# MDIL-SNU/SevenNet

Measured on AMD Instinct MI355X. Metric: atom-steps/sec (energy+forces), SevenNet-0 100k-atom cell, 1/2/4/8 MI355X, higher is better.
Workload: dtype f32 (storage / accumulate / tensor product; in-kernel W2 products f16x3 = two fp16 terms per operand, three matrix-core products: fp32-rounding class; node linears bf16x6); 1 GPU; sevennet_0 shape (5 interaction layers), 97336-atom periodic diamond-Si cell (a=5.431 A x 23^3, sigma=0.05 A), cutoff 5.0 A, 2725408 directed edges, seeded synthetic weights; atoms=97336, edges=2725408, parallelism=single GPU, fused=auto, terms=4

## Files before the change

### include/snet_hip.h

```cpp
#ifndef SNET_HIP_H
#define SNET_HIP_H

#include <stdint.h>

#ifdef __cplusplus
extern "C" {
#endif

#define SNET_ABI_VERSION 4

int snet_abi_version(void);
const char *snet_last_error(void);
int snet_conv_num_shapes(void);
const char *snet_conv_shape_tag(int i);

typedef struct snet_edge_params {
  float cutoff;
  int32_t n_basis;
  int32_t cutoff_kind;
  int32_t poly_p;
  float cutoff_on;
  int32_t lmax;
  int32_t normalize;
} snet_edge_params;

int snet_edge_vectors(const double *pos, const int32_t *center, const int32_t *src, const double *shift, int64_t n_edges,
                      float *edge_vec, void *stream);
int snet_edge_embed_fwd(const snet_edge_params *p_host, const float *coeffs_host, const float *edge_vec,
                        int64_t n_edges, float *emb, float *sh, float *dsh, void *stream);
int snet_edge_embed_bwd(const snet_edge_params *p_host, const float *coeffs_host, const float *edge_vec,
                        int64_t n_edges, const float *g_emb, const float *g_sh, float *g_vec, int32_t accumulate,
                        void *stream);

int snet_gemm(const float *A, const float *B, float *C, int64_t n_nodes, int32_t d, int32_t K, int32_t N,
              int64_t a_node_stride, int64_t a_off, int64_t c_node_stride, int64_t c_off,
              const int32_t *row_idx, int32_t accumulate, void *stream);

typedef struct snet_gemm_desc {
  const float *B;
  const void *B_split;
  int64_t a_off, c_off;
  int32_t d, K, N, accumulate;
} snet_gemm_desc;
#define SNET_MAX_GEMM_GROUP 8
int snet_gemm_grouped(const snet_gemm_desc *descs_host, int32_t n_desc, const float *A, float *C, int64_t n_nodes,
                      int64_t a_node_stride, int64_t c_node_stride, const int32_t *row_idx, void *stream);
int64_t snet_gemm_split_size(int32_t K, int32_t N);
int snet_gemm_split_pack(const float *B_host, int32_t K, int32_t N, void *packed_host);
typedef struct snet_mlp_plan snet_mlp_plan;
int snet_radial_mlp_plan_create(int32_t nb, int32_t h1, int32_t h2, int32_t wn, const float *W0_host,
                                const float *W1_host, const float *W2_host, int32_t act, float cst, int32_t mode,
                                snet_mlp_plan **plan);
void snet_radial_mlp_plan_destroy(snet_mlp_plan *plan);
int snet_radial_mlp_fwd(const snet_mlp_plan *plan, const float *emb, int64_t n_edges, float *w_out, void *stream);
int snet_radial_mlp_bwd(const snet_mlp_plan *plan, const float *emb, const float *g_w, int64_t n_edges,
                        float *g_emb, void *stream);

int snet_act_fwd(const float *z, float *a, int64_t n, int32_t act, float cst, void *stream);
int snet_act_bwd(const float *z, const float *g_a, float *g_z, int64_t n, int32_t act, float cst, void *stream);

typedef struct snet_conv_plan snet_conv_plan;
int snet_conv_plan_create(const char *tag, snet_conv_plan **plan);
void snet_conv_plan_destroy(snet_conv_plan *plan);
int snet_conv_register_library(const char *path);
int snet_conv_plan_dims(const snet_conv_plan *plan, int32_t *dx, int32_t *dout, int32_t *nsh, int32_t *wn);

int snet_conv_fwd(const snet_conv_plan *plan, const float *x, const float *sh, const float *w, const int32_t *w_row,
                  const int32_t *row_ptr, const int32_t *src, int64_t n_dst, float scale, float *out,
                  void *stream);
#define SNET_FUSED_TERMS_DEFAULT 4
typedef struct snet_fused_plan snet_fused_plan;
int snet_radial_mlp_hidden_fwd(const snet_mlp_plan *plan, const float *emb, int64_t n_edges, float *h2, void *stream);
int snet_radial_mlp_hidden_fwd_layers(const snet_mlp_plan *const *plans, int32_t n_layers, const float *emb, int64_t n_edges,
                                      float *const *h2, void *stream);
int snet_radial_mlp_hidden_bwd(const snet_mlp_plan *plan, const float *emb, const float *g_h2, int64_t n_edges,
                               float *g_emb, void *stream);
int snet_conv_fused_available(const snet_conv_plan *plan);
int snet_fused_plan_create(const snet_conv_plan *plan, const snet_mlp_plan *mlp, int32_t terms, snet_fused_plan **out);
void snet_fused_plan_destroy(snet_fused_plan *plan);
int snet_edge_tiles(const int32_t *row_ptr, int64_t n_dst, int32_t *tile_ptr, int32_t *tile_node, int64_t tile_capacity,
                    int64_t *n_tiles, void *stream);
int snet_edge_tiles_packed(const int32_t *row_ptr, int64_t node_begin, int64_t node_end, int32_t *tile_e0,
                           int32_t *tile_nodes, int64_t tile_capacity, int64_t *n_tiles, void *stream);
int snet_fused_plan_tile_mode(const snet_fused_plan *plan);
int snet_conv_plan_transposed(const snet_conv_plan *plan, char *tag, float *col_scale, int32_t *dead, int32_t dead_capacity,
                              int32_t *n_dead);
int snet_edges_by_source(const int32_t *row_ptr, int64_t n_dst, const int32_t *eperm, const int32_t *w_row, int64_t n_edges,
                         int32_t *center_t, int32_t *w_row_t, void *stream);
int snet_conv_fwd_fused(const snet_fused_plan *plan, const float *x, const float *sh, const float *h2,
                        const int32_t *w_row, const int32_t *row_ptr, const int32_t *src, int64_t n_dst, float scale,
                        float *out, void *stream);
int snet_conv_bwd_fused(const snet_fused_plan *plan, const float *x, const float *sh, const float *dsh,
                        const float *h2, const int32_t *w_row, const int32_t *row_ptr, const int32_t *src,
                        const int32_t *tile_ptr, const int32_t *tile_node, int64_t n_tiles, float scale,
                        const float *g_out, float *g_xe, float *g_h2, const float *emb, float *g_emb, float *g_vec,
                        const float *x_rowmax, const float *g_rowmax, void *stream);
int snet_conv_bwd_fused_sh(const snet_fused_plan *plan, const float *x, const float *sh, const float *h2, const int32_t *w_row,
                           const int32_t *row_ptr, const int32_t *src, const int32_t *tile_ptr, const int32_t *tile_node,
                           int64_t n_tiles, float scale, const float *g_out, float *g_xe, float *g_h2, const float *emb,
                           float *g_emb, float *g_sh, const float *x_rowmax, const float *g_rowmax, void *stream);
int snet_fused_plan_has_mlp_tail(const snet_fused_plan *plan);
int snet_fused_plan_prefers_tangent(const snet_fused_plan *plan);
int snet_edge_embed_tangent(const snet_edge_params *p_host, const float *coeffs_host, const float *edge_vec,
                            const int32_t *edge_of_row, int64_t n_rows, float *demb, void *stream);
int snet_radial_mlp_hidden_fwd_layers_tangent(const snet_mlp_plan *const *plans, int32_t n_layers, const float *emb, const float *demb,
                                              int64_t n_rows, float *const *h2, float *const *h2d, void *stream);
int snet_conv_bwd_fused_tangent(const snet_fused_plan *plan, const float *x, const float *sh, const float *dsh, const float *h2,
                                const float *h2d, const int32_t *w_row, const int32_t *row_ptr, const int32_t *src,
                                const int32_t *tile_ptr, const int32_t *tile_node, int64_t n_tiles, float scale, const float *g_out,
                                float *g_xe, const float *edge_vec, float *g_vec, const float *x_rowmax, const float *g_rowmax,
                                void *stream);
typedef struct snet_layer0_plan snet_layer0_plan;
int snet_layer0_plan_create(const snet_conv_plan *conv, const float *W2_host, const float *table_host, float scale,
                            int32_t n_slots, snet_layer0_plan **plan);
void snet_layer0_plan_destroy(snet_layer0_plan *plan);
int snet_layer0_fold(const float *W2_host, int32_t wn, int32_t mul, const float *table_host, float scale, int32_t n_slots, int32_t l,
                     float *bt_host);
int64_t snet_layer0_scratch_size(const snet_layer0_plan *plan, int64_t n_nodes);
int snet_layer0_conv_bwd(const snet_layer0_plan *plan, const float *g_out, const float *h2, const float *h2d, const int32_t *w_row,
                         const int32_t *row_ptr, const int32_t *src, const int32_t *types, const int32_t *species_slot,
                         const float *sh, const float *dsh, const float *edge_vec, int64_t n_nodes, float *scratch, float *g_vec,
                         void *stream);
typedef struct snet_lastlayer_plan snet_lastlayer_plan;
int snet_lastlayer_plan_create(const snet_conv_plan *conv, const float *W2_host, snet_lastlayer_plan **plan);
void snet_lastlayer_plan_destroy(snet_lastlayer_plan *plan);
int snet_lastlayer_conv_bwd(const snet_lastlayer_plan *plan, const float *x, const float *g_out, const float *sh, const float *dsh,
                            const float *edge_vec, const float *h2, const float *h2d, const int32_t *col_ptr,
                            const int32_t *center_t, const int32_t *w_row_t, const int32_t *eperm, int64_t row_a, int64_t row_b,
                            float scale, float *g_x, float *g_vec, void *stream);
int snet_fused_plan_gxe_chunks(const snet_fused_plan *plan, int32_t *chunk_pos, int32_t capacity);
int snet_segment_sum_rows_chunked(const float *x, const int32_t *seg_ptr, const int32_t *perm, int64_t n_seg, int32_t dim,
                                  const int32_t *chunk_pos, float *out, void *stream);
int snet_row_absmax(const float *x, int64_t n_rows, int32_t dim, float *out, void *stream);
int snet_row_absmax_multi(const float *const *x, const int64_t *n_rows, const int32_t *dims, float *const *out, int32_t n,
                          void *stream);
int snet_row_norm2(const float *x, int64_t n_rows, int32_t dim, float mult, float *out, void *stream);
int snet_conv_bwd_edge(const snet_conv_plan *plan, const float *x, const float *sh, const float *w,
                       const int32_t *w_row, const int32_t *row_ptr, const int32_t *src, int64_t n_dst, float scale,
                       const float *g_out, float *g_w, float *g_xe, float *g_sh, void *stream);
int snet_conv_bwd_edge_vec(const snet_conv_plan *plan, const float *x, const float *sh, const float *dsh,
                           const float *w, const int32_t *w_row, const int32_t *row_ptr, const int32_t *src,
                           int64_t n_dst, float scale, const float *g_out, float *g_w, float *g_xe, float *g_vec,
                           void *stream);
int snet_conv_bwd_node(const snet_conv_plan *plan, const float *sh, const float *w, const int32_t *w_row,
                       const int32_t *col_ptr,
                       const int32_t *eperm, const int32_t *dst, int64_t n_src, float scale,
                       const float *g_out, float *g_x, void *stream);

int snet_segment_sum_rows(const float *x, const int32_t *seg_ptr, const int32_t *perm, int64_t n_seg, int32_t dim,
                          float *out, void *stream);

typedef struct snet_gate_seg {
  int32_t kind;
  int32_t in_off;
  int32_t out_off;
  int32_t mul;
  int32_t l;
  int32_t gate_off;
  int32_t act;
  float cst;
} snet_gate_seg;
#define SNET_MAX_GATE_SEGS 16
int snet_gate_fwd(float *y, const float *addend, float *out, int64_t n_nodes, int32_t dim_in, int32_t dim_out,
                  const snet_gate_seg *segs_host, int32_t n_segs, void *stream);
int snet_gate_bwd(const float *y, const float *g_out, float *g_y, int64_t n_nodes, int32_t dim_in,
                  int32_t dim_out, const snet_gate_seg *segs_host, int32_t n_segs, void *stream);
int snet_gate_bwd_norm(const float *y, const float *g_out, float *g_y, int64_t n_nodes, int32_t dim_in, int32_t dim_out,
                       const snet_gate_seg *segs, int32_t n_segs, float norm_mult, float *row_norm, void *stream);

int snet_embed_rows(const float *table, const int32_t *types, float *out, int64_t n_nodes, int32_t dim,
                    void *stream);

int snet_add_inplace(float *y, const float *x, int64_t n, void *stream);
int snet_add_row_bias(float *y, const float *bias, int64_t n_rows, int32_t dim, void *stream);
int snet_permute_cols(const float *x, const int32_t *col_idx, float *out, int64_t n_rows, int32_t dim,
                      void *stream);

int snet_rescale_reduce(const float *e_scaled, const int32_t *types, const float *scale, const float *shift,
                        int32_t n_scale, int64_t n_nodes, float *e_atom, double *energy, void *stream);

int snet_i32_shift(const int32_t *in, int32_t delta, int32_t *out, int64_t n, void *stream);

int snet_readout_energy(const float *x, int64_t n_nodes, int32_t dim, const double *v, double c, const int32_t *types,
                        const float *scale, const float *shift, int32_t n_scale, float *e_atom, double *energy,
                        void *stream);
int snet_readout_grad(const double *v, int32_t dim, const int32_t *types, const float *scale, int32_t n_scale,
                      int64_t n_nodes, float *g_x, void *stream);

int snet_edge_force(const float *g_vec, const float *edge_vec, const int32_t *row_ptr, const int32_t *col_ptr,
                    const int32_t *eperm, int64_t n_nodes, int64_t n_edges, float *forces, float *virial_atom,
                    double *virial_total, void *stream);

int snet_readout_energy_seg(const float *x, int64_t n_nodes, int32_t dim, const double *v, double c, const int32_t *types,
                            const float *scale, const float *shift, int32_t n_scale, const int32_t *seg_ptr, int32_t n_seg,
                            float *e_atom, double *energy_seg, double *energy_total, void *stream);
int snet_rescale_reduce_seg(const float *e_scaled, const int32_t *types, const float *scale, const float *shift,
                            int32_t n_scale, int64_t n_nodes, const int32_t *seg_ptr, int32_t n_seg, float *e_atom,
                            double *energy_seg, double *energy_total, void *stream);
int snet_edge_force_seg(const float *g_vec, const float *edge_vec, const int32_t *row_ptr, const int32_t *col_ptr,
// ... 168 lines not shown
```

### sevennet_amd/_lib.py

```python
from __future__ import annotations

import ctypes as C
import os

_HERE = os.path.dirname(os.path.abspath(__file__))
ABI_VERSION = 4
LIB_PATH = os.environ.get('SNET_HIP_LIB') or os.path.join(_HERE, 'libsnet_hip.so')

c_f32p = C.c_void_p
c_i32p = C.c_void_p
c_f64p = C.c_void_p
c_stream = C.c_void_p


class EdgeParams(C.Structure):
    _fields_ = [('cutoff', C.c_float), ('n_basis', C.c_int32), ('cutoff_kind', C.c_int32),
                ('poly_p', C.c_int32), ('cutoff_on', C.c_float), ('lmax', C.c_int32),
                ('normalize', C.c_int32)]


class GemmDesc(C.Structure):
    _fields_ = [('B', C.c_void_p), ('B_split', C.c_void_p), ('a_off', C.c_int64), ('c_off', C.c_int64), ('d', C.c_int32), ('K', C.c_int32),
                ('N', C.c_int32), ('accumulate', C.c_int32)]


class GateSeg(C.Structure):
    _fields_ = [('kind', C.c_int32), ('in_off', C.c_int32), ('out_off', C.c_int32), ('mul', C.c_int32),
                ('l', C.c_int32), ('gate_off', C.c_int32), ('act', C.c_int32), ('cst', C.c_float)]


SIGNATURES = {
    'snet_abi_version': (C.c_int, []),
    'snet_last_error': (C.c_char_p, []),
    'snet_conv_num_shapes': (C.c_int, []),
    'snet_conv_shape_tag': (C.c_char_p, [C.c_int]),
    'snet_edge_embed_fwd': (C.c_int, [C.POINTER(EdgeParams), C.POINTER(C.c_float), c_f32p, C.c_int64, c_f32p,
                                      c_f32p, c_f32p, c_stream]),
    'snet_edge_embed_bwd': (C.c_int, [C.POINTER(EdgeParams), C.POINTER(C.c_float), c_f32p, C.c_int64, c_f32p,
                                      c_f32p, c_f32p, C.c_int32, c_stream]),
    'snet_radial_mlp_plan_create': (C.c_int, [C.c_int32, C.c_int32, C.c_int32, C.c_int32, C.POINTER(C.c_float),
                                              C.POINTER(C.c_float), C.POINTER(C.c_float), C.c_int32, C.c_float,
                                              C.c_int32, C.POINTER(C.c_void_p)]),
    'snet_radial_mlp_plan_destroy': (None, [C.c_void_p]),
    'snet_radial_mlp_fwd': (C.c_int, [C.c_void_p, c_f32p, C.c_int64, c_f32p, c_stream]),
    'snet_radial_mlp_bwd': (C.c_int, [C.c_void_p, c_f32p, c_f32p, C.c_int64, c_f32p, c_stream]),
    'snet_conv_bwd_edge_vec': (C.c_int, [C.c_void_p, c_f32p, c_f32p, c_f32p, c_f32p, c_i32p, c_i32p, c_i32p, C.c_int64,
                                         C.c_float, c_f32p, c_f32p, c_f32p, c_f32p, c_stream]),
    'snet_gemm': (C.c_int, [c_f32p, c_f32p, c_f32p, C.c_int64, C.c_int32, C.c_int32, C.c_int32, C.c_int64,
                            C.c_int64, C.c_int64, C.c_int64, c_i32p, C.c_int32, c_stream]),
    'snet_gemm_grouped': (C.c_int, [C.POINTER(GemmDesc), C.c_int32, c_f32p, c_f32p, C.c_int64, C.c_int64, C.c_int64,
                                    c_i32p, c_stream]),
    'snet_gemm_split_size': (C.c_int64, [C.c_int32, C.c_int32]),
    'snet_gemm_split_pack': (C.c_int, [C.c_void_p, C.c_int32, C.c_int32, C.c_void_p]),
    'snet_act_fwd': (C.c_int, [c_f32p, c_f32p, C.c_int64, C.c_int32, C.c_float, c_stream]),
    'snet_act_bwd': (C.c_int, [c_f32p, c_f32p, c_f32p, C.c_int64, C.c_int32, C.c_float, c_stream]),
    'snet_conv_plan_create': (C.c_int, [C.c_char_p, C.POINTER(C.c_void_p)]),
    'snet_conv_plan_destroy': (None, [C.c_void_p]),
    'snet_conv_register_library': (C.c_int, [C.c_char_p]),
    'snet_conv_plan_dims': (C.c_int, [C.c_void_p, C.POINTER(C.c_int32), C.POINTER(C.c_int32),
                                      C.POINTER(C.c_int32), C.POINTER(C.c_int32)]),
    'snet_conv_fwd': (C.c_int, [C.c_void_p, c_f32p, c_f32p, c_f32p, c_i32p, c_i32p, c_i32p, C.c_int64, C.c_float,
                                c_f32p, c_stream]),
    'snet_radial_mlp_hidden_fwd': (C.c_int, [C.c_void_p, c_f32p, C.c_int64, c_f32p, c_stream]),
    'snet_radial_mlp_hidden_fwd_layers': (C.c_int, [C.POINTER(C.c_void_p), C.c_int32, c_f32p, C.c_int64, C.POINTER(C.c_void_p), c_stream]),
    'snet_radial_mlp_hidden_bwd': (C.c_int, [C.c_void_p, c_f32p, c_f32p, C.c_int64, c_f32p, c_stream]),
    'snet_conv_fused_available': (C.c_int, [C.c_void_p]),
    'snet_conv_plan_transposed': (C.c_int, [C.c_void_p, C.c_char_p, c_f32p, c_i32p, C.c_int32, C.POINTER(C.c_int32)]),
    'snet_edges_by_source': (C.c_int, [c_i32p, C.c_int64, c_i32p, c_i32p, C.c_int64, c_i32p, c_i32p, c_stream]),
    'snet_fused_plan_create': (C.c_int, [C.c_void_p, C.c_void_p, C.c_int32, C.POINTER(C.c_void_p)]),
    'snet_fused_plan_destroy': (None, [C.c_void_p]),
    'snet_edge_tiles': (C.c_int, [c_i32p, C.c_int64, c_i32p, c_i32p, C.c_int64, C.POINTER(C.c_int64), c_stream]),
    'snet_conv_fwd_fused': (C.c_int, [C.c_void_p, c_f32p, c_f32p, c_f32p, c_i32p, c_i32p, c_i32p, C.c_int64, C.c_float,
                                      c_f32p, c_stream]),
    'snet_conv_bwd_fused': (C.c_int, [C.c_void_p, c_f32p, c_f32p, c_f32p, c_f32p, c_i32p, c_i32p, c_i32p, c_i32p,
                                      c_i32p, C.c_int64, C.c_float, c_f32p, c_f32p, c_f32p, c_f32p, c_f32p, c_f32p, c_f32p, c_f32p,
                                      c_stream]),
    'snet_conv_bwd_fused_sh': (C.c_int, [C.c_void_p, c_f32p, c_f32p, c_f32p, c_i32p, c_i32p, c_i32p, c_i32p,
                                         c_i32p, C.c_int64, C.c_float, c_f32p, c_f32p, c_f32p, c_f32p, c_f32p, c_f32p, c_f32p, c_f32p,
                                         c_stream]),
    'snet_fused_plan_has_mlp_tail': (C.c_int, [C.c_void_p]),
    'snet_fused_plan_prefers_tangent': (C.c_int, [C.c_void_p]),
    'snet_edge_embed_tangent': (C.c_int, [C.POINTER(EdgeParams), C.POINTER(C.c_float), c_f32p, c_i32p, C.c_int64, c_f32p, c_stream]),
    'snet_radial_mlp_hidden_fwd_layers_tangent': (C.c_int, [C.POINTER(C.c_void_p), C.c_int32, c_f32p, c_f32p, C.c_int64,
                                                            C.POINTER(C.c_void_p), C.POINTER(C.c_void_p), c_stream]),
    'snet_conv_bwd_fused_tangent': (C.c_int, [C.c_void_p, c_f32p, c_f32p, c_f32p, c_f32p, c_f32p, c_i32p, c_i32p, c_i32p, c_i32p,
                                              c_i32p, C.c_int64, C.c_float, c_f32p, c_f32p, c_f32p, c_f32p, c_f32p, c_f32p,
                                              c_stream]),
    'snet_model_set_layer0_moments': (C.c_int, [C.c_void_p, C.c_int32]),
    'snet_layer0_plan_create': (C.c_int, [C.c_void_p, C.c_void_p, C.c_void_p, C.c_float, C.c_int32, C.POINTER(C.c_void_p)]),
    'snet_layer0_fold': (C.c_int, [C.c_void_p, C.c_int32, C.c_int32, C.c_void_p, C.c_float, C.c_int32, C.c_int32, C.c_void_p]),
    'snet_layer0_plan_destroy': (None, [C.c_void_p]),
    'snet_layer0_scratch_size': (C.c_int64, [C.c_void_p, C.c_int64]),
    'snet_layer0_conv_bwd': (C.c_int, [C.c_void_p, c_f32p, c_f32p, c_f32p, c_i32p, c_i32p, c_i32p, c_i32p, c_i32p, c_f32p, c_f32p, c_f32p,
                                       C.c_int64, c_f32p, c_f32p, c_stream]),
    'snet_model_set_last_layer_merged': (C.c_int, [C.c_void_p, C.c_int32]),
    'snet_lastlayer_plan_create': (C.c_int, [C.c_void_p, C.c_void_p, C.POINTER(C.c_void_p)]),
    'snet_lastlayer_plan_destroy': (None, [C.c_void_p]),
    'snet_lastlayer_conv_bwd': (C.c_int, [C.c_void_p, c_f32p, c_f32p, c_f32p, c_f32p, c_f32p, c_f32p, c_f32p, c_i32p, c_i32p, c_i32p,
                                          c_i32p, C.c_int64, C.c_int64, C.c_float, c_f32p, c_f32p, c_stream]),
    'snet_fused_plan_gxe_chunks': (C.c_int, [C.c_void_p, C.POINTER(C.c_int32), C.c_int32]),
    'snet_segment_sum_rows_chunked': (C.c_int, [c_f32p, c_i32p, c_i32p, C.c_int64, C.c_int32, c_i32p, c_f32p, c_stream]),
    'snet_edge_vectors': (C.c_int, [c_f64p, c_i32p, c_i32p, c_f64p, C.c_int64, c_f32p, c_stream]),
    'snet_row_absmax': (C.c_int, [c_f32p, C.c_int64, C.c_int32, c_f32p, c_stream]),
    'snet_row_absmax_multi': (C.c_int, [C.POINTER(C.c_void_p), C.POINTER(C.c_int64), C.POINTER(C.c_int32), C.POINTER(C.c_void_p), C.c_int32, c_stream]),
    'snet_row_norm2': (C.c_int, [c_f32p, C.c_int64, C.c_int32, C.c_float, c_f32p, c_stream]),
    'snet_conv_bwd_edge': (C.c_int, [C.c_void_p, c_f32p, c_f32p, c_f32p, c_i32p, c_i32p, c_i32p, C.c_int64, C.c_float,
                                     c_f32p, c_f32p, c_f32p, c_f32p, c_stream]),
    'snet_segment_sum_rows': (C.c_int, [c_f32p, c_i32p, c_i32p, C.c_int64, C.c_int32, c_f32p, c_stream]),
    'snet_conv_bwd_node': (C.c_int, [C.c_void_p, c_f32p, c_f32p, c_i32p, c_i32p, c_i32p, c_i32p, C.c_int64, C.c_float,
                                     c_f32p, c_f32p, c_stream]),
    'snet_gate_fwd': (C.c_int, [c_f32p, c_f32p, c_f32p, C.c_int64, C.c_int32, C.c_int32, C.POINTER(GateSeg), C.c_int32,
                                c_stream]),
    'snet_gate_bwd': (C.c_int, [c_f32p, c_f32p, c_f32p, C.c_int64, C.c_int32, C.c_int32, C.POINTER(GateSeg),
                                C.c_int32, c_stream]),
    'snet_gate_bwd_norm': (C.c_int, [c_f32p, c_f32p, c_f32p, C.c_int64, C.c_int32, C.c_int32, C.POINTER(GateSeg),
                                     C.c_int32, C.c_float, c_f32p, c_stream]),
    'snet_embed_rows': (C.c_int, [c_f32p, c_i32p, c_f32p, C.c_int64, C.c_int32, c_stream]),
    'snet_add_row_bias': (C.c_int, [c_f32p, c_f32p, C.c_int64, C.c_int32, c_stream]),
    'snet_add_inplace': (C.c_int, [c_f32p, c_f32p, C.c_int64, c_stream]),
    'snet_permute_cols': (C.c_int, [c_f32p, c_i32p, c_f32p, C.c_int64, C.c_int32, c_stream]),
    'snet_rescale_reduce': (C.c_int, [c_f32p, c_i32p, c_f32p, c_f32p, C.c_int32, C.c_int64, c_f32p, c_f64p,
                                      c_stream]),
    'snet_readout_energy': (C.c_int, [c_f32p, C.c_int64, C.c_int32, c_f64p, C.c_double, c_i32p, c_f32p, c_f32p, C.c_int32,
                                      c_f32p, c_f64p, c_stream]),
    'snet_readout_grad': (C.c_int, [c_f64p, C.c_int32, c_i32p, c_f32p, C.c_int32, C.c_int64, c_f32p, c_stream]),
    'snet_edge_force': (C.c_int, [c_f32p, c_f32p, c_i32p, c_i32p, c_i32p, C.c_int64, C.c_int64, c_f32p, c_f32p,
                                  c_f64p, c_stream]),
    'snet_readout_energy_seg': (C.c_int, [c_f32p, C.c_int64, C.c_int32, c_f64p, C.c_double, c_i32p, c_f32p, c_f32p, C.c_int32,
                                          c_i32p, C.c_int32, c_f32p, c_f64p, c_f64p, c_stream]),
    'snet_rescale_reduce_seg': (C.c_int, [c_f32p, c_i32p, c_f32p, c_f32p, C.c_int32, C.c_int64, c_i32p, C.c_int32, c_f32p, c_f64p,
                                          c_f64p, c_stream]),
    'snet_edge_force_seg': (C.c_int, [c_f32p, c_f32p, c_i32p, c_i32p, c_i32p, C.c_int64, C.c_int64, c_i32p, C.c_int32, c_f32p,
                                      c_f32p, c_f64p, c_f64p, c_stream]),
    'snet_batch_nl_count': (C.c_int, [C.c_void_p, c_i32p, C.c_int32, C.c_void_p, c_i32p, C.c_int64, C.c_double, c_i32p, c_stream]),
    'snet_batch_nl_fill': (C.c_int, [C.c_void_p, c_i32p, C.c_int32, C.c_void_p, c_i32p, C.c_int64, C.c_double, c_i32p, c_i32p,
                                     c_i32p, c_f32p, c_i32p, c_stream]),
    'snet_fire_step': (C.c_int, [c_f64p, c_f64p, c_f32p, c_f64p, C.c_int64, c_i32p, C.c_int32, c_f64p, c_f64p, c_i32p, c_i32p, c_i32p,
                                 c_f64p, c_i32p, C.c_double, C.c_double, C.c_double, C.c_int32, C.c_double, C.c_double, C.c_double,
                                 C.c_double, C.c_double, c_stream]),
    'snet_fire_cell_step': (C.c_int, [c_f64p, c_f64p, c_f64p, c_f64p, c_f64p, c_f32p, c_f64p, c_f64p, c_f64p, C.c_int64, c_i32p, C.c_int32,
                                      c_f64p, c_f64p, c_i32p, c_i32p, c_i32p, c_i32p, c_f64p, c_i32p, C.c_double, C.c_double,
                                      C.c_double, C.c_int32, C.c_double, C.c_double, C.c_double, C.c_double, C.c_double, C.c_double,
                                      C.c_int32, C.c_int32, C.c_int32, C.c_double, c_stream]),
    'snet_neb_forces': (C.c_int, [c_f64p, c_f32p, c_f64p, c_f64p, c_f64p, C.c_int64, c_i32p, C.c_int32, c_i32p, C.c_int32, c_f64p, c_i32p,
                                  C.c_int64, c_f64p, c_f64p, c_f64p, c_i32p, c_i32p, c_f64p, C.c_int32, c_i32p, c_i32p, c_f64p, c_i32p,
                                  c_stream]),
    'snet_vib_displace': (C.c_int, [c_f64p, C.c_int64, c_i32p, C.c_int32, c_i32p, c_i32p, C.c_int32, C.c_double, c_f64p, C.c_int64, c_i32p,
                                    c_stream]),
    'snet_vib_rows': (C.c_int, [c_f32p, c_f64p, C.c_int64, c_i32p, C.c_int32, c_i32p, C.c_int32, C.c_int32, C.c_double, c_i32p, c_i32p,
                                C.c_int64, C.c_void_p, C.c_int32, c_f64p, C.c_int64, c_i32p, c_stream]),
    'snet_vib_finish': (C.c_int, [c_f64p, C.c_void_p, c_i32p, C.c_int64, c_f64p, C.c_int32, C.c_int64, c_i32p, c_f64p, c_f64p, c_f64p,
                                  c_stream]),
    'snet_ph_rows': (C.c_int, [c_f32p, c_f64p, C.c_int64, c_i32p, C.c_int32, c_i32p, C.c_int32, C.c_int32, C.c_double, c_i32p, c_i32p,
                               C.c_void_p, C.c_int32, c_f64p, C.c_int64, c_i32p, c_stream]),
    'snet_ph_finish': (C.c_int, [c_f64p, C.c_void_p, c_i32p, c_i32p, C.c_int32, C.c_int64, C.c_int32, c_i32p, c_f64p, c_f64p, c_stream]),
    'snet_ph_images': (C.c_int, [c_f64p, C.c_int64, c_i32p, c_i32p, c_i32p, C.c_int32, c_f64p, c_f64p, C.c_void_p, C.c_int32, C.c_double,
                                 c_i32p, c_i32p, C.c_int64, c_i32p, c_stream]),
    'snet_ph_dynmat': (C.c_int, [c_f64p, C.c_void_p, C.c_int64, c_f64p, C.c_int64, c_i32p, c_i32p, c_f64p, C.c_int32, c_f64p, c_i32p,
                                 c_i32p, C.c_void_p, C.c_int64, c_f64p, c_i32p, c_i32p, C.c_int32, C.c_void_p, C.c_int32, C.c_int32,
                                 c_i32p, c_f64p, c_f64p, C.c_int64, c_f64p, c_stream]),
    'snet_mdb_step': (C.c_int, [c_f64p, c_f64p, c_f32p, c_f64p, c_f64p, C.c_int64, c_i32p, c_i32p, C.c_int32, c_f64p, c_i32p, c_f64p,
                                C.c_double, C.c_double, C.c_double, C.c_uint64, C.c_int32, c_stream]),
    'snet_mdb_init_velocities': (C.c_int, [c_f64p, c_f64p, C.c_int64, c_i32p, c_i32p, C.c_int32, c_f64p, C.c_uint64, C.c_int32,
                                           c_stream]),
    'snet_mdb_npt_step': (C.c_int, [c_f64p, c_f64p, c_f64p, c_f32p, c_f64p, c_f64p, c_f64p, c_f64p, C.c_int64, c_i32p, c_i32p, C.c_int32,
                                    c_f64p, c_f64p, c_f64p, c_i32p, c_f64p, c_f64p, c_f64p, c_i32p, c_i32p, C.c_double, C.c_double,
                                    C.c_double, C.c_uint64, C.c_int32, C.c_double, C.c_double, c_stream]),
    'snet_nl_grid': (C.c_int, [C.POINTER(C.c_double), C.c_double, C.POINTER(C.c_int32), C.POINTER(C.c_double), C.POINTER(C.c_int32)]),
    'snet_nl_bin': (C.c_int, [C.POINTER(C.c_double), C.c_double, C.POINTER(C.c_int32), C.POINTER(C.c_double), C.c_void_p, C.c_int64,
                              C.c_void_p, c_i32p, c_i32p, c_stream]),
    'snet_nl_count': (C.c_int, [C.POINTER(C.c_double), C.c_double, C.POINTER(C.c_int32), C.POINTER(C.c_double), C.c_void_p, c_i32p,
                                c_i32p, c_i32p, C.c_int64, c_i32p, c_stream]),
    'snet_nl_fill': (C.c_int, [C.POINTER(C.c_double), C.c_double, C.POINTER(C.c_int32), C.POINTER(C.c_double), C.c_void_p, c_i32p,
                               c_i32p, c_i32p, c_i32p, C.c_int64, c_i32p, c_i32p, c_i32p, c_f32p, c_i32p, c_stream]),
    'snet_gather_rows': (C.c_int, [c_f32p, c_i32p, c_f32p, C.c_int64, C.c_int32, c_stream]),
    'snet_scatter_add_rows': (C.c_int, [c_f32p, c_i32p, c_f32p, C.c_int64, C.c_int32, c_stream]),
    'snet_model_load': (C.c_int, [C.c_char_p, C.POINTER(C.c_void_p)]),
    'snet_model_load_memory': (C.c_int, [C.c_void_p, C.c_int64, C.POINTER(C.c_void_p)]),
    'snet_model_destroy': (None, [C.c_void_p]),
    'snet_model_info': (C.c_int, [C.c_void_p, C.POINTER(C.c_float), C.POINTER(C.c_int32), C.POINTER(C.c_int32),
                                  C.POINTER(C.c_int32), C.c_int32]),
    'snet_model_meta': (C.c_int, [C.c_void_p, C.c_char_p, C.c_char_p, C.c_int32]),
    'snet_edge_tiles_packed': (C.c_int, [c_i32p, C.c_int64, C.c_int64, c_i32p, c_i32p, C.c_int64, C.POINTER(C.c_int64), c_stream]),
    'snet_fused_plan_tile_mode': (C.c_int, [C.c_void_p]),
    'snet_i32_shift': (C.c_int, [c_i32p, C.c_int32, c_i32p, C.c_int64, c_stream]),
    'snet_model_set_interior': (C.c_int, [C.c_void_p, C.c_int64]),
    'snet_model_set_topology_cache': (C.c_int, [C.c_void_p, C.c_int32]),
    'snet_model_topology_changed': (C.c_int, [C.c_void_p]),
    'snet_model_eval_syncs': (C.c_int64, [C.c_void_p]),
    'snet_model_set_halo': (C.c_int, [C.c_void_p, C.c_void_p, C.c_void_p, C.c_void_p, C.c_int32]),
    'snet_model_eval': (C.c_int, [C.c_void_p, C.c_int64, C.c_int64, C.c_int64, c_i32p, c_i32p, c_i32p, c_i32p, c_i32p,
                                  c_i32p, c_f32p, c_i32p, c_i32p, C.c_int64, C.c_void_p, c_f32p, c_f32p, c_f32p, C.c_void_p, c_f32p, c_stream]),
    'snet_rccl_unique_id': (C.c_int, [C.c_void_p]),
    'snet_rccl_comm_create': (C.c_int, [C.c_void_p, C.c_int32, C.c_int32, C.POINTER(C.c_void_p)]),
    'snet_rccl_comm_destroy': (None, [C.c_void_p]),
    'snet_rccl_available': (C.c_int, []),
    'snet_rccl_comm_info': (C.c_int, [C.c_void_p, C.POINTER(C.c_int32), C.POINTER(C.c_int32)]),
    'snet_rccl_allreduce_sum_f64': (C.c_int, [C.c_void_p, c_f64p, C.c_int64, c_stream]),
    'snet_loopback_hub_create': (C.c_int, [C.c_int32, C.POINTER(C.c_void_p)]),
    'snet_loopback_hub_abort': (None, [C.c_void_p]),
    'snet_loopback_hub_destroy': (None, [C.c_void_p]),
    'snet_loopback_comm_create': (C.c_int, [C.c_void_p, C.c_int32, C.POINTER(C.c_void_p)]),
    'snet_halo_create': (C.c_int, [C.c_void_p, C.c_int32, C.c_int32, C.c_void_p, C.c_void_p, C.c_void_p, C.c_void_p, C.POINTER(C.c_void_p)]),
    'snet_halo_destroy': (None, [C.c_void_p]),
# ... 86 lines not shown
```

### sevennet_amd/csrc/snet_gemm.hip

```cpp
#include <cmath>
#include <cstdlib>
#include <cstring>

#include <type_traits>

#include "snet_common.h"
#include "snet_split.h"

#ifndef SNET_GEMM_OCC
#define SNET_GEMM_OCC 4
#endif
namespace {

using snet::f32x16;

struct RowMap {
  int64_t n0;
  uint32_t m0, d, inv;
  __device__ __forceinline__ RowMap(int64_t row0, int d_) : d((uint32_t)d_), inv(65536u / (uint32_t)d_ + 1u) {
    n0 = row0 / d_;
    m0 = (uint32_t)(row0 - n0 * d_);
  }
  __device__ __forceinline__ void at(int off, int64_t &n, int &m) const {
    const uint32_t x = m0 + (uint32_t)off, q = (x * inv) >> 16;
// ... 227 lines not shown
  auto load_a = [&](int q, float (&v)[MT][8]) {
#pragma unroll
    for (int mt = 0; mt < MT; ++mt) {
      const int k = 16 * q + 8 * half;
      if (a_ok[mt] && a_vec && k + 7 < K) {
        const f32x4 lo = *reinterpret_cast<const f32x4 *>(a_ptr[mt] + 16 * q);
        const f32x4 hi = *reinterpret_cast<const f32x4 *>(a_ptr[mt] + 16 * q + 4);
#pragma unroll
        for (int i = 0; i < 4; ++i) { v[mt][i] = lo[i]; v[mt][4 + i] = hi[i]; }
      } else {
#pragma unroll
        for (int i = 0; i < 8; ++i) v[mt][i] = (a_ok[mt] && k + i < K) ? a_ptr[mt][16 * q + i] : 0.f;
      }
    }
  };
  constexpr int NST = (SLAB + 255) / 256;
  auto load_b = [&](int q, u32x4 (&st)[NST]) {
    if (tile0 + NT <= n_tiles) {
#pragma unroll
      for (int i = 0; i < NST; ++i) {
        const int idx = tid + 256 * i;
        const int t = idx / 192, rem = idx - 192 * t;
        if (SLAB % 256 == 0 || idx < SLAB) st[i] = Bp[((int64_t)(tile0 + t) * nq + q) * 192 + rem];
      }
      return;
    }
#pragma unroll
    for (int i = 0; i < NST; ++i) {
      const int idx = tid + 256 * i;
      const int t = idx / 192, rem = idx - 192 * t;
      u32x4 z = {0u, 0u, 0u, 0u};
      if (idx < SLAB && tile0 + t < n_tiles) z = Bp[((int64_t)(tile0 + t) * nq + q) * 192 + rem];
      st[i] = z;
    }
  };
  auto store_b = [&](int buf, const u32x4 (&st)[NST]) {
#pragma unroll
    for (int i = 0; i < NST; ++i) {
      const int idx = tid + 256 * i;
      if (idx < SLAB) Bs[buf * SLAB + idx] = st[i];
    }
  };

  f32x16 acc[MT][NT];
#pragma unroll
  for (int mt = 0; mt < MT; ++mt)
#pragma unroll
    for (int t = 0; t < NT; ++t) acc[mt][t] = zero16();

  float av[MT][8], an[MT][8];
  u32x4 st[NST];
  load_a(0, av);
  load_b(0, st);
  store_b(0, st);
  __syncthreads();
  int buf = 0;
  for (int q = 0; q < nq; ++q) {
    const bool more = q + 1 < nq;
    if (more) {
      load_a(q + 1, an);
      load_b(q + 1, st);
    }
    Split3 a[MT];
#pragma unroll
    for (int mt = 0; mt < MT; ++mt) a[mt] = split8(av[mt]);
#pragma unroll
    for (int t = 0; t < NT; ++t) {
      bf16x8 b[3];
#pragma unroll
      for (int term = 0; term < 3; ++term) b[term] = as_bf16x8(Bs[buf * SLAB + (t * 3 + term) * 64 + lane]);
#pragma unroll
      for (int mt = 0; mt < MT; ++mt) acc[mt][t] = mfma6(a[mt], b, acc[mt][t]);
    }
    if (more) {
      store_b(buf ^ 1, st);
#pragma unroll
      for (int mt = 0; mt < MT; ++mt)
#pragma unroll
        for (int i = 0; i < 8; ++i) av[mt][i] = an[mt][i];
    }
    __syncthreads();
    buf ^= 1;
  }

  gemm_split_store<NT, MT>(acc, rows, row0, half, li, tile0, C, n_rows, N, c_node_stride, c_off, row_idx, accumulate);
}


template <int NT>
__global__ __launch_bounds__(256) void gemm_kernel(
    const float *__restrict__ A, const float *__restrict__ B, float *__restrict__ C, int64_t n_rows, int d, int K,
    int N, int64_t a_node_stride, int64_t a_off, int64_t c_node_stride, int64_t c_off,
    const int32_t *__restrict__ row_idx, int accumulate) {
  __shared__ float As[BK * AS_STRIDE];
  __shared__ float Bs[BK * 32 * NT];
  gemm_body<NT>(As, Bs, blockIdx.x, blockIdx.y, A, B, C, n_rows, d, K, N, a_node_stride, a_off, c_node_stride, c_off,
                row_idx, accumulate);
}

struct GroupArgs {
  int n;
  int first_block[SNET_MAX_GEMM_GROUP + 1];
  int nbx[SNET_MAX_GEMM_GROUP];
  snet_gemm_desc p[SNET_MAX_GEMM_GROUP];
};

__global__ __launch_bounds__(256) void gemm_grouped_kernel(GroupArgs G, const float *__restrict__ A,
                                                           float *__restrict__ C, int64_t n_nodes,
                                                           int64_t a_node_stride, int64_t c_node_stride,
                                                           const int32_t *__restrict__ row_idx) {
  __shared__ float As[BK * AS_STRIDE];
  __shared__ float Bs[BK * 128];
  int q = 0;
  while (q + 1 < G.n && (int)blockIdx.x >= G.first_block[q + 1]) ++q;
  const snet_gemm_desc P = G.p[q];
  const int b = blockIdx.x - G.first_block[q];
  const int bx = b % G.nbx[q], by = b / G.nbx[q];
  const int64_t n_rows = n_nodes * P.d;
  if (P.N > 64)
    gemm_body<4>(As, Bs, bx, by, A, P.B, C, n_rows, P.d, P.K, P.N, a_node_stride, P.a_off, c_node_stride, P.c_off,
                 row_idx, P.accumulate);
  else if (P.N > 32)
    gemm_body<2>(As, Bs, bx, by, A, P.B, C, n_rows, P.d, P.K, P.N, a_node_stride, P.a_off, c_node_stride, P.c_off,
                 row_idx, P.accumulate);
  else
    gemm_body<1>(As, Bs, bx, by, A, P.B, C, n_rows, P.d, P.K, P.N, a_node_stride, P.a_off, c_node_stride, P.c_off,
                 row_idx, P.accumulate);
}

template <int MT>
__global__ __launch_bounds__(256, MT == 1 ? SNET_GEMM_OCC : 2) void gemm_split_grouped_kernel(GroupArgs G, const float *__restrict__ A,
                                                                    float *__restrict__ C, int64_t n_nodes,
                                                                    int64_t a_node_stride, int64_t c_node_stride,
                                                                    const int32_t *__restrict__ row_idx) {
  __shared__ snet::u32x4 Bs[2 * 4 * 192];
  int q = 0;
  while (q + 1 < G.n && (int)blockIdx.x >= G.first_block[q + 1]) ++q;
  const snet_gemm_desc P = G.p[q];
  const int b = blockIdx.x - G.first_block[q];
  const int bx = b % G.nbx[q], by = b / G.nbx[q];
  const int64_t n_rows = n_nodes * P.d;
  const snet::u32x4 *Bp = static_cast<const snet::u32x4 *>(P.B_split);
  if (P.N > 64)
    gemm_split_body<4, MT>(Bs, bx, by, A, Bp, C, n_rows, P.d, P.K, P.N, a_node_stride, P.a_off, c_node_stride, P.c_off,
                           row_idx, P.accumulate);
  else if (P.N > 32)
    gemm_split_body<2, MT>(Bs, bx, by, A, Bp, C, n_rows, P.d, P.K, P.N, a_node_stride, P.a_off, c_node_stride, P.c_off,
                           row_idx, P.accumulate);
  else
    gemm_split_body<1, MT>(Bs, bx, by, A, Bp, C, n_rows, P.d, P.K, P.N, a_node_stride, P.a_off, c_node_stride, P.c_off,
                           row_idx, P.accumulate);
}

inline uint16_t bf16_rne(float v) {
  uint32_t u;
  memcpy(&u, &v, 4);
  u += 0x7fffu + ((u >> 16) & 1u);
  return (uint16_t)(u >> 16);
}
inline float bf16_f(uint16_t h) {
  const uint32_t u = (uint32_t)h << 16;
  float f;
  memcpy(&f, &u, 4);
  return f;
}

}

extern "C" int64_t snet_gemm_split_size(int32_t K, int32_t N) {
  if (K < 1 || N < 1) return 0;
  return (int64_t)((N + 31) / 32) * ((K + 15) / 16) * 3 * 64 * 16;
}

extern "C" int snet_gemm_split_pack(const float *B_host, int32_t K, int32_t N, void *packed_host) {
  SNET_REQUIRE(B_host != nullptr && packed_host != nullptr && K >= 1 && N >= 1, "snet_gemm_split_pack: bad argument");
  uint16_t *out = static_cast<uint16_t *>(packed_host);
  const int nq = (K + 15) / 16, n_tiles = (N + 31) / 32;
  for (int t = 0; t < n_tiles; ++t)
    for (int q = 0; q < nq; ++q)
      for (int lane = 0; lane < 64; ++lane)
        for (int i = 0; i < 8; ++i) {
          const int k = 16 * q + 8 * (lane >> 5) + i, n = 32 * t + (lane & 31);
          const float x = (k < K && n < N) ? B_host[(size_t)k * N + n] : 0.f;
          const uint16_t h = bf16_rne(x);
          const float r1 = x - bf16_f(h);
          const uint16_t m = bf16_rne(r1);
          const uint16_t l = bf16_rne(r1 - bf16_f(m));
          const size_t base = ((size_t)(t * nq + q) * 3) * 64;
          out[((base + 0 * 64 + lane) * 8) + i] = h;
          out[((base + 1 * 64 + lane) * 8) + i] = m;
          out[((base + 2 * 64 + lane) * 8) + i] = l;
        }
  return 0;
}

extern "C" int snet_gemm_grouped(const snet_gemm_desc *descs_host, int32_t n_desc, const float *A, float *C,
                                 int64_t n_nodes, int64_t a_node_stride, int64_t c_node_stride,
                                 const int32_t *row_idx, void *stream) {
  SNET_REQUIRE(descs_host != nullptr && n_desc >= 1 && n_desc <= SNET_MAX_GEMM_GROUP,
               "snet_gemm_grouped: 1..8 problems required");
  if (n_nodes <= 0) return 0;
  GroupArgs G;
  G.n = n_desc;
  int n_split = 0;
  int64_t rows_max = 0;  (void)rows_max;
  for (int i = 0; i < n_desc; ++i) {
    n_split += descs_host[i].B_split != nullptr;
    rows_max = rows_max > n_nodes * descs_host[i].d ? rows_max : n_nodes * descs_host[i].d;
  }
  SNET_REQUIRE(n_split == 0 || n_split == n_desc, "snet_gemm_grouped: mix of split-packed and fp32 weights in one group");
  const bool split = n_split > 0;
  static const int mt_env = getenv("SNET_GEMM_MT") ? atoi(getenv("SNET_GEMM_MT")) : 0;
  const int mt = mt_env ? mt_env : 1;
  const int bm = split ? 128 * mt : BM;
  int64_t total = 0;
  for (int i = 0; i < n_desc; ++i) {
    const snet_gemm_desc &p = descs_host[i];
    SNET_REQUIRE(p.d >= 1 && p.d <= 150 && p.K >= 1 && p.N >= 1 && (p.B != nullptr || p.B_split != nullptr),
                 "snet_gemm_grouped: bad problem");
    const int bn = p.N > 64 ? 128 : (p.N > 32 ? 64 : 32);
    const int64_t nbx = (n_nodes * p.d + bm - 1) / bm;
    const int64_t nby = (p.N + bn - 1) / bn;
    SNET_REQUIRE(nbx < (1ll << 30), "snet_gemm_grouped: too many rows");
    G.p[i] = p;
    G.nbx[i] = (int)nbx;
    G.first_block[i] = (int)total;
    total += nbx * nby;
  }
  G.first_block[n_desc] = (int)total;
  SNET_REQUIRE(total < (1ll << 31), "snet_gemm_grouped: grid too large");
  hipStream_t st = static_cast<hipStream_t>(stream);
  if (!split)
    gemm_grouped_kernel<<<(unsigned)total, 256, 0, st>>>(G, A, C, n_nodes, a_node_stride, c_node_stride, row_idx);
  else if (mt == 2)
    gemm_split_grouped_kernel<2><<<(unsigned)total, 256, 0, st>>>(G, A, C, n_nodes, a_node_stride, c_node_stride, row_idx);
  else
    gemm_split_grouped_kernel<1><<<(unsigned)total, 256, 0, st>>>(G, A, C, n_nodes, a_node_stride, c_node_stride, row_idx);
  SNET_CHECK_LAUNCH("snet_gemm_grouped");
  return 0;
}

extern "C" int snet_gemm(const float *A, const float *B, float *C, int64_t n_nodes, int32_t d, int32_t K,
                         int32_t N, int64_t a_node_stride, int64_t a_off, int64_t c_node_stride, int64_t c_off,
                         const int32_t *row_idx, int32_t accumulate, void *stream) {
  SNET_REQUIRE(d >= 1 && d <= 150 && K >= 1 && N >= 1, "snet_gemm: bad shape (1 <= d <= 150)");
  if (n_nodes <= 0) return 0;
  hipStream_t st = static_cast<hipStream_t>(stream);
  const int64_t n_rows = n_nodes * d;
  const int64_t gx = (n_rows + BM - 1) / BM;
  SNET_REQUIRE(gx < (1ll << 31), "snet_gemm: too many rows");
  if (N > 64) {
    dim3 grid((unsigned)gx, (unsigned)((N + 127) / 128));
    gemm_kernel<4><<<grid, 256, 0, st>>>(A, B, C, n_rows, d, K, N, a_node_stride, a_off, c_node_stride, c_off,
                                         row_idx, accumulate);
  } else if (N > 32) {
    dim3 grid((unsigned)gx, 1);
    gemm_kernel<2><<<grid, 256, 0, st>>>(A, B, C, n_rows, d, K, N, a_node_stride, a_off, c_node_stride, c_off,
                                         row_idx, accumulate);
  } else {
    dim3 grid((unsigned)gx, 1);
    gemm_kernel<1><<<grid, 256, 0, st>>>(A, B, C, n_rows, d, K, N, a_node_stride, a_off, c_node_stride, c_off,
                                         row_idx, accumulate);
  }
  SNET_CHECK_LAUNCH("snet_gemm");
  return 0;
}
```

### sevennet_amd/csrc/snet_model.cpp

```cpp
#include <algorithm>
#include <cmath>
#include <cstdio>
#include <cstdlib>
#include <cstring>
#include <exception>
#include <map>
#include <string>
#include <vector>

#include "snet_common.h"

namespace {

struct Reader {
  const unsigned char *p, *end;
  bool ok = true;
  void get(void *dst, size_t n) {
    if (!ok || (size_t)(end - p) < n) {
      ok = false;
      return;
    }
    memcpy(dst, p, n);
    p += n;
  }
  int32_t i32() {
    int32_t v = 0;
    get(&v, 4);
    return v;
  }
  float f32() {
    float v = 0;
    get(&v, 4);
    return v;
  }
  double f64() {
    double v = 0;
    get(&v, 8);
    return v;
  }
  std::vector<double> darr(size_t n) {
    if (!ok || n > (size_t)(end - p) / 8) {
      ok = false;
      return {};
    }
    std::vector<double> v(n);
    if (n) get(v.data(), 8 * n);
    return v;
  }
  std::vector<float> farr(size_t n) {
    if (!ok || n > (size_t)(end - p) / 4) {
      ok = false;
      return {};
    }
    std::vector<float> v(n);
    if (n) get(v.data(), 4 * n);
    return v;
  }
};

struct Block {
  int l, in_off, mul_in, out_off, mul_out, species, accumulate;
  void *W = nullptr, *WT = nullptr;
};
struct Linear {
  int dim_in = 0, dim_out = 0, n_species = 0;
  std::vector<Block> blocks;
  std::vector<std::pair<int, int>> zero, zero_in;
  struct Group {
    int species;
    std::vector<snet_gemm_desc> descs;
  };
  std::vector<Group> fwd, rev;
  float *bias = nullptr;
  float t_norm = 0.f;
  bool present() const { return dim_out > 0; }
};

void plan_groups(Linear &L, bool transpose) {
  auto &groups = transpose ? L.rev : L.fwd;
  std::vector<std::pair<int, int>> written;
  std::vector<std::vector<int>> targets;
  for (const Block &b : L.blocks) {
    const int tgt = transpose ? b.in_off : b.out_off;
    bool acc = false;
    for (auto &w : written) acc |= (w.first == tgt && w.second == b.species);
    snet_gemm_desc d;
    d.B = nullptr;
    d.B_split = transpose ? b.WT : b.W;
    d.a_off = transpose ? b.out_off : b.in_off;
    d.c_off = tgt;
    d.d = 2 * b.l + 1;
    d.K = transpose ? b.mul_out : b.mul_in;
    d.N = transpose ? b.mul_in : b.mul_out;
    d.accumulate = acc;
    bool placed = false;
    if (!groups.empty() && groups.back().species == b.species && groups.back().descs.size() < SNET_MAX_GEMM_GROUP) {
      bool clash = false;
      for (int t : targets.back()) clash |= (t == tgt);
      if (!clash) {
        groups.back().descs.push_back(d);
        targets.back().push_back(tgt);
        placed = true;
      }
    }
    if (!placed) {
      groups.push_back({b.species, {d}});
      targets.push_back({tgt});
    }
    written.push_back({tgt, b.species});
  }
}
struct Layer {
  int dx, dmid, gin, dout, wn;
  char tag[13];
  float conv_scale;
  int mlp[4];
  snet_conv_plan *conv = nullptr;
  snet_mlp_plan *mlp_plan = nullptr;
  snet_fused_plan *fused = nullptr;
  int32_t *gxe_chunks = nullptr;
  snet_conv_plan *tconv = nullptr;
  snet_mlp_plan *tmlp = nullptr;
  snet_fused_plan *tfused = nullptr;
  snet_lastlayer_plan *merged = nullptr;
  int tile_mode = 0;
  std::vector<int32_t> t_dead;
  Linear sc, si1, si2;
  std::vector<snet_gate_seg> segs;
};

bool dev_upload(const std::vector<float> &h, float **d) {
  if (h.empty()) {
    *d = nullptr;
    return true;
  }
  if (hipMalloc((void **)d, h.size() * 4) != hipSuccess) return false;
  return hipMemcpy(*d, h.data(), h.size() * 4, hipMemcpyHostToDevice) == hipSuccess;
}

bool upload_split(const std::vector<float> &w, int K, int N, void **d) {
  std::vector<unsigned char> packed((size_t)snet_gemm_split_size(K, N));
  if (snet_gemm_split_pack(w.data(), K, N, packed.data())) return false;
  if (hipMalloc(d, packed.size()) != hipSuccess) return false;
  return hipMemcpy(*d, packed.data(), packed.size(), hipMemcpyHostToDevice) == hipSuccess;
}

bool read_linear(Reader &r, Linear &L) {
  L.dim_in = r.i32();
  L.dim_out = r.i32();
  L.n_species = r.i32();
  const int nb = r.i32(), nz = r.i32(), nzi = r.i32();
  if (!r.ok || nb < 0 || nb > 4096 || nz < 0 || nz > 4096 || nzi < 0 || nzi > 4096) return false;
  L.blocks.resize(nb);
  for (auto &b : L.blocks) {
    b.l = r.i32(); b.in_off = r.i32(); b.mul_in = r.i32(); b.out_off = r.i32(); b.mul_out = r.i32();
    b.species = r.i32(); b.accumulate = r.i32();
    if (!r.ok || b.l < 0 || b.l > 8 || b.mul_in <= 0 || b.mul_out <= 0 || b.mul_in > (1 << 16) || b.mul_out > (1 << 16) ||
        b.in_off < 0 || b.out_off < 0 || b.species < -1)
      return false;
  }
  for (int i = 0; i < nz; ++i) {
    const int off = r.i32(), len = r.i32();
    L.zero.push_back({off, len});
  }
  for (int i = 0; i < nzi; ++i) {
    const int off = r.i32(), len = r.i32();
    L.zero_in.push_back({off, len});
  }
  std::map<std::pair<int, int>, std::vector<double>> row_sq;
  for (auto &b : L.blocks) {
    std::vector<float> w = r.farr((size_t)b.mul_in * b.mul_out);
    if (!r.ok) return false;
    std::vector<float> wt(w.size());
    for (int k = 0; k < b.mul_in; ++k)
      for (int n = 0; n < b.mul_out; ++n) wt[(size_t)n * b.mul_in + k] = w[(size_t)k * b.mul_out + n];
    if (!upload_split(w, b.mul_in, b.mul_out, &b.W) || !upload_split(wt, b.mul_out, b.mul_in, &b.WT)) return false;
    auto &sq = row_sq[{b.in_off, b.species}];
    sq.resize((size_t)b.mul_in, 0.0);
    for (int k = 0; k < b.mul_in; ++k)
      for (int n = 0; n < b.mul_out; ++n) sq[k] += (double)w[(size_t)k * b.mul_out + n] * w[(size_t)k * b.mul_out + n];
  }
  for (auto &kv : row_sq)
    for (double v : kv.second) L.t_norm = std::max(L.t_norm, (float)std::sqrt(v));
  const int has_bias = r.i32();
  if (!r.ok || (has_bias != 0 && has_bias != 1)) return false;
  if (has_bias) {
    std::vector<float> b = r.farr((size_t)L.dim_out);
    if (!r.ok || !dev_upload(b, &L.bias)) return false;
  }
  plan_groups(L, false);
  plan_groups(L, true);
  return r.ok;
}

struct Arena {
  char *base = nullptr;
  size_t cap = 0, off = 0;
  float *f(size_t n) {
    const size_t bytes = ((n * 4 + 255) / 256) * 256;
    float *p = reinterpret_cast<float *>(base + off);
    off += bytes;
    return p;
  }
};

}

struct snet_model {
  int n_species, n_layers, lmax, normalize, n_basis, cutoff_kind, poly_p, act_radial, n_scale, d0;
  float cutoff, cutoff_on, act_cst;
  std::vector<float> coeffs;
  float *embed = nullptr, *scale = nullptr, *shift = nullptr;
  double *ro_v = nullptr, ro_c = 0.0;
  std::vector<int> fcn_dims;
  std::vector<float *> fcn_w, fcn_wt;
  int fcn_act = 0;
  float fcn_cst = 1.f;
  double *one_d = nullptr;
  float *h0_table = nullptr, *sc0_table = nullptr;
  float scale0 = 1.f;
  std::vector<Layer> layers;
  Linear ro1, ro2;
  std::string meta;
  Arena arena;
  snet_halo_fn halo_fwd = nullptr, halo_rev = nullptr;
  void *halo_user = nullptr;
  bool fold_forces = true;
  std::vector<std::vector<int32_t>> species_rows_host;
  int32_t *species_rows = nullptr;
  size_t species_rows_cap = 0;
  std::vector<int64_t> species_off, species_cnt;
  bool topo_cache = false, topo_valid = false;
  struct TopoKey { int64_t NT, N, E; const void *row_ptr, *src, *eperm, *w_row; } topo_key{0, 0, 0, nullptr, nullptr, nullptr, nullptr};
  int32_t *c_tile_ptr = nullptr, *c_tile_node = nullptr, *c_center_t = nullptr, *c_w_row_t = nullptr;
  size_t c_tile_cap = 0, c_edge_cap = 0, c_node_cap = 0;
  int64_t c_n_tiles = 0;
  int64_t n_interior = 0;
  hipStream_t halo_stream = nullptr;
  hipEvent_t ev_h0 = nullptr, ev_h1 = nullptr;
  int32_t *c_tile_ptr_b = nullptr;
  size_t c_tile_ptr_b_cap = 0;
  int64_t c_tile_k = 0;
  bool c_split_valid = false;
  int32_t *c_ptile_e0 = nullptr, *c_ptile_nodes = nullptr;
  size_t c_ptile_cap = 0;
  int64_t c_pn_tiles = 0, c_ptile_k = 0;
  std::vector<int32_t> types_prev;
  int64_t eval_syncs = 0;
  hipStream_t side = nullptr;
  hipEvent_t ev_main = nullptr, ev_bwd[2] = {nullptr, nullptr};
  std::vector<hipEvent_t> ev_w;
  bool overlap = getenv("SNET_NO_OVERLAP") == nullptr;
  int fused_terms = [] {
    const char *e = getenv("SNET_FUSED_TERMS");
    const int v = e ? atoi(e) : SNET_FUSED_TERMS_DEFAULT;
    return v >= 1 && v <= 4 ? v : SNET_FUSED_TERMS_DEFAULT;
  }();
  bool l0_mode = [] {
    const char *e = getenv("SNET_LAYER0_MOMENTS");
    return e == nullptr || strcmp(e, "0") != 0;
  }();
  bool ll_mode = [] {
    const char *e = getenv("SNET_LAST_LAYER_MERGED");
    return e == nullptr || strcmp(e, "0") != 0;
  }();
  bool l0_shape_ok = false;
  std::vector<float> h0_host;
  struct L0Plan { snet_layer0_plan *plan; int32_t *slot; int n_slots; };
  std::map<std::vector<int32_t>, L0Plan> l0_plans;
  std::vector<int32_t> l0_present;
  const void *l0_key_types = nullptr;
  int64_t l0_key_nt = -1;
};

constexpr int64_t OVERLAP_MAX_EDGES = 1000000;

namespace {

int run_linear(snet_model *m, const Linear &L, const float *x, float *y, int64_t n, bool transpose, bool accumulate_all,
               hipStream_t st) {
  if (n <= 0) return 0;
  const int64_t a_stride = transpose ? L.dim_out : L.dim_in, c_stride = transpose ? L.dim_in : L.dim_out;
  if (!accumulate_all)
    for (auto &z : transpose ? L.zero_in : L.zero)
      if (hipMemset2DAsync(y + z.first, (size_t)c_stride * 4, 0, (size_t)z.second * 4, (size_t)n, st) != hipSuccess) {
        snet::set_error("snet_model_eval: memset failed");
        return 1;
      }
  for (const Linear::Group &g : transpose ? L.rev : L.fwd) {
    const int32_t *rows = nullptr;
    int64_t cnt = n;
    if (g.species >= 0) {
      cnt = m->species_cnt[g.species];
      rows = m->species_rows + m->species_off[g.species];
      if (cnt == 0) continue;
    }
    int rc;
    if (accumulate_all) {
      snet_gemm_desc tmp[SNET_MAX_GEMM_GROUP];
      for (size_t i = 0; i < g.descs.size(); ++i) {
        tmp[i] = g.descs[i];
        tmp[i].accumulate = 1;
      }
      rc = snet_gemm_grouped(tmp, (int)g.descs.size(), x, y, cnt, a_stride, c_stride, rows, st);
    } else {
      rc = snet_gemm_grouped(g.descs.data(), (int)g.descs.size(), x, y, cnt, a_stride, c_stride, rows, st);
    }
    if (rc) return rc;
  }
  if (!transpose && L.bias) return snet_add_row_bias(y, L.bias, n, L.dim_out, st);
  return 0;
}

}

extern "C" int snet_model_load_memory(const void *blob, int64_t n_bytes, snet_model **out) {
  SNET_REQUIRE(blob != nullptr && out != nullptr && n_bytes > 8, "snet_model_load: null / empty model");
  Reader r{static_cast<const unsigned char *>(blob), static_cast<const unsigned char *>(blob) + n_bytes};
  char magic[8];
  r.get(magic, 8);
  SNET_REQUIRE(r.ok && memcmp(magic, "SNETMDL4", 8) == 0, "snet_model_load: not a .snet model file of this version (SNETMDL4)");
  auto *m = new snet_model;
  bool good = false;
  try {
  m->n_species = r.i32(); m->n_layers = r.i32(); m->lmax = r.i32(); m->normalize = r.i32(); m->n_basis = r.i32();
  m->cutoff_kind = r.i32(); m->poly_p = r.i32(); m->act_radial = r.i32(); m->n_scale = r.i32(); m->d0 = r.i32();
  m->cutoff = r.f32(); m->cutoff_on = r.f32(); m->act_cst = r.f32();
  good = r.ok && m->n_layers > 0 && m->n_layers < 64 && m->n_basis > 0 && m->n_basis <= 16 && m->n_species > 0 &&
         m->n_species <= 4096 && m->lmax >= 0 && m->lmax <= 3 && (m->normalize == 0 || m->normalize == 1) &&
         (m->act_radial >= 0 && m->act_radial < 7) && (m->cutoff_kind == 0 || m->cutoff_kind == 1) &&
         (m->n_scale == 1 || m->n_scale == m->n_species) && m->d0 > 0 && m->d0 <= (1 << 16) && m->cutoff > 0.f;
  if (good) {
    m->coeffs = r.farr(m->n_basis);
    std::vector<float> emb = r.farr((size_t)m->n_species * m->d0), sc = r.farr(m->n_scale), sh = r.farr(m->n_scale);
    good = r.ok && dev_upload(emb, &m->embed) && dev_upload(sc, &m->scale) && dev_upload(sh, &m->shift);
    if (good) m->scale0 = sc[0];
  }
  for (int t = 0; good && t < m->n_layers; ++t) {
    Layer L;
    L.dx = r.i32(); L.dmid = r.i32(); L.gin = r.i32(); L.dout = r.i32(); L.wn = r.i32();
    r.get(L.tag, 12);
    L.tag[12] = 0;
    L.conv_scale = r.f32();
    for (int i = 0; i < 4; ++i) L.mlp[i] = r.i32();
    if (!r.ok) { good = false; break; }
    bool dims_ok = L.dx > 0 && L.dmid > 0 && L.gin > 0 && L.dout > 0 && L.wn > 0;
    for (int i = 0; i < 4; ++i) dims_ok = dims_ok && L.mlp[i] > 0 && L.mlp[i] <= (1 << 16);
    for (int v : {L.dx, L.dmid, L.gin, L.dout, L.wn}) dims_ok = dims_ok && v <= (1 << 20);
    if (!dims_ok) { good = false; break; }
    std::vector<float> w0 = r.farr((size_t)L.mlp[0] * L.mlp[1]), w1 = r.farr((size_t)L.mlp[1] * L.mlp[2]),
                       w2 = r.farr((size_t)L.mlp[2] * L.mlp[3]);
    good = r.ok && L.mlp[3] == L.wn;
    if (good && snet_radial_mlp_plan_create(L.mlp[0], L.mlp[1], L.mlp[2], L.mlp[3], w0.data(), w1.data(), w2.data(),
                                            m->act_radial, m->act_cst, 1, &L.mlp_plan)) good = false;
    if (good && snet_conv_plan_create(L.tag, &L.conv)) good = false;
    if (good && getenv("SNET_NO_FUSED") == nullptr && snet_conv_fused_available(L.conv) &&
        snet_fused_plan_create(L.conv, L.mlp_plan, m->fused_terms, &L.fused))
      good = false;
    if (good && L.fused) {
      L.tile_mode = snet_fused_plan_tile_mode(L.fused);
      std::vector<int32_t> cp((size_t)L.dx / 16);
      good = snet_fused_plan_gxe_chunks(L.fused, cp.data(), (int32_t)cp.size()) == 0 &&
             hipMalloc((void **)&L.gxe_chunks, cp.size() * 4) == hipSuccess &&
             hipMemcpy(L.gxe_chunks, cp.data(), cp.size() * 4, hipMemcpyHostToDevice) == hipSuccess;
    }
    if (good && L.fused && t > 0 && L.dmid < L.dx && getenv("SNET_NO_TRANSPOSED") == nullptr) {
      char ttag[13];
      std::vector<float> cs((size_t)L.wn);
      int32_t dead[32], nd = 0;
      if (snet_conv_plan_transposed(L.conv, ttag, cs.data(), dead, 32, &nd) == 0 && ttag[0] != 0 &&
          snet_conv_plan_create(ttag, &L.tconv) == 0 && snet_conv_fused_available(L.tconv)) {
        std::vector<float> w2t(w2);
        for (int k = 0; k < L.mlp[2]; ++k)
          for (int c = 0; c < L.wn; ++c) w2t[(size_t)k * L.wn + c] *= cs[c];
        good = snet_radial_mlp_plan_create(L.mlp[0], L.mlp[1], L.mlp[2], L.mlp[3], w0.data(), w1.data(), w2t.data(),
                                           m->act_radial, m->act_cst, 1, &L.tmlp) == 0 &&
               snet_fused_plan_create(L.tconv, L.tmlp, m->fused_terms, &L.tfused) == 0;
        L.t_dead.assign(dead, dead + 2 * nd);
      } else if (L.tconv) {
        snet_conv_plan_destroy(L.tconv);
        L.tconv = nullptr;
      }
    }
    good = good && read_linear(r, L.sc) && read_linear(r, L.si1) && read_linear(r, L.si2);
    if (good) {
      const int ns = r.i32();
      good = r.ok && ns >= 1 && ns <= SNET_MAX_GATE_SEGS;
      for (int i = 0; good && i < ns; ++i) {
        snet_gate_seg s;
        s.kind = r.i32(); s.in_off = r.i32(); s.out_off = r.i32(); s.mul = r.i32(); s.l = r.i32();
        s.gate_off = r.i32(); s.act = r.i32(); s.cst = r.f32();
        L.segs.push_back(s);
      }
      good = good && r.ok;
    }
    m->layers.push_back(L);
  }
  const int ro_kind = good ? r.i32() : 0;
  good = good && r.ok && (ro_kind == 0 || ro_kind == 1);
  if (good && ro_kind == 0) good = read_linear(r, m->ro1) && read_linear(r, m->ro2);
  if (good) {
    const int dx0 = r.i32(), gin0 = r.i32();
    good = r.ok && dx0 == m->layers[0].dx && (gin0 == 0 || gin0 == m->layers[0].gin) && (gin0 != 0) == m->layers[0].sc.present();
    if (good) {
      std::vector<float> h0 = r.farr((size_t)m->n_species * dx0), sc0 = r.farr((size_t)m->n_species * gin0);
      good = r.ok && dev_upload(h0, &m->h0_table) && dev_upload(sc0, &m->sc0_table);
      m->h0_host = h0;
    }
  }
  if (good && ro_kind == 1) {
    const int nl = r.i32();
    good = r.ok && nl >= 1 && nl <= 16;
    for (int i = 0; good && i <= nl; ++i) {
      m->fcn_dims.push_back(r.i32());
      good = r.ok && m->fcn_dims.back() >= 1 && m->fcn_dims.back() <= (1 << 16);
    }
    m->fcn_act = good ? r.i32() : 0;
    m->fcn_cst = good ? r.f32() : 1.f;
    good = good && r.ok && m->fcn_act >= 0 && m->fcn_act < snet::N_ACT && m->fcn_dims.front() == m->layers.back().dout && m->fcn_dims.back() == 1;
    for (int i = 0; good && i < nl; ++i) {
      const int di = m->fcn_dims[i], dn = m->fcn_dims[i + 1];
      std::vector<float> w = r.farr((size_t)di * dn), wt((size_t)di * dn);
      for (int a = 0; a < di && r.ok; ++a)
        for (int b = 0; b < dn; ++b) wt[(size_t)b * di + a] = w[(size_t)a * dn + b];
      float *dw = nullptr, *dwt = nullptr;
      good = r.ok && dev_upload(w, &dw) && dev_upload(wt, &dwt);
      m->fcn_w.push_back(dw);
      m->fcn_wt.push_back(dwt);
    }
    const double one = 1.0;
    good = good && hipMalloc((void **)&m->one_d, 8) == hipSuccess && hipMemcpy(m->one_d, &one, 8, hipMemcpyHostToDevice) == hipSuccess;
    if (good) m->ro1.dim_in = m->fcn_dims.front();
  }
  if (good && ro_kind == 0) {
    const int d_ro = r.i32();
    m->ro_c = r.f64();
    good = r.ok && d_ro == m->ro1.dim_in && d_ro == m->layers.back().dout;
    if (good) {
      std::vector<double> v = r.darr((size_t)d_ro);
      good = r.ok && hipMalloc((void **)&m->ro_v, v.size() * 8) == hipSuccess &&
             hipMemcpy(m->ro_v, v.data(), v.size() * 8, hipMemcpyHostToDevice) == hipSuccess;
    }
  }
  if (good) {
    const int nm = r.i32();
    good = r.ok && nm >= 0 && nm <= (1 << 20) && (int64_t)(r.end - r.p) == nm;
    if (good) m->meta.assign(reinterpret_cast<const char *>(r.p), (size_t)nm);
  }
  if (good && ("\n" + m->meta).find("\nlayer0_moments=1\n") != std::string::npos) {
    const Layer &L0 = m->layers[0];
    snet_layer0_plan *probe = nullptr;
    const int nsl = m->n_species <= 4 ? m->n_species : 1;
    if (L0.fused && L0.mlp[1] == 64 && L0.mlp[2] == 64 &&
        snet_layer0_plan_create(L0.conv, snet::mlp_plan_w2_host(L0.mlp_plan), m->h0_host.data(), L0.conv_scale, nsl, &probe) == 0) {
      m->l0_shape_ok = true;
      if (m->n_species <= 4) {
        std::vector<int32_t> all(m->n_species);
        for (int s = 0; s < m->n_species; ++s) all[s] = s;
        int32_t *ds = nullptr;
        good = hipMalloc((void **)&ds, all.size() * 4) == hipSuccess &&
               hipMemcpy(ds, all.data(), all.size() * 4, hipMemcpyHostToDevice) == hipSuccess;
        m->l0_plans[all] = {probe, ds, m->n_species};
      } else {
        snet_layer0_plan_destroy(probe);
      }
    }
  }
  if (good && m->n_layers > 1 && ("\n" + m->meta).find("\nlast_layer_merged=1\n") != std::string::npos) {
    Layer &LL = m->layers.back();
    if (LL.fused && LL.tfused && m->fused_terms == 4 && LL.mlp[1] == 64 && LL.mlp[2] == 64 &&
        snet_lastlayer_plan_create(LL.conv, snet::mlp_plan_w2_host(LL.mlp_plan), &LL.merged) != 0)
      LL.merged = nullptr;
  }
  } catch (const std::exception &e) {
    snet::set_error(std::string("exception: ") + e.what());
    good = false;
  }
  if (!good) {
    const std::string prev = snet_last_error();
    snet::set_error("snet_model_load: malformed model file or device upload failed" +
                    (prev.empty() ? std::string() : " (" + prev + ")"));
    snet_model_destroy(m);
    return 1;
  }
  *out = m;
  return 0;
}

extern "C" int snet_model_load(const char *path, snet_model **out) {
  SNET_REQUIRE(path != nullptr, "snet_model_load: null path");
  FILE *f = fopen(path, "rb");
  if (!f) {
    snet::set_error(std::string("snet_model_load: cannot open ") + path);
    return 1;
  }
  fseek(f, 0, SEEK_END);
  const long n = ftell(f);
  fseek(f, 0, SEEK_SET);
  std::vector<unsigned char> buf(n > 0 ? n : 0);
  const size_t got = n > 0 ? fread(buf.data(), 1, n, f) : 0;
  fclose(f);
  SNET_REQUIRE((long)got == n && n > 0, "snet_model_load: short read");
  return snet_model_load_memory(buf.data(), n, out);
}

extern "C" void snet_model_destroy(snet_model *m) {
  if (!m) return;
  auto free_lin = [](Linear &L) {
    for (auto &b : L.blocks) {
      if (b.W) (void)hipFree(b.W);
      if (b.WT) (void)hipFree(b.WT);
    }
    if (L.bias) (void)hipFree(L.bias);
  };
  for (float *w : m->fcn_w) if (w) (void)hipFree(w);
  for (float *w : m->fcn_wt) if (w) (void)hipFree(w);
  if (m->one_d) (void)hipFree(m->one_d);
  for (auto &kv : m->l0_plans) {
    snet_layer0_plan_destroy(kv.second.plan);
    if (kv.second.slot) (void)hipFree(kv.second.slot);
  }
  for (auto &L : m->layers) {
    snet_fused_plan_destroy(L.fused);
    snet_fused_plan_destroy(L.tfused);
    snet_lastlayer_plan_destroy(L.merged);
    snet_radial_mlp_plan_destroy(L.tmlp);
    snet_conv_plan_destroy(L.tconv);
    if (L.gxe_chunks) (void)hipFree(L.gxe_chunks);
    snet_conv_plan_destroy(L.conv);
    snet_radial_mlp_plan_destroy(L.mlp_plan);
    free_lin(L.sc); free_lin(L.si1); free_lin(L.si2);
  }
  free_lin(m->ro1); free_lin(m->ro2);
  for (hipEvent_t e : m->ev_w) if (e) (void)hipEventDestroy(e);
  for (hipEvent_t e : {m->ev_main, m->ev_bwd[0], m->ev_bwd[1]}) if (e) (void)hipEventDestroy(e);
  if (m->side) (void)hipStreamDestroy(m->side);
  if (m->halo_stream) (void)hipStreamDestroy(m->halo_stream);
// ... 290 lines not shown
    if (m->topo_cache) {
      if (m->c_node_cap < (size_t)N + 64 || m->c_tile_cap < (size_t)N + (size_t)E / 16 + 64) {
        if (m->c_tile_ptr) (void)hipFree(m->c_tile_ptr);
        if (m->c_tile_node) (void)hipFree(m->c_tile_node);
        m->c_tile_ptr = m->c_tile_node = nullptr;
        m->c_node_cap = (size_t)N + 64;
        m->c_tile_cap = (size_t)N + (size_t)E / 16 + 64;
        SNET_REQUIRE(hipMalloc((void **)&m->c_tile_ptr, m->c_node_cap * 4) == hipSuccess &&
                         hipMalloc((void **)&m->c_tile_node, m->c_tile_cap * 4) == hipSuccess, "snet_model_eval: alloc");
      }
      tile_ptr = m->c_tile_ptr;
      tile_node = m->c_tile_node;
    } else {
      tile_ptr = reinterpret_cast<int32_t *>(A.f((size_t)N + 64));
      tile_node = reinterpret_cast<int32_t *>(A.f((size_t)N + (size_t)E / 16 + 64));
    }
    if (topo_hit) {
      n_tiles = m->c_n_tiles;
    } else {
      if ((rc = snet_edge_tiles(row_ptr, N, tile_ptr, tile_node, N + E / 16 + 1, &n_tiles, st))) return rc;
      ++m->eval_syncs;
      m->c_n_tiles = n_tiles;
    }
  }
  int32_t *ptile_e0 = nullptr, *ptile_nodes = nullptr;
  int64_t pn_tiles = 0, ptile_k = 0;
  if (need_tiles[1] && E > 0) {
    const size_t cap = (size_t)N + (size_t)E / 16 + 2;
    if (m->topo_cache) {
      if (m->c_ptile_cap < cap) {
        if (m->c_ptile_e0) (void)hipFree(m->c_ptile_e0);
        if (m->c_ptile_nodes) (void)hipFree(m->c_ptile_nodes);
        m->c_ptile_e0 = m->c_ptile_nodes = nullptr;
        m->c_ptile_cap = cap + cap / 8 + 64;
        SNET_REQUIRE(hipMalloc((void **)&m->c_ptile_e0, (m->c_ptile_cap + 1) * 4) == hipSuccess &&
                         hipMalloc((void **)&m->c_ptile_nodes, m->c_ptile_cap * 8) == hipSuccess, "snet_model_eval: alloc");
      }
      ptile_e0 = m->c_ptile_e0;
      ptile_nodes = m->c_ptile_nodes;
    } else {
      ptile_e0 = reinterpret_cast<int32_t *>(A.f((size_t)N + (size_t)E / 16 + 64));
      ptile_nodes = reinterpret_cast<int32_t *>(A.f(2 * ((size_t)N + (size_t)E / 16 + 64)));
    }
    if (topo_hit) {
      pn_tiles = m->c_pn_tiles;
      ptile_k = m->c_ptile_k;
    } else {
      const int64_t cut = n_int > 0 && n_int < N ? n_int : 0;
      int64_t nb = 0;
      if (cut > 0) {
        if ((rc = snet_edge_tiles_packed(row_ptr, 0, cut, ptile_e0, ptile_nodes, (int64_t)cap, &ptile_k, st))) return rc;
        ++m->eval_syncs;
      }
      if ((rc = snet_edge_tiles_packed(row_ptr, cut, N, ptile_e0 + ptile_k, ptile_nodes + 2 * ptile_k, (int64_t)cap - ptile_k, &nb, st)))
        return rc;
      ++m->eval_syncs;
      pn_tiles = ptile_k + nb;
      m->c_pn_tiles = pn_tiles;
      m->c_ptile_k = ptile_k;
    }
  }
  int32_t *center_t = nullptr, *w_row_t = nullptr;
  float *sh_t = nullptr;
  if (any_transposed && E > 0) {
    if (m->topo_cache) {
      if (m->c_edge_cap < (size_t)E + 64) {
        if (m->c_center_t) (void)hipFree(m->c_center_t);
        if (m->c_w_row_t) (void)hipFree(m->c_w_row_t);
        m->c_center_t = m->c_w_row_t = nullptr;
        m->c_edge_cap = (size_t)E + 64;
        SNET_REQUIRE(hipMalloc((void **)&m->c_center_t, m->c_edge_cap * 4) == hipSuccess &&
                         hipMalloc((void **)&m->c_w_row_t, m->c_edge_cap * 4) == hipSuccess, "snet_model_eval: alloc");
      }
      center_t = m->c_center_t;
      w_row_t = m->c_w_row_t;
    } else {
      center_t = reinterpret_cast<int32_t *>(A.f((size_t)E + 64));
      w_row_t = reinterpret_cast<int32_t *>(A.f((size_t)E + 64));
    }
    if (need_sh_t) sh_t = A.f((size_t)E * nsh + 64);
    if (!topo_hit && (rc = snet_edges_by_source(row_ptr, N, eperm, pairs ? w_row : nullptr, E, center_t, w_row_t, st))) return rc;
    if (need_sh_t && (rc = snet_gather_rows(sh, eperm, sh_t, E, nsh, st))) return rc;
  }
  int32_t *tile_ptr_b = nullptr;
  int64_t tile_k = 0;
  if (hsplit && need_tiles[0]) {
    if (m->c_tile_ptr_b_cap < (size_t)N + 64) {
      if (m->c_tile_ptr_b) (void)hipFree(m->c_tile_ptr_b);
      m->c_tile_ptr_b = nullptr;
      m->c_tile_ptr_b_cap = (size_t)N + 64;
      m->c_split_valid = false;
      SNET_REQUIRE(hipMalloc((void **)&m->c_tile_ptr_b, m->c_tile_ptr_b_cap * 4) == hipSuccess, "snet_model_eval: alloc");
    }
    tile_ptr_b = m->c_tile_ptr_b;
    if (topo_hit && m->c_split_valid) {
      tile_k = m->c_tile_k;
    } else {
      int32_t k32 = 0;
      SNET_REQUIRE(hipMemcpyAsync(&k32, tile_ptr + n_int, 4, hipMemcpyDeviceToHost, st) == hipSuccess &&
                       hipStreamSynchronize(st) == hipSuccess, "snet_model_eval: tile readback failed");
      ++m->eval_syncs;
      tile_k = m->c_tile_k = k32;
      if ((rc = snet_i32_shift(tile_ptr, -k32, tile_ptr_b, N + 1, st))) return rc;
      m->c_split_valid = true;
    }
  }
  if (!topo_hit && !(hsplit && need_tiles[0])) m->c_split_valid = false;
  if (m->topo_cache) {
    m->topo_key = key;
    m->topo_valid = true;
  }
  float *gw_buf[2] = {nullptr, nullptr};
  bool gw_busy[2] = {false, false};
  if (ov) {
    gw_buf[0] = A.f((size_t)E * wn_max);
    gw_buf[1] = A.f((size_t)E * wn_max);
    SNET_REQUIRE(hipEventRecord(m->ev_main, st) == hipSuccess && hipStreamWaitEvent(m->side, m->ev_main, 0) == hipSuccess,
                 "snet_model_eval: stream ordering failed");
    for (int t = 0; t < Lc; ++t) {
      if ((rc = snet_radial_mlp_fwd(m->layers[t].mlp_plan, emb_w, WR, saved[t].w, m->side))) return rc;
      SNET_REQUIRE(hipEventRecord(m->ev_w[t], m->side) == hipSuccess, "snet_model_eval: stream ordering failed");
    }
  }
  const size_t mark = A.off;

  {
    const snet_mlp_plan *hp[8];
    float *ho[8], *hd[8];
    float *demb = nullptr;
    for (int pass = 0; pass < 2; ++pass) {
      int nh = 0;
      for (int t = 0; t <= Lc; ++t) {
        if (t < Lc && m->layers[t].fused && (saved[t].wd != nullptr) == (pass == 0)) {
          hp[nh] = m->layers[t].mlp_plan; ho[nh] = saved[t].w; hd[nh] = saved[t].wd; ++nh;
        }
        if (nh == 8 || (t == Lc && nh > 0)) {
          if (pass == 0 && demb == nullptr) {
            demb = A.f((size_t)WR * nb);
            if ((rc = snet_edge_embed_tangent(&ep, m->coeffs.data(), edge_vec, pairs ? pair_edge : nullptr, WR, demb, st))) return rc;
          }
          if ((rc = pass == 0 ? snet_radial_mlp_hidden_fwd_layers_tangent(hp, nh, emb_w, demb, WR, ho, hd, st)
                              : snet_radial_mlp_hidden_fwd_layers(hp, nh, emb_w, WR, ho, st))) return rc;
          nh = 0;
        }
      }
    }
  }

  for (int t = 0; t < Lc; ++t) {
    Layer &L = m->layers[t];
    A.off = mark;
    float *sc = nullptr;
    float *h = saved[t].h;
    if (t == 0) {
      if (L.sc.present()) {
        sc = saved[t].y;
        if ((rc = snet_embed_rows(m->sc0_table, types, sc, N, L.gin, st))) return rc;
      }
      if ((rc = snet_embed_rows(m->h0_table, types, h, NT, L.dx, st))) return rc;
    } else {
      if (L.sc.present()) {
        sc = saved[t].y;
        if ((rc = run_linear(m, L.sc, x, sc, N, false, false, st))) return rc;
      }
      if ((rc = run_linear(m, L.si1, x, h, N, false, false, st))) return rc;
    }
    const bool fsplit = hsplit && t > 0 && L.fused != nullptr;
    if (t > 0 && has_halo) {
      if (fsplit)
        SNET_REQUIRE(hipEventRecord(m->ev_h0, st) == hipSuccess && hipStreamWaitEvent(m->halo_stream, m->ev_h0, 0) == hipSuccess,
                     "snet_model_eval: stream ordering failed");
      if ((rc = m->halo_fwd(m->halo_user, h, NT, N, L.dx, fsplit ? (void *)m->halo_stream : stream))) {
        snet::set_error("snet_model_eval: forward halo callback failed");
        return rc;
      }
      if (fsplit) SNET_REQUIRE(hipEventRecord(m->ev_h1, m->halo_stream) == hipSuccess, "snet_model_eval: stream ordering failed");
    }
    float *mid = A.f((size_t)N * L.dmid);
    if (E == 0) SNET_REQUIRE(hipMemsetAsync(mid, 0, (size_t)N * L.dmid * 4, st) == hipSuccess, "snet_model_eval: memset");
    else
      for (auto &z : L.si2.zero_in)
        SNET_REQUIRE(hipMemset2DAsync(mid + z.first, (size_t)L.dmid * 4, 0, (size_t)z.second * 4, (size_t)N, st) == hipSuccess,
                     "snet_model_eval: memset");
    if (L.fused) {
      const int64_t na = fsplit ? n_int : 0;
      if (na > 0 && (rc = snet_conv_fwd_fused(L.fused, h, sh, saved[t].w, pairs ? w_row : nullptr, row_ptr, src, na, L.conv_scale, mid, st)))
        return rc;
      if (fsplit) SNET_REQUIRE(hipStreamWaitEvent(st, m->ev_h1, 0) == hipSuccess, "snet_model_eval: stream ordering failed");
      if ((rc = snet_conv_fwd_fused(L.fused, h, sh, saved[t].w, pairs ? w_row : nullptr, row_ptr + na, src, N - na, L.conv_scale,
                                    mid + (size_t)na * L.dmid, st)))
        return rc;
    } else {
      if (ov)
        SNET_REQUIRE(hipStreamWaitEvent(st, m->ev_w[t], 0) == hipSuccess, "snet_model_eval: stream ordering failed");
      else if ((rc = snet_radial_mlp_fwd(L.mlp_plan, emb_w, WR, saved[t].w, st)))
        return rc;
      if ((rc = snet_conv_fwd(L.conv, h, sh, saved[t].w, pairs ? w_row : nullptr, row_ptr, src, N, L.conv_scale, mid, st)))
        return rc;
    }
    float *y = saved[t].y;
    if ((rc = run_linear(m, L.si2, mid, y, N, false, sc != nullptr, st))) return rc;
    if ((rc = snet_gate_fwd(y, nullptr, x2, N, L.gin, L.dout, L.segs.data(), (int)L.segs.size(), st))) return rc;
    std::swap(x, x2);
  }
  A.off = mark;
  float *ea = e_atom ? e_atom : A.f((size_t)N + 64);
  float *g_x = x2, *gx_next = x;
  if (!m->fcn_dims.empty()) {
    const std::vector<int> &d = m->fcn_dims;
    const int nl = (int)d.size() - 1;
    std::vector<float *> zs;
    const float *a = x;
    float *z = nullptr;
    for (int i = 0; i < nl; ++i) {
      z = A.f((size_t)N * d[i + 1] + 64);
      if ((rc = snet_gemm(a, m->fcn_w[i], z, N, 1, d[i], d[i + 1], d[i], 0, d[i + 1], 0, nullptr, 0, st))) return rc;
      if (i + 1 < nl) {
        float *an = A.f((size_t)N * d[i + 1] + 64);
        if ((rc = snet_act_fwd(z, an, N * d[i + 1], m->fcn_act, m->fcn_cst, st))) return rc;
        zs.push_back(z);
        a = an;
      }
    }
    if ((rc = snet_rescale_reduce(z, types, m->scale, m->shift, m->n_scale, N, ea, energy, st))) return rc;
    float *gz = A.f((size_t)N + 64);
    if ((rc = snet_readout_grad(m->one_d, 1, types, m->scale, m->n_scale, N, gz, st))) return rc;
    for (int i = nl - 1; i >= 0; --i) {
      float *ga = i == 0 ? g_x : A.f((size_t)N * d[i] + 64);
      if ((rc = snet_gemm(gz, m->fcn_wt[i], ga, N, 1, d[i + 1], d[i], d[i + 1], 0, d[i], 0, nullptr, 0, st))) return rc;
      if (i > 0 && (rc = snet_act_bwd(zs[i - 1], ga, ga, N * d[i], m->fcn_act, m->fcn_cst, st))) return rc;
      gz = ga;
    }
  } else {
    if ((rc = snet_readout_energy(x, N, m->ro1.dim_in, m->ro_v, m->ro_c, types, m->scale, m->shift, m->n_scale, ea, energy, st)))
      return rc;
    if ((rc = snet_readout_grad(m->ro_v, m->ro1.dim_in, types, m->scale, m->n_scale, N, g_x, st))) return rc;
  }
  SNET_REQUIRE(hipMemsetAsync(g_vec, 0, (size_t)E * 3 * 4, st) == hipSuccess &&
                   (all_tangent || hipMemsetAsync(g_emb, 0, (size_t)E * nb * 4, st) == hipSuccess),
               "snet_model_eval: memset failed");
  std::vector<float *> x_max_of((size_t)Lc, nullptr);
  if (E > 0 && m->fused_terms == 4) {
    const float *xs[8];
    float *outs[8];
    int64_t rows[8];
    int32_t dims[8];
    int nj = 0;
    for (int t = 0; t <= Lc; ++t) {
      if (t < Lc && m->layers[t].fused && !(t == 0 && l0 != nullptr) &&
          !(t == Lc - 1 && ll_on && m->layers[t].tfused && t > 0)) {
        x_max_of[t] = A.f((size_t)NT + 64);
        xs[nj] = saved[t].h; outs[nj] = x_max_of[t]; rows[nj] = NT; dims[nj] = m->layers[t].dx; ++nj;
      }
      if (nj == 8 || (t == Lc && nj > 0)) {
        if ((rc = snet_row_absmax_multi(xs, rows, dims, outs, nj, st))) return rc;
        nj = 0;
      }
    }
  }
  const size_t mark2 = A.off;
  for (int t = Lc - 1; t >= 0; --t) {
    Layer &L = m->layers[t];
    A.off = mark2;
    float *g_y = A.f((size_t)N * L.gin);
    const bool merged = t > 0 && t == Lc - 1 && ll_on && L.tfused != nullptr && E > 0;
    float *g_max = (L.fused && E > 0 && m->fused_terms == 4 && !(t == 0 && l0 != nullptr) && !merged) ? A.f((size_t)N) : nullptr;
    if ((rc = snet_gate_bwd_norm(saved[t].y, g_x, g_y, N, L.gin, L.dout, L.segs.data(), (int)L.segs.size(),
                                 g_max ? L.si2.t_norm : 0.f, g_max, st)))
      return rc;
    float *g_m = A.f((size_t)N * L.dmid);
    if ((rc = run_linear(m, L.si2, g_y, g_m, N, true, false, st))) return rc;
    const bool transposed = t > 0 && L.tfused != nullptr && E > 0;
    float *g_xe = t > 0 && !transposed ? A.f((size_t)E * L.dx) : nullptr;
    if (L.fused) {
      const bool tg = saved[t].wd != nullptr;
      const bool tail = tg || snet_fused_plan_has_mlp_tail(L.fused) != 0;
      float *g_h2 = tail ? nullptr : A.f((size_t)E * 64);
      float *x_max = x_max_of[t];
      auto bwd_tiles = [&](const int32_t *tp, const int32_t *tn, int64_t nt) -> int {
        if (E <= 0 || nt <= 0 || merged) return 0;
        if (tg)
          return snet_conv_bwd_fused_tangent(L.fused, saved[t].h, sh, dsh, saved[t].w, saved[t].wd, pairs ? w_row : nullptr, row_ptr, src,
                                             tp, tn, nt, L.conv_scale, g_m, g_xe, edge_vec, g_vec, x_max, g_max, st);
        return snet_conv_bwd_fused(L.fused, saved[t].h, sh, dsh, saved[t].w, pairs ? w_row : nullptr, row_ptr, src, tp, tn, nt,
                                   L.conv_scale, g_m, g_xe, g_h2, tail ? emb : nullptr, tail ? g_emb : nullptr, g_vec, x_max, g_max, st);
      };
      const bool rsplit = hsplit && t > 0;
      const bool packed = L.tile_mode != 0;
      auto bwd_all = [&]() -> int {
        if (t == 0 && l0 != nullptr)
          return snet_layer0_conv_bwd(l0->plan, g_m, saved[t].w, saved[t].wd, pairs ? w_row : nullptr, row_ptr, src, types, l0->slot, sh,
                                      dsh, edge_vec, N, A.f(l0_scratch), g_vec, st);
        return packed ? bwd_tiles(ptile_e0, ptile_nodes, pn_tiles) : bwd_tiles(tile_ptr, tile_node, n_tiles);
      };
      if (!rsplit && (rc = bwd_all())) return rc;
      if (t > 0) {
        float *g_h = A.f((size_t)NT * L.dx);
        auto gh_rows = [&](int64_t a, int64_t b) -> int {
          if (b <= a) return 0;
          if (merged)
            return snet_lastlayer_conv_bwd(L.merged, saved[t].h, g_m, sh, dsh, edge_vec, saved[t].w, saved[t].wd, col_ptr, center_t,
                                           w_row_t, eperm, a, b, L.conv_scale, g_h, g_vec, st);
          if (transposed)
            return snet_conv_fwd_fused(L.tfused, g_m, sh_t, saved[t].w, w_row_t, col_ptr + a, center_t, b - a, L.conv_scale,
                                       g_h + (size_t)a * L.dx, st);
          return snet_segment_sum_rows_chunked(g_xe, col_ptr + a, eperm, b - a, L.dx, L.gxe_chunks, g_h + (size_t)a * L.dx, st);
        };
        if (transposed && !merged)
          for (size_t i = 0; i + 1 < L.t_dead.size(); i += 2)
            SNET_REQUIRE(hipMemset2DAsync(g_h + L.t_dead[i], (size_t)L.dx * 4, 0, (size_t)L.t_dead[i + 1] * 4, (size_t)NT, st) ==
                             hipSuccess, "snet_model_eval: memset failed");
        if (rsplit) {
          if (!transposed && (rc = packed ? bwd_tiles(ptile_e0 + ptile_k, ptile_nodes + 2 * ptile_k, pn_tiles - ptile_k)
                                          : bwd_tiles(tile_ptr_b, tile_node + tile_k, n_tiles - tile_k))) return rc;
          if ((rc = gh_rows(N, NT))) return rc;
          SNET_REQUIRE(hipEventRecord(m->ev_h0, st) == hipSuccess && hipStreamWaitEvent(m->halo_stream, m->ev_h0, 0) == hipSuccess,
                       "snet_model_eval: stream ordering failed");
          if ((rc = snet_halo_reverse_exchange(m->halo_user, g_h, NT, N, L.dx, m->halo_stream))) return rc;
          SNET_REQUIRE(hipEventRecord(m->ev_h1, m->halo_stream) == hipSuccess, "snet_model_eval: stream ordering failed");
          if ((rc = transposed ? bwd_all() : packed ? bwd_tiles(ptile_e0, ptile_nodes, ptile_k) : bwd_tiles(tile_ptr, tile_node, tile_k))) return rc;
          if ((rc = gh_rows(0, N))) return rc;
          if (!tail && (rc = snet_radial_mlp_hidden_bwd(L.mlp_plan, emb, g_h2, E, g_emb, st))) return rc;
          if (L.sc.present())
            if ((rc = run_linear(m, L.sc, g_y, gx_next, N, true, false, st))) return rc;
          SNET_REQUIRE(hipStreamWaitEvent(st, m->ev_h1, 0) == hipSuccess, "snet_model_eval: stream ordering failed");
          if ((rc = snet_halo_reverse_accumulate(m->halo_user, g_h, L.dx, st))) return rc;
          if ((rc = run_linear(m, L.si1, g_h, gx_next, N, true, L.sc.present(), st))) return rc;
          std::swap(g_x, gx_next);
          continue;
        }
        if ((rc = gh_rows(0, NT))) return rc;
        if (has_halo)
          if ((rc = m->halo_rev(m->halo_user, g_h, NT, N, L.dx, stream))) {
            snet::set_error("snet_model_eval: reverse halo callback failed");
            return rc;
          }
        if (!tail && (rc = snet_radial_mlp_hidden_bwd(L.mlp_plan, emb, g_h2, E, g_emb, st))) return rc;
        if (L.sc.present())
          if ((rc = run_linear(m, L.sc, g_y, gx_next, N, true, false, st))) return rc;
        if ((rc = run_linear(m, L.si1, g_h, gx_next, N, true, L.sc.present(), st))) return rc;
        std::swap(g_x, gx_next);
        continue;
      }
      if (!tail && (rc = snet_radial_mlp_hidden_bwd(L.mlp_plan, emb, g_h2, E, g_emb, st))) return rc;
      break;
    }
    float *g_w = ov ? gw_buf[t & 1] : A.f((size_t)E * L.wn);
    if (ov && gw_busy[t & 1])
      SNET_REQUIRE(hipStreamWaitEvent(st, m->ev_bwd[t & 1], 0) == hipSuccess, "snet_model_eval: stream ordering failed");
    if ((rc = snet_conv_bwd_edge_vec(L.conv, saved[t].h, sh, dsh, saved[t].w, pairs ? w_row : nullptr, row_ptr, src, N,
                                     L.conv_scale, g_m, g_w,
                                     g_xe, g_vec, st)))
      return rc;
    if (ov) {
      SNET_REQUIRE(hipEventRecord(m->ev_main, st) == hipSuccess && hipStreamWaitEvent(m->side, m->ev_main, 0) == hipSuccess,
                   "snet_model_eval: stream ordering failed");
      if ((rc = snet_radial_mlp_bwd(L.mlp_plan, emb, g_w, E, g_emb, m->side))) return rc;
      SNET_REQUIRE(hipEventRecord(m->ev_bwd[t & 1], m->side) == hipSuccess, "snet_model_eval: stream ordering failed");
      gw_busy[t & 1] = true;
    } else if ((rc = snet_radial_mlp_bwd(L.mlp_plan, emb, g_w, E, g_emb, st))) {
      return rc;
    }
    if (t == 0) break;
    float *g_h = A.f((size_t)NT * L.dx);
    if ((rc = snet_segment_sum_rows(g_xe, col_ptr, eperm, NT, L.dx, g_h, st))) return rc;
    if (has_halo)
      if ((rc = m->halo_rev(m->halo_user, g_h, NT, N, L.dx, stream))) {
        snet::set_error("snet_model_eval: reverse halo callback failed");
        return rc;
      }
    if (L.sc.present())
      if ((rc = run_linear(m, L.sc, g_y, gx_next, N, true, false, st))) return rc;
    if ((rc = run_linear(m, L.si1, g_h, gx_next, N, true, L.sc.present(), st))) return rc;
    std::swap(g_x, gx_next);
  }
  for (int b = 0; b < 2; ++b)
    if (gw_busy[b])
      SNET_REQUIRE(hipStreamWaitEvent(st, m->ev_bwd[b], 0) == hipSuccess, "snet_model_eval: stream ordering failed");
  if (!all_tangent && (rc = snet_edge_embed_bwd(&ep, m->coeffs.data(), edge_vec, E, g_emb, nullptr, g_vec, 1, st))) return rc;
  A.off = mark2;
  float *F = forces ? forces : A.f((size_t)NT * 3);
  if ((rc = snet_edge_force(g_vec, edge_vec, row_ptr, col_ptr, eperm, NT, E, F, virial_atom, virial, st))) return rc;
  if (has_halo && m->fold_forces) {
    if ((rc = m->halo_rev(m->halo_user, F, NT, N, 3, stream))) return rc;
    if (virial_atom && (rc = m->halo_rev(m->halo_user, virial_atom, NT, N, 6, stream))) return rc;
  }
  return 0;
}
```

### sevennet_amd/engine.py

```python
from __future__ import annotations

import ctypes as C
from dataclasses import dataclass
from typing import Dict, List, Optional

import numpy as np
import torch

from . import _lib
from .model_spec import (ACT_CST, ACT_ID, LinearSpec, ModelSpec, build_model_spec, folded_readout, lastlayer_merged_eligible,
                         layer0_moments_eligible,                         linear_modal_bias, linear_weight_matrices, species_only_tables, transposed_scalar_conv)


def _ptr(t: Optional[torch.Tensor]):
    return None if t is None else C.c_void_p(t.data_ptr())


def _stream():
    return C.c_void_p(torch.cuda.current_stream().cuda_stream)


@dataclass
class Graph:
    n_total: int
    n_local: int
    n_edges: int
    types: torch.Tensor
    center: torch.Tensor
    src: torch.Tensor
    row_ptr: torch.Tensor
    col_ptr: torch.Tensor
    eperm: torch.Tensor
    edge_vec: torch.Tensor
    order: Optional[torch.Tensor] = None
    species_rows: Optional[List[torch.Tensor]] = None
    w_row: Optional[torch.Tensor] = None
    pair_edge: Optional[torch.Tensor] = None
    n_pairs: int = 0
    tile_ptr: Optional[torch.Tensor] = None
    tile_node: Optional[torch.Tensor] = None
    n_tiles: int = 0
    src_T: Optional[torch.Tensor] = None
    w_row_T: Optional[torch.Tensor] = None
    n_interior: int = 0
    _tile_split: Optional[tuple] = None
    _tiles_packed: Optional[tuple] = None
    seg_ptr: Optional[torch.Tensor] = None
    seg_ptr_host: Optional[np.ndarray] = None

    def by_source(self, lib, stream):
        if self.src_T is None:
            self.src_T, self.w_row_T = torch.empty_like(self.eperm), torch.empty_like(self.eperm)
            _lib.check(lib.snet_edges_by_source(_ptr(self.row_ptr), self.n_local, _ptr(self.eperm), _ptr(self.w_row),
                                                self.n_edges, _ptr(self.src_T), _ptr(self.w_row_T), stream),
                       'snet_edges_by_source')
        return self.src_T, self.w_row_T

    def _packed_tiles(self):
        lib = _lib.load()
        dev = self.edge_vec.device
        cut = self.n_interior if 0 < self.n_interior < self.n_local else 0
        with torch.cuda.device(dev):
            cap = self.n_local + self.n_edges // 16 + 2
            tp = torch.empty(cap + 1, dtype=torch.int32, device=dev)
            tn = torch.empty(2 * cap, dtype=torch.int32, device=dev)
            k = 0
            n = C.c_int64()
            if cut:
                _lib.check(lib.snet_edge_tiles_packed(_ptr(self.row_ptr), 0, cut, _ptr(tp), _ptr(tn), cap, C.byref(n), _stream()),
                           'snet_edge_tiles_packed')
                k = int(n.value)
            _lib.check(lib.snet_edge_tiles_packed(_ptr(self.row_ptr), cut, self.n_local, C.c_void_p(tp.data_ptr() + 4 * k),
                                                  C.c_void_p(tn.data_ptr() + 8 * k), cap - k, C.byref(n), _stream()),
                       'snet_edge_tiles_packed')
        return tp, tn, k + int(n.value), k

    def tiles(self, mode: int = 0):
        if mode == 1:
            if self._tiles_packed is None:
                self._tiles_packed = self._packed_tiles()
            return self._tiles_packed[:3]
        if self.tile_ptr is None:
            lib = _lib.load()
            dev = self.edge_vec.device
            with torch.cuda.device(dev):
                tp = torch.empty(self.n_local + 1, dtype=torch.int32, device=dev)
                cap = self.n_local + self.n_edges // 16 + 1
                tn = torch.empty(cap, dtype=torch.int32, device=dev)
                n = C.c_int64()
                _lib.check(lib.snet_edge_tiles(_ptr(self.row_ptr), self.n_local, _ptr(tp), _ptr(tn), cap, C.byref(n),
                                               _stream()), 'snet_edge_tiles')
            self.tile_ptr, self.tile_node, self.n_tiles = tp, tn, int(n.value)
        return self.tile_ptr, self.tile_node, self.n_tiles

    def tiles_split(self, mode: int = 0):
        if mode == 1:
            tp, tn, nt = self.tiles(1)
            k = self._tiles_packed[3]
            return (tp, tn, k), (tp[k:], tn[2 * k:], nt - k)
        if self._tile_split is None:
            tp, tn, nt = self.tiles()
            k = int(tp[self.n_interior].item())
            self._tile_split = ((tp, tn, k), ((tp - k).contiguous(), tn[k:], nt - k))
        return self._tile_split

    def share_pairs(self):
        lib = _lib.load()
        E = self.n_edges
        if E == 0:
            return self
        dev = self.edge_vec.device
        with torch.cuda.device(dev):
            w_row = torch.empty(E, dtype=torch.int32, device=dev)
            pair_edge = torch.empty(E, dtype=torch.int32, device=dev)
            n = C.c_int64()
            _lib.check(lib.snet_edge_pairs(_ptr(self.row_ptr), _ptr(self.src), _ptr(self.edge_vec), self.n_local, E,
                                           _ptr(w_row), _ptr(pair_edge), C.byref(n), _stream()), 'snet_edge_pairs')
        self.w_row, self.pair_edge, self.n_pairs = w_row, pair_edge[:n.value].contiguous(), int(n.value)
        return self


def species_row_lists(types_local: torch.Tensor, num_species: int) -> List[torch.Tensor]:
    t = types_local.long()
    order = torch.sort(t, stable=True).indices.to(torch.int32)
    counts = torch.bincount(t, minlength=num_species).cpu().tolist()
    rows, o = [], 0
    for s in range(num_species):
        rows.append(order[o:o + counts[s]])
        o += counts[s]
    return rows


def build_graph(types, edge_index, edge_vec, n_local: Optional[int] = None, device='cuda',
                num_species: int = 0, share_pairs: bool = True, n_interior: int = 0) -> Graph:
    dev = torch.device(device)
    types = torch.as_tensor(types).to(dev, torch.int32)
    ei = torch.as_tensor(edge_index).to(dev, torch.int64)
    ev = torch.as_tensor(edge_vec).to(dev, torch.float32)
    n_total = int(types.shape[0])
    n_local = n_total if n_local is None else int(n_local)
    E = int(ei.shape[1])
    order = None
    if E > 1 and bool((ei[0, 1:] < ei[0, :-1]).any()):
        order = torch.sort(ei[0], stable=True).indices
        ei = ei[:, order]
        ev = ev[order]
    center, src = ei[0], ei[1]
    if E and (int(center.max()) >= n_local):
        raise ValueError('edge centers must be owned (local) atoms')
    row_ptr = torch.zeros(n_total + 1, dtype=torch.int64, device=dev)
    col_ptr = torch.zeros(n_total + 1, dtype=torch.int64, device=dev)
    if E:
        row_ptr[1:] = torch.cumsum(torch.bincount(center, minlength=n_total), 0)
        col_ptr[1:] = torch.cumsum(torch.bincount(src, minlength=n_total), 0)
        eperm = torch.sort(src, stable=True).indices
    else:
        eperm = torch.zeros(0, dtype=torch.int64, device=dev)
    rows = None
    if num_species:
        rows = species_row_lists(types[:n_local], num_species)
    g = Graph(n_total, n_local, E, types, center.to(torch.int32).contiguous(), src.to(torch.int32).contiguous(),
              row_ptr.to(torch.int32), col_ptr.to(torch.int32), eperm.to(torch.int32).contiguous(),
              ev.contiguous(), order, rows)
    g.n_interior = int(n_interior) if 0 < int(n_interior) < n_local else 0
    return g.share_pairs() if share_pairs and dev.type == 'cuda' else g


def _pack_split(m: np.ndarray, dev) -> torch.Tensor:
    lib = _lib.load()
    m = np.ascontiguousarray(m, dtype=np.float32)
    K, N = m.shape
    buf = np.empty(int(lib.snet_gemm_split_size(K, N)), np.uint8)
    _lib.check(lib.snet_gemm_split_pack(C.c_void_p(m.ctypes.data), K, N, C.c_void_p(buf.ctypes.data)),
               'snet_gemm_split_pack')
    return torch.from_numpy(buf).to(dev)


class _Linear:

    def __init__(self, spec: LinearSpec, flat: np.ndarray, dev, split: bool = True, modal_idx: int = -1, bias_flat=None):
        self.spec = spec
        self.split = split
        b = linear_modal_bias(spec, flat, modal_idx, bias_flat)
        self.bias = None if b is None else torch.from_numpy(b).to(dev)
        mats = linear_weight_matrices(spec, flat)
        if split:
            self.w = [_pack_split(m, dev) for m in mats]
            self.wt = [_pack_split(np.ascontiguousarray(m.T), dev) for m in mats]
        else:
            self.w = [torch.from_numpy(m).to(dev) for m in mats]
            self.wt = [torch.from_numpy(np.ascontiguousarray(m.T)).to(dev) for m in mats]
        fed = {b.in_off for b in spec.blocks}
        self.zero_in = [(off, m * (2 * l + 1)) for off, (m, l, _) in zip(spec.irreps_in.offsets(), spec.irreps_in) if off not in fed]
        self.groups_fwd = self._plan(transpose=False)
        self.groups_T = self._plan(transpose=True)
        acc = {}
        for b, m in zip(spec.blocks, mats):
            acc[(b.in_off, b.species)] = acc.get((b.in_off, b.species), 0.0) + (np.asarray(m, np.float32).astype(np.float64) ** 2).sum(1)
        self.t_norm = float(max(np.sqrt(v).max() for v in acc.values())) if acc else 0.0

    def _plan(self, transpose: bool):
        sp = self.spec
        groups = []
        written = set()
        pair_seen = {}
        for b, w, wt in zip(sp.blocks, self.w, self.wt):
            if transpose:
                tgt, a_off, c_off, K, N, B = b.in_off, b.out_off, b.in_off, b.mul_out, b.mul_in, wt
            else:
                tgt, a_off, c_off, K, N, B = b.out_off, b.in_off, b.out_off, b.mul_in, b.mul_out, w
            key = (tgt, b.species)
            acc = key in written
            desc = _lib.GemmDesc(None if self.split else B.data_ptr(), B.data_ptr() if self.split else None, a_off, c_off,
                                 2 * b.l + 1, K, N, int(acc))
            placed = False
            if groups and groups[-1][0] == b.species and len(groups[-1][1]) < 8 and tgt not in groups[-1][2]:
                groups[-1][1].append(desc)
                groups[-1][2].add(tgt)
                placed = True
            if not placed:
                groups.append([b.species, [desc], {tgt}])
            written.add(key)
        out = []
        for species, descs, _ in groups:
            arr = (_lib.GemmDesc * len(descs))(*descs)
            out.append((species, arr, len(descs)))
        return out


class _Span:

    def __init__(self, eng, name):
        self.eng, self.name = eng, name

    def __enter__(self):
        self.on = self.eng.events is not None and (self.eng.event_filter is None or self.name in self.eng.event_filter)
        if self.on:
            self.a = torch.cuda.Event(enable_timing=True)
            self.b = torch.cuda.Event(enable_timing=True)
            self.a.record()

    def __exit__(self, *exc):
        if self.on:
            self.b.record()
            self.eng.events.append((self.name, self.a, self.b))


class HipForceEngine:
    OVERLAP_MAX_EDGES = 1_000_000

    def __init__(self, config: dict, state_dict: Dict[str, np.ndarray], device='cuda:0', mlp_mode: str = 'bf16x6',
                 linear_mode: str = 'bf16x6', fused='auto', fused_terms='f16x3', modal=None, overlap: bool = True,
                 mlp_tail: bool = True, transposed_conv: bool = True, species_tables: bool = True,
                 fold_readout: bool = True, tangent: bool = True, layer0_moments: bool = True,
                 last_layer_merged: bool = True):
        self.fused_terms, self.fused_mode = self._check_modes(mlp_mode, linear_mode, fused, fused_terms)
        self.mlp_mode = mlp_mode
        self.linear_mode = linear_mode
        self.overlap, self.halo_split = bool(overlap), True
        self._side = None
        self._acc_descs = {}
        self.events = None
        self.event_filter = None
        self.lib = _lib.load()
        if not torch.cuda.is_available():
            raise RuntimeError('HipForceEngine needs a ROCm GPU (no CPU fallback exists)')
        self.dev = torch.device(device)
        self.spec: ModelSpec = build_model_spec(config)
        sp = self.spec
        self.modal_idx = mi = sp.modal_index(modal)
        shapes = sp.param_shapes()
        sd = {}
        for k, shp in shapes.items():
            if k not in state_dict:
                raise KeyError(f'state_dict is missing {k}')
            v = state_dict[k]
            v = v.detach().cpu().numpy() if isinstance(v, torch.Tensor) else np.asarray(v)
            if k.startswith('rescale_atomic_energy.'):
                sd[k] = v.astype(np.float64)
                continue
            if v.size != int(np.prod(shp)):
                raise ValueError(f'{k}: checkpoint tensor has {v.size} entries, the model config implies {shp}')
            sd[k] = v.astype(np.float64).reshape(shp)

        self.edge_params = _lib.EdgeParams(sp.cutoff, sp.n_basis, sp.cutoff_kind, sp.cutoff_p, sp.cutoff_on,
                                           sp.lmax_edge, int(sp.normalize_sph))
        self.coeffs = (C.c_float * sp.n_basis)(*[float(v) for v in sd['edge_embedding.basis_function.coeffs']])
        self.nsh = sp.irreps_sh.dim
        with torch.cuda.device(self.dev):
            emb = linear_weight_matrices(sp.embed, sd[sp.embed.name])
            assert len(emb) == 1
            eb = linear_modal_bias(sp.embed, sd[sp.embed.name], mi, sd.get(sp.embed.bias_name))
            table = emb[0] if eb is None else emb[0] + eb[None, :]
            self.embed_table = torch.from_numpy(np.ascontiguousarray(table, np.float32)).to(self.dev)
            self.layers = []
            split = linear_mode == 'bf16x6'
            for ls in sp.layers:
                L = type('L', (), {})()
                L.spec = ls
                L.sc = _Linear(ls.sc, sd[ls.sc.name], self.dev, split, mi) if ls.sc is not None else None
                L.si1 = _Linear(ls.si1, sd[ls.si1.name], self.dev, split, mi, sd.get(ls.si1.bias_name))
                L.si2 = _Linear(ls.si2, sd[ls.si2.name], self.dev, split, mi, sd.get(ls.si2.bias_name))
                L.mlp_w, L.mlp_wt = [], []
                rw = ls.radial_weights(sd)
                for i in range(len(ls.mlp_dims) - 1):
                    w = rw[i] / np.sqrt(ls.mlp_dims[i])
                    L.mlp_w.append(torch.from_numpy(np.ascontiguousarray(w, dtype=np.float32)).to(self.dev))
                    L.mlp_wt.append(torch.from_numpy(np.ascontiguousarray(w.T, dtype=np.float32)).to(self.dev))
                L.fused_mlp = (len(ls.mlp_dims) == 4 and ls.mlp_dims[1] == 64 and ls.mlp_dims[2] == 64
                               and ls.mlp_dims[0] <= 32)
                L.mlp_plan = None
                if L.fused_mlp:
                    d = ls.mlp_dims
                    hw = [np.ascontiguousarray(rw[i] / np.sqrt(d[i]), dtype=np.float32) for i in range(3)]
                    fp = [w.ctypes.data_as(C.POINTER(C.c_float)) for w in hw]
                    mp = C.c_void_p()
                    _lib.check(self.lib.snet_radial_mlp_plan_create(d[0], d[1], d[2], d[3], fp[0], fp[1], fp[2],
                                                                    ACT_ID[sp.act_radial], ACT_CST[sp.act_radial],
                                                                    1 if mlp_mode == 'bf16x6' else 0, C.byref(mp)),
                               'snet_radial_mlp_plan_create')
                    L.mlp_plan, L.w2_host = mp, hw[2]
                L.scale = 1.0 / float(sd[f'{ls.t}_convolution.denominator'][0])
                if ls.conv.tag not in _lib.compiled_conv_tags():
                    from .jit import ensure_conv_shape
                    ensure_conv_shape(ls.conv)
                plan = C.c_void_p()
                _lib.check(self.lib.snet_conv_plan_create(ls.conv.tag.encode(), C.byref(plan)), 'snet_conv_plan_create')
                L.plan = plan
                L.fplan = None
                L.mlp_tail = False
                can = bool(L.fused_mlp and mlp_mode == 'bf16x6' and self.lib.snet_conv_fused_available(plan))
                if fused is True and not can:
                    raise RuntimeError(f'layer {ls.t}: no fused tensor-product kernels for this shape / mlp_mode')
                if fused is not False and can:
                    fpl = C.c_void_p()
                    _lib.check(self.lib.snet_fused_plan_create(plan, L.mlp_plan, self.fused_terms, C.byref(fpl)),
                               'snet_fused_plan_create')
                    L.fplan = fpl
                    L.mlp_tail = bool(self.lib.snet_fused_plan_has_mlp_tail(fpl)) and mlp_tail
                    nch = ls.si1.dim_out // 16
                    cp = (C.c_int32 * nch)()
                    _lib.check(self.lib.snet_fused_plan_gxe_chunks(fpl, cp, nch), 'snet_fused_plan_gxe_chunks')
                    L.gxe_chunks = torch.tensor(list(cp), dtype=torch.int32, device=self.dev)
                L.fused_fwd = L.fplan is not None and fused in ('auto', True, 'fwd')
                L.fused_bwd = L.fplan is not None and fused in ('auto', True, 'bwd')
                L.tile_mode = int(self.lib.snet_fused_plan_tile_mode(L.fplan)) if L.fplan is not None else 0
                L.tangent = bool(L.fused_bwd and tangent and self.lib.snet_fused_plan_prefers_tangent(L.fplan))
                L.tplan = None
                tr = transposed_scalar_conv(ls.conv) if (L.fused_bwd and transposed_conv and ls.t > 0) else None
                if tr is not None and ls.conv.irreps_out.dim < ls.conv.irreps_x.dim:
                    spec_t, kappa = tr
                    if spec_t.tag not in _lib.compiled_conv_tags():
                        from .jit import ensure_conv_shape
                        ensure_conv_shape(spec_t)
                    ttag, col = C.create_string_buffer(13), np.empty(ls.conv.weight_numel, np.float32)
                    dead, nd = (C.c_int32 * 32)(), C.c_int32()
                    _lib.check(self.lib.snet_conv_plan_transposed(plan, ttag, col.ctypes.data_as(C.c_void_p), C.cast(dead, C.c_void_p),
                                                                  32, C.byref(nd)), 'snet_conv_plan_transposed')
                    assert ttag.value.decode() == spec_t.tag, (ttag.value, spec_t.tag)
                    w2t = np.ascontiguousarray(np.asarray(hw[2], np.float32) * col[None, :], dtype=np.float32)
                    tpl, tmlp, tfp = C.c_void_p(), C.c_void_p(), C.c_void_p()
                    _lib.check(self.lib.snet_conv_plan_create(spec_t.tag.encode(), C.byref(tpl)), 'snet_conv_plan_create')
                    _lib.check(self.lib.snet_radial_mlp_plan_create(d[0], d[1], d[2], d[3], fp[0], fp[1],
                                                                    w2t.ctypes.data_as(C.POINTER(C.c_float)),
                                                                    ACT_ID[sp.act_radial], ACT_CST[sp.act_radial], 1, C.byref(tmlp)),
                               'snet_radial_mlp_plan_create')
                    _lib.check(self.lib.snet_fused_plan_create(tpl, tmlp, self.fused_terms, C.byref(tfp)), 'snet_fused_plan_create')
                    L.tplan, L.tmlp, L.tconv = tfp, tmlp, tpl
                    L.t_dead = [(dead[2 * i], dead[2 * i + 1]) for i in range(nd.value)]
                self._init_last_layer(L, len(sp.layers), last_layer_merged)
                segs = (_lib.GateSeg * len(ls.gate.segs))()
                inv_act = {v: k for k, v in ACT_ID.items()}
                for i, s in enumerate(ls.gate.segs):
                    segs[i] = _lib.GateSeg(s.kind, s.in_off, s.out_off, s.mul, s.l, s.gate_off, s.act,
                                           ACT_CST[inv_act[s.act]])
                L.gate_segs = segs
                self.layers.append(L)
            self.h0_table = self.sc0_table = None
            if species_tables:
                h0, sc0 = species_only_tables(sp, sd, mi)
                self.h0_table = torch.from_numpy(h0).to(self.dev)
                self.sc0_table = None if sc0 is None else torch.from_numpy(sc0).to(self.dev)
            self.ro_v = self.ro_fcn = None
            if sp.readout_fcn_dims:
                d = sp.readout_fcn_dims
                ws = [np.ascontiguousarray(sd[f'readout_FCN.fcn.layer{i}.weight'] / np.sqrt(d[i]), dtype=np.float32) for i in range(len(d) - 1)]
                self.ro_fcn = type('F', (), {})()
                self.ro_fcn.dims = d
                self.ro_fcn.w = [torch.from_numpy(w).to(self.dev) for w in ws]
                self.ro_fcn.wt = [torch.from_numpy(np.ascontiguousarray(w.T)).to(self.dev) for w in ws]
                self.ro_fcn.act, self.ro_fcn.cst = ACT_ID[sp.readout_fcn_act], ACT_CST[sp.readout_fcn_act]
            else:
                if fold_readout:
                    v, self.ro_c = folded_readout(sp, sd, mi)
                    self.ro_v = torch.from_numpy(v).to(self.dev)
                self.ro1 = _Linear(sp.readout1, sd[sp.readout1.name], self.dev, split, mi, sd.get(sp.readout1.bias_name))
                self.ro2 = _Linear(sp.readout2, sd[sp.readout2.name], self.dev, split, mi, sd.get(sp.readout2.bias_name))
            sc_v, sh_v = sp.rescale_vectors(sd, mi)
            self.n_scale = len(sc_v)
            self.scale = torch.tensor(sc_v, dtype=torch.float32, device=self.dev)
            self.shift = torch.tensor(sh_v, dtype=torch.float32, device=self.dev)
            self.scale0 = float(sc_v[0])
        self.act_radial = ACT_ID[sp.act_radial]
        self.act_cst = ACT_CST[sp.act_radial]
        self.needs_species_rows = any(ls.sc is not None and ls.sc.n_species for ls in sp.layers)
        self._init_layer0(layer0_moments)

    @staticmethod
    def _check_modes(mlp_mode, linear_mode, fused, fused_terms):
        if mlp_mode not in ('bf16x6', 'fp32') or linear_mode not in ('bf16x6', 'fp32'):
            raise ValueError("mlp_mode / linear_mode must be 'bf16x6' or 'fp32'")
        if fused not in ('auto', True, False, 'fwd', 'bwd'):
            raise ValueError("fused must be 'auto', True, False, 'fwd' or 'bwd'")
        codes = {'bf16': 1, 'bf16x3': 2, 'bf16x6': 3, 'f16x3': 4}
        if fused_terms not in codes and fused_terms not in codes.values():
            raise ValueError(f"fused_terms must be one of {sorted(codes)} (or the C-ABI code 1..4)")
        code = int(codes.get(fused_terms, fused_terms))
        return code, {v: k for k, v in codes.items()}[code]

    def __del__(self):
        try:
            for pl, _, _ in (getattr(self, 'l0_plans', None) or {}).values():
                self.lib.snet_layer0_plan_destroy(pl)
            for L in getattr(self, 'layers', []):
                if getattr(L, 'fplan', None) is not None:
                    self.lib.snet_fused_plan_destroy(L.fplan)
                if getattr(L, 'tplan', None) is not None:
                    self.lib.snet_fused_plan_destroy(L.tplan)
                    self.lib.snet_conv_plan_destroy(L.tconv)
                    self.lib.snet_radial_mlp_plan_destroy(L.tmlp)
                if getattr(L, 'mplan', None) is not None:
                    self.lib.snet_lastlayer_plan_destroy(L.mplan)
                self.lib.snet_conv_plan_destroy(L.plan)
                if getattr(L, 'mlp_plan', None) is not None:
                    self.lib.snet_radial_mlp_plan_destroy(L.mlp_plan)
        except Exception:
            pass

    def kernel_times_ms(self) -> Dict[str, List[float]]:
        out: Dict[str, List[float]] = {}
        for name, a, b in self.events or []:
            out.setdefault(name, []).append(a.elapsed_time(b))
        return out

    def _new(self, *shape):
        return torch.empty(*shape, dtype=torch.float32, device=self.dev)

    def _gemm(self, A, B, Cm, n_nodes, d, K, N, a_stride, a_off, c_stride, c_off, rows=None, acc=False):
        _lib.check(self.lib.snet_gemm(_ptr(A), _ptr(B), _ptr(Cm), n_nodes, d, K, N, a_stride, a_off, c_stride,
                                      c_off, _ptr(rows), int(acc), _stream()), 'snet_gemm')

    def _run_groups(self, groups, A, Cm, n, a_stride, c_stride, g: Graph, force_acc=False):
        for species, arr, cnt in groups:
            rows, m = None, n
            if species >= 0:
                rows = g.species_rows[species]
                m = rows.numel()
                if m == 0:
                    continue
            if force_acc:
                arr2 = self._acc_descs.get(id(arr))
                if arr2 is None:
                    arr2 = (_lib.GemmDesc * cnt)(*[_lib.GemmDesc(d.B, d.B_split, d.a_off, d.c_off, d.d, d.K, d.N, 1) for d in arr[:cnt]])
                    self._acc_descs[id(arr)] = arr2
                arr = arr2
            _lib.check(self.lib.snet_gemm_grouped(arr, cnt, _ptr(A), _ptr(Cm), m, a_stride, c_stride, _ptr(rows),
                                                  _stream()), 'snet_gemm_grouped')

    def _linear(self, lin: _Linear, x, n, g: Graph, out=None, accumulate=False):
        sp = lin.spec
        y = self._new(max(n, 0), sp.dim_out) if out is None else out
        if not accumulate:
            for off, ln in sp.zero_out:
                y[:, off:off + ln].zero_()
        self._run_groups(lin.groups_fwd, x, y, n, sp.dim_in, sp.dim_out, g, force_acc=accumulate)
        if lin.bias is not None and n > 0:
            _lib.check(self.lib.snet_add_row_bias(_ptr(y), _ptr(lin.bias), n, sp.dim_out, _stream()), 'snet_add_row_bias')
        return y

    def _linear_T(self, lin: _Linear, gy, n, g: Graph, out=None, accumulate=False):
        sp = lin.spec
        gx = out if out is not None else self._new(max(n, 0), sp.dim_in)
        if not accumulate:
            fed = {b.in_off for b in sp.blocks}
            for off, (m, l, _) in zip(sp.irreps_in.offsets(), sp.irreps_in):
                if off not in fed:
                    gx[:, off:off + m * (2 * l + 1)].zero_()
        self._run_groups(lin.groups_T, gy, gx, n, sp.dim_out, sp.dim_in, g, force_acc=accumulate)
        return gx

    def _mlp_fwd(self, L, emb, E, out=None):
        dims = L.spec.mlp_dims
        if L.fused_mlp:
            w = self._new(E, dims[3]) if out is None else out
            _lib.check(self.lib.snet_radial_mlp_fwd(L.mlp_plan, _ptr(emb), E, _ptr(w), _stream()), 'snet_radial_mlp_fwd')
            return w, None
        zs, a = [], emb
        for i, wm in enumerate(L.mlp_w):
            z = self._new(E, dims[i + 1])
            self._gemm(a, wm, z, E, 1, dims[i], dims[i + 1], dims[i], 0, dims[i + 1], 0)
            if i + 1 < len(L.mlp_w):
                zs.append(z)
                a = self._new(E, dims[i + 1])
                _lib.check(self.lib.snet_act_fwd(_ptr(z), _ptr(a), z.numel(), self.act_radial, self.act_cst,
                                                 _stream()), 'snet_act_fwd')
                zs.append(a)
            else:
                return z, zs

    def _mlp_bwd(self, L, emb, zs, g_w, g_emb_total, E):
        dims = L.spec.mlp_dims
        if L.fused_mlp:
            _lib.check(self.lib.snet_radial_mlp_bwd(L.mlp_plan, _ptr(emb), _ptr(g_w), E, _ptr(g_emb_total), _stream()),
                       'snet_radial_mlp_bwd')
            return
        g = g_w
        nl = len(L.mlp_w)
        for i in range(nl - 1, -1, -1):
            if i == 0:
                self._gemm(g, L.mlp_wt[0], g_emb_total, E, 1, dims[1], dims[0], dims[1], 0, dims[0], 0, None, True)
            else:
                ga = self._new(E, dims[i])
                self._gemm(g, L.mlp_wt[i], ga, E, 1, dims[i + 1], dims[i], dims[i + 1], 0, dims[i], 0)
                z = zs[2 * (i - 1)]
                _lib.check(self.lib.snet_act_bwd(_ptr(z), _ptr(ga), _ptr(ga), z.numel(), self.act_radial,
                                                 self.act_cst, _stream()), 'snet_act_bwd')
                g = ga

    def _init_last_layer(self, L, n_layers, last_layer_merged):
        ls = L.spec
        L.mplan = None
        if (last_layer_merged and L.tplan is not None and ls.t == n_layers - 1 and L.fused_fwd and self.fused_terms == 4
                and lastlayer_merged_eligible(ls.conv, ls.mlp_dims)):
            mpl = C.c_void_p()
            _lib.check(self.lib.snet_lastlayer_plan_create(L.plan, L.w2_host.ctypes.data_as(C.c_void_p), C.byref(mpl)),
                       'snet_lastlayer_plan_create')
            L.mplan, L.tangent = mpl, True

    def _init_layer0(self, layer0_moments):
        L0 = self.layers[0]
        self.l0_plans = None
        if (layer0_moments and self.h0_table is not None and L0.fused_fwd and L0.fused_bwd
                and layer0_moments_eligible(L0.spec.conv, L0.spec.mlp_dims)):
            self.l0_plans, self.h0_host = {}, self.h0_table.cpu().numpy()

    def _layer0_plan(self, g: Graph):
        if self.l0_plans is None or g.n_edges == 0:
            return None
        ns = self.h0_host.shape[0]
        present = tuple(range(ns)) if ns <= 4 else getattr(g, '_species_present', None)
        if present is None:
            present = g._species_present = tuple(int(v) for v in torch.unique(g.types).cpu())
        if not 1 <= len(present) <= 4 or present[0] < 0 or present[-1] >= ns:
            return None
        if present not in self.l0_plans:
            L0, plan = self.layers[0], C.c_void_p()
            table = np.ascontiguousarray(self.h0_host[list(present)], np.float32)
            _lib.check(self.lib.snet_layer0_plan_create(L0.plan, C.c_void_p(L0.w2_host.ctypes.data), C.c_void_p(table.ctypes.data),
                                                        L0.scale, len(present), C.byref(plan)), 'snet_layer0_plan_create')
            slot = np.zeros(ns, np.int32)
            slot[list(present)] = np.arange(len(present), dtype=np.int32)
            self.l0_plans[present] = (plan, torch.from_numpy(slot).to(self.dev), len(present))
        return self.l0_plans[present]

    def _layer0_bwd(self, c, g_m, h2, h2d, g_vec):
        g, (plan, slot, _) = c.g, c.l0
        scratch = self._new(int(self.lib.snet_layer0_scratch_size(plan, c.N)))
        with _Span(self, 'conv_bwd_l0'):
            _lib.check(self.lib.snet_layer0_conv_bwd(plan, _ptr(g_m), _ptr(h2), _ptr(h2d), _ptr(c.w_row), _ptr(g.row_ptr), _ptr(g.src),
                                                     _ptr(g.types), _ptr(slot), _ptr(c.sh), _ptr(c.dsh), _ptr(g.edge_vec), c.N,
                                                     _ptr(scratch), _ptr(g_vec), c.st), 'snet_layer0_conv_bwd')

    def compute(self, g: Graph, halo=None, want_atomic_virial: bool = False, keep: bool = False):
        lib, sp = self.lib, self.spec
        if self.needs_species_rows and g.species_rows is None:
            raise ValueError('graph was built without num_species but the model has a per-species self-connection')
        if g.seg_ptr is not None and (halo is not None or g.n_total != g.n_local):
            raise ValueError('a batch of systems (Graph.seg_ptr) cannot be combined with a halo decomposition')
        with torch.cuda.device(self.dev):
            c = self._begin(g, halo, keep)
            x = self._forward_layers(c)
            e_atom, energy, g_x = self._readout(c, x)
            g_vec = self._reverse_layers(c, g_x)
            return self._forces(c, g_vec, e_atom, energy, want_atomic_virial)

    def _begin(self, g: Graph, halo, keep: bool):
        from types import SimpleNamespace
        lib, sp = self.lib, self.spec
        st = _stream()
        N, NT, E = g.n_local, g.n_total, g.n_edges
        nb, nsh = sp.n_basis, self.nsh
        inter = {}
        emb, sh, dsh = self._new(E, nb), self._new(E, nsh), self._new(E, nsh * 3)
        with _Span(self, 'edge_embed_fwd'):
            _lib.check(lib.snet_edge_embed_fwd(C.byref(self.edge_params), self.coeffs, _ptr(g.edge_vec), E,
                                               _ptr(emb), _ptr(sh), _ptr(dsh), st), 'snet_edge_embed_fwd')
        pairs = g.w_row is not None and all(L.fused_mlp for L in self.layers)
        w_row = g.w_row if pairs else None
        if pairs:
            emb_p = self._new(g.n_pairs, nb)
            _lib.check(lib.snet_gather_rows(_ptr(emb), _ptr(g.pair_edge), _ptr(emb_p), g.n_pairs, nb, st),
                       'snet_gather_rows')
        side = None
        w_ready = {}
        any_fused = any(L.fused_fwd or L.fused_bwd for L in self.layers)
        l0 = self._layer0_plan(g)
        if E > 0:
            for L in self.layers:
                if L.fused_bwd:
                    g.tiles(L.tile_mode)
        if self.overlap and E <= self.OVERLAP_MAX_EDGES and not any_fused and all(L.fused_mlp for L in self.layers):
            if self._side is None:
                self._side = torch.cuda.Stream(device=self.dev)
            side = self._side
            main = torch.cuda.current_stream()
            rows_w = g.n_pairs if pairs else E
            w_bufs = [self._new(rows_w, L_.spec.conv.weight_numel) for L_ in self.layers]
            wn_max = max(L_.spec.conv.weight_numel for L_ in self.layers)
            gw_bufs = [self._new(E * wn_max), self._new(E * wn_max)]
            gw_done = [None, None]
            side.wait_stream(main)
            with torch.cuda.stream(side):
                for t_, L_ in enumerate(self.layers):
                    with _Span(self, f'radial_mlp_fwd[wn={L_.spec.conv.weight_numel}]@side'):
                        self._mlp_fwd(L_, emb_p if pairs else emb, rows_w, out=w_bufs[t_])
                    ev = torch.cuda.Event()
                    ev.record(side)
                    w_ready[t_] = (w_bufs[t_], ev)
        d0 = sp.embed.dim_out
        x = None
        if keep or self.h0_table is None:
            x = self._new(NT, d0)
            _lib.check(lib.snet_embed_rows(_ptr(self.embed_table), _ptr(g.types), _ptr(x), NT, d0, st),
                       'snet_embed_rows')
        if keep:
            inter['edge_embedding'], inter['edge_attr'], inter['x_embed'] = emb, sh, x[:N]
        saved = []
        split = bool(halo is not None and g.n_interior and hasattr(halo, 'forward_start') and hasattr(halo, 'reverse_start')
                     and E > 0 and self.halo_split)
        h2_rows = g.n_pairs if pairs else E
        h2_of = {t_: self._new(h2_rows, 64) for t_, L_ in enumerate(self.layers) if L_.fused_fwd or L_.fused_bwd}
        h2d_of = {t_: self._new(h2_rows, 64) for t_, L_ in enumerate(self.layers) if L_.tangent or (t_ == 0 and l0 is not None)}
        with _Span(self, 'radial_mlp_hidden_fwd'):
            demb = None
            if h2d_of:
                demb = self._new(h2_rows, nb)
                _lib.check(lib.snet_edge_embed_tangent(C.byref(self.edge_params), self.coeffs, _ptr(g.edge_vec),
                                                       _ptr(g.pair_edge) if pairs else None, h2_rows, _ptr(demb), st), 'snet_edge_embed_tangent')
            for tg_, ts in ((True, sorted(h2d_of)), (False, sorted(set(h2_of) - set(h2d_of)))):
                for i in range(0, len(ts), 8):
                    grp = ts[i:i + 8]
                    plans = (C.c_void_p * len(grp))(*[self.layers[t_].mlp_plan for t_ in grp])
                    outs = (C.c_void_p * len(grp))(*[h2_of[t_].data_ptr() for t_ in grp])
                    if tg_:
                        outs_d = (C.c_void_p * len(grp))(*[h2d_of[t_].data_ptr() for t_ in grp])
                        _lib.check(lib.snet_radial_mlp_hidden_fwd_layers_tangent(plans, len(grp), _ptr(emb_p if pairs else emb), _ptr(demb),
                                                                                 h2_rows, outs, outs_d, st),
                                   'snet_radial_mlp_hidden_fwd_layers_tangent')
                    else:
                        _lib.check(lib.snet_radial_mlp_hidden_fwd_layers(plans, len(grp), _ptr(emb_p if pairs else emb), h2_rows, outs, st),
                                   'snet_radial_mlp_hidden_fwd_layers')
        return SimpleNamespace(g=g, halo=halo, keep=keep, st=st, N=N, NT=NT, E=E, nb=nb, nsh=nsh, inter=inter, emb=emb, sh=sh, dsh=dsh,
                               pairs=pairs, w_row=w_row, emb_p=emb_p if pairs else None, side=side, w_ready=w_ready,
                               gw_bufs=gw_bufs if side is not None else None, gw_done=gw_done if side is not None else None,
                               x=x, saved=saved, split=split, h2_of=h2_of, h2d_of=h2d_of, l0=l0)

    def _forward_layers(self, c):
        lib, g, halo, keep, st, inter = self.lib, c.g, c.halo, c.keep, c.st, c.inter
        N, NT, E = c.N, c.NT, c.E
        emb, sh, pairs, emb_p, w_row, side, w_ready = c.emb, c.sh, c.pairs, c.emb_p, c.w_row, c.side, c.w_ready
        x, saved, split, h2_of = c.x, c.saved, c.split, c.h2_of
        for t, L in enumerate(self.layers):
            ls = L.spec
            n_in = NT if t == 0 else N
            with _Span(self, 'node_linear_fwd'):
                h = self._new(NT, ls.si1.dim_out)
                if t == 0 and self.h0_table is not None:
                    _lib.check(lib.snet_embed_rows(_ptr(self.h0_table), _ptr(g.types), _ptr(h), NT, ls.si1.dim_out, st),
                               'snet_embed_rows')
                else:
                    self._linear(L.si1, x, n_in, g, out=h)
            pending = None
            if t > 0 and halo is not None:
                with _Span(self, 'halo_fwd'):
                    if hasattr(halo, 'forward_start'):
                        pending = halo.forward_start(h, N)
                    else:
                        halo.forward(h, N)
            with _Span(self, 'node_linear_fwd'):
                if t == 0 and self.h0_table is not None:
                    sc = None
                    if self.sc0_table is not None:
                        sc = self._new(N, ls.gate.irreps_in.dim)
                        _lib.check(lib.snet_embed_rows(_ptr(self.sc0_table), _ptr(g.types), _ptr(sc), N, ls.gate.irreps_in.dim,
                                                       st), 'snet_embed_rows')
                else:
                    sc = self._linear(L.sc, x, N, g) if L.sc is not None else None
            dmid = ls.conv.irreps_out.dim
            m = self._new(N, dmid)
            if E == 0:
                m.zero_()
            else:
                for off, ln in L.si2.zero_in:
                    m[:, off:off + ln].zero_()
            h2 = w = zs = None
            rows_w = g.n_pairs if pairs else E
            h2 = h2_of.pop(t, None)
            if not (L.fused_fwd and L.fused_bwd):
                if side is not None:
                    (w, ev), zs = w_ready.pop(t), None
                    torch.cuda.current_stream().wait_event(ev)
                else:
                    with _Span(self, f'radial_mlp_fwd[wn={ls.conv.weight_numel}]'):
                        w, zs = self._mlp_fwd(L, emb_p, g.n_pairs) if pairs else self._mlp_fwd(L, emb, E)
            def conv_rows(a, b):
                if b <= a:
                    return
                rp, mo = C.c_void_p(g.row_ptr.data_ptr() + 4 * a), C.c_void_p(m.data_ptr() + 4 * a * dmid)
                if L.fused_fwd:
                    with _Span(self, f'conv_fwd_fused[{ls.conv.tag}]'):
                        _lib.check(lib.snet_conv_fwd_fused(L.fplan, _ptr(h), _ptr(sh), _ptr(h2), _ptr(w_row), rp,
                                                           _ptr(g.src), b - a, L.scale, mo, st), 'snet_conv_fwd_fused')
                else:
                    with _Span(self, f'conv_fwd[{ls.conv.tag}]'):
                        _lib.check(lib.snet_conv_fwd(L.plan, _ptr(h), _ptr(sh), _ptr(w), _ptr(w_row), rp,
                                                     _ptr(g.src), b - a, L.scale, mo, st), 'snet_conv_fwd')
            n_int = g.n_interior if (pending is not None and split) else 0
            conv_rows(0, n_int)
            if pending is not None:
                with _Span(self, 'halo_fwd'):
                    halo.forward_finish(pending)
            conv_rows(n_int, N)
            if L.fused_bwd:
                w = None
            with _Span(self, 'node_linear_fwd'):
                y = self._linear(L.si2, m, N, g) if sc is None else self._linear(L.si2, m, N, g, out=sc, accumulate=True)
            xo = self._new(N, ls.gate.irreps_out.dim)
            with _Span(self, 'gate_fwd'):
                _lib.check(lib.snet_gate_fwd(_ptr(y), None, _ptr(xo), N, ls.gate.irreps_in.dim,
                                             ls.gate.irreps_out.dim, L.gate_segs, len(ls.gate.segs), st), 'snet_gate_fwd')
            saved.append((h, w, zs, y, h2))
            if keep:
                inter[f'{t}_si1'], inter[f'{t}_conv'], inter[f'{t}_gate_in'], inter[f'{t}_x'] = h[:N], m, y, xo
            x = xo
        return x

    def _readout(self, c, x):
        lib, sp, g, st, N = self.lib, self.spec, c.g, c.st, c.N
        e_atom = self._new(N)
        energy = torch.empty(1, dtype=torch.float64, device=self.dev)
        c.e_sys = None if g.seg_ptr is None else torch.empty(len(g.seg_ptr_host) - 1, dtype=torch.float64, device=self.dev)
        d_ro = sp.readout1.dim_in
        if self.ro_fcn is not None:
            F = self.ro_fcn
            d, nl = F.dims, len(F.w)
            zs, a = [], x
            for i in range(nl):
                z = self._new(N, d[i + 1])
                self._gemm(a, F.w[i], z, N, 1, d[i], d[i + 1], d[i], 0, d[i + 1], 0)
                if i + 1 < nl:
                    a = self._new(N, d[i + 1])
                    _lib.check(lib.snet_act_fwd(_ptr(z), _ptr(a), z.numel(), F.act, F.cst, st), 'snet_act_fwd')
                    zs.append(z)
            self._rescale_reduce(c, z, e_atom, energy)
            gz = self._new(N, 1)
            if self.n_scale > 1:
                _lib.check(lib.snet_embed_rows(_ptr(self.scale), _ptr(g.types), _ptr(gz), N, 1, st), 'snet_embed_rows')
            else:
                gz.fill_(self.scale0)
            for i in range(nl - 1, -1, -1):
                ga = self._new(N, d[i])
                self._gemm(gz, F.wt[i], ga, N, 1, d[i + 1], d[i], d[i + 1], 0, d[i], 0)
                if i > 0:
                    _lib.check(lib.snet_act_bwd(_ptr(zs[i - 1]), _ptr(ga), _ptr(ga), ga.numel(), F.act, F.cst, st), 'snet_act_bwd')
                gz = ga
            g_x = gz
        elif self.ro_v is not None:
            if c.e_sys is None:
                _lib.check(lib.snet_readout_energy(_ptr(x), N, d_ro, _ptr(self.ro_v), self.ro_c, _ptr(g.types), _ptr(self.scale),
                                                   _ptr(self.shift), self.n_scale, _ptr(e_atom), _ptr(energy), st), 'snet_readout_energy')
            else:
                _lib.check(lib.snet_readout_energy_seg(_ptr(x), N, d_ro, _ptr(self.ro_v), self.ro_c, _ptr(g.types), _ptr(self.scale),
                                                       _ptr(self.shift), self.n_scale, _ptr(g.seg_ptr), c.e_sys.numel(), _ptr(e_atom),
                                                       _ptr(c.e_sys), _ptr(energy), st), 'snet_readout_energy_seg')
            g_x = self._new(N, d_ro)
            _lib.check(lib.snet_readout_grad(_ptr(self.ro_v), d_ro, _ptr(g.types), _ptr(self.scale), self.n_scale, N, _ptr(g_x),
                                             st), 'snet_readout_grad')
        else:
            h1 = self._linear(self.ro1, x, N, g)
            e_sc = self._linear(self.ro2, h1, N, g)
            self._rescale_reduce(c, e_sc, e_atom, energy)
            g_e = self._new(N, 1)
            if self.n_scale > 1:
                _lib.check(lib.snet_embed_rows(_ptr(self.scale), _ptr(g.types), _ptr(g_e), N, 1, st), 'snet_embed_rows')
            else:
                g_e.fill_(self.scale0)
            g_h1 = self._linear_T(self.ro2, g_e, N, g)
            g_x = self._linear_T(self.ro1, g_h1, N, g)
        return e_atom, energy, g_x

    def _rescale_reduce(self, c, e_sc, e_atom, energy):
        lib, g, st, N = self.lib, c.g, c.st, c.N
        if c.e_sys is None:
            _lib.check(lib.snet_rescale_reduce(_ptr(e_sc), _ptr(g.types), _ptr(self.scale), _ptr(self.shift),
                                               self.n_scale, N, _ptr(e_atom), _ptr(energy), st), 'snet_rescale_reduce')
        else:
            _lib.check(lib.snet_rescale_reduce_seg(_ptr(e_sc), _ptr(g.types), _ptr(self.scale), _ptr(self.shift), self.n_scale, N,
                                                   _ptr(g.seg_ptr), c.e_sys.numel(), _ptr(e_atom), _ptr(c.e_sys), _ptr(energy), st),
                       'snet_rescale_reduce_seg')

    def _reverse_layers(self, c, g_x):
        lib, g, halo, st = self.lib, c.g, c.halo, c.st
        N, NT, E, nb, nsh = c.N, c.NT, c.E, c.nb, c.nsh
        emb, sh, dsh, w_row, side, gw_bufs, gw_done = c.emb, c.sh, c.dsh, c.w_row, c.side, c.gw_bufs, c.gw_done
        saved, split = c.saved, c.split
        sh_T = None
        g_vec = torch.zeros(E, 3, dtype=torch.float32, device=self.dev)
        need_g_emb = any(not (L_.tangent or (t_ == 0 and c.l0 is not None)) for t_, L_ in enumerate(self.layers))
        g_emb = torch.zeros(E, nb, dtype=torch.float32, device=self.dev) if need_g_emb else None
        x_max_of = {}
        if self.fused_terms == 4 and E > 0:
            ts = [t_ for t_, L_ in enumerate(self.layers)
                  if L_.fused_bwd and not (t_ == 0 and c.l0 is not None) and L_.mplan is None]
            for t_ in ts:
                x_max_of[t_] = self._new(NT)
            with _Span(self, 'row_bounds'):
                for i in range(0, len(ts), 8):
                    grp = ts[i:i + 8]
                    k = len(grp)
                    _lib.check(lib.snet_row_absmax_multi((C.c_void_p * k)(*[saved[t_][0].data_ptr() for t_ in grp]), (C.c_int64 * k)(*[NT] * k),
                                                         (C.c_int32 * k)(*[self.layers[t_].spec.si1.dim_out for t_ in grp]),
                                                         (C.c_void_p * k)(*[x_max_of[t_].data_ptr() for t_ in grp]), k, st),
                               'snet_row_absmax_multi')
        for t in range(len(self.layers) - 1, -1, -1):
            L = self.layers[t]
            ls = L.spec
            h, w, zs, y, h2 = saved[t]
            l0 = c.l0 if t == 0 else None
            tangent = L.tangent or l0 is not None
            g_y = self._new(N, ls.gate.irreps_in.dim)
            g_max = self._new(N) if (L.fused_bwd and self.fused_terms == 4 and E > 0 and l0 is None and L.mplan is None) else None
            with _Span(self, 'gate_bwd'):
                _lib.check(lib.snet_gate_bwd_norm(_ptr(y), _ptr(g_x), _ptr(g_y), N, ls.gate.irreps_in.dim, ls.gate.irreps_out.dim,
                                                  L.gate_segs, len(ls.gate.segs), L.si2.t_norm if g_max is not None else 0.0,
                                                  _ptr(g_max), st), 'snet_gate_bwd_norm')
            with _Span(self, 'node_linear_bwd'):
                g_m = self._linear_T(L.si2, g_y, N, g)
            use_t = t > 0 and getattr(L, 'tplan', None) is not None and E > 0
            use_m = use_t and L.mplan is not None
            g_xe = self._new(E, ls.si1.dim_out) if (t > 0 and not use_t) else None
            g_w = g_h2 = None
            rsplit = split and t > 0 and L.fused_bwd
            pending = None
            g_h = self._new(NT, ls.si1.dim_out) if t > 0 else None
            if use_t:
                src_t, w_row_t = g.by_source(lib, st)
                if L.t_dead and not use_m:
                    g_h.zero_()
                if sh_T is None and not use_m:
                    sh_T = self._new(E, nsh)
                    _lib.check(lib.snet_gather_rows(_ptr(sh), _ptr(g.eperm), _ptr(sh_T), E, nsh, st), 'snet_gather_rows')

            def gh_rows(a, b):
                if b <= a:
                    return
                cp, go = C.c_void_p(g.col_ptr.data_ptr() + 4 * a), C.c_void_p(g_h.data_ptr() + 4 * a * ls.si1.dim_out)
                if use_m:
                    with _Span(self, f'conv_bwd_merged[{ls.conv.tag}]'):
                        _lib.check(lib.snet_lastlayer_conv_bwd(L.mplan, _ptr(h), _ptr(g_m), _ptr(sh), _ptr(dsh), _ptr(g.edge_vec), _ptr(h2),
                                                               _ptr(h2d), _ptr(g.col_ptr), _ptr(src_t), _ptr(w_row_t), _ptr(g.eperm), a, b,
                                                               L.scale, _ptr(g_h), _ptr(g_vec), st), 'snet_lastlayer_conv_bwd')
                    return
                if use_t:
                    with _Span(self, f'conv_bwd_node[transposed {ls.conv.tag}]'):
                        _lib.check(lib.snet_conv_fwd_fused(L.tplan, _ptr(g_m), _ptr(sh_T), _ptr(h2), _ptr(w_row_t), cp, _ptr(src_t),
                                                           b - a, L.scale, go, st), 'snet_conv_fwd_fused')
                    return
                with _Span(self, 'conv_bwd_node[segment_sum]'):
                    if L.fused_bwd:
                        _lib.check(lib.snet_segment_sum_rows_chunked(_ptr(g_xe), cp, _ptr(g.eperm), b - a, ls.si1.dim_out,
                                                                     _ptr(L.gxe_chunks), go, st), 'snet_segment_sum_rows_chunked')
                    else:
                        _lib.check(lib.snet_segment_sum_rows(_ptr(g_xe), cp, _ptr(g.eperm), b - a, ls.si1.dim_out, go, st),
                                   'snet_segment_sum_rows')

            if L.fused_bwd:
                g_h2 = None if (L.mlp_tail or tangent) else self._new(E, 64)
                x_max = x_max_of.pop(t, None)
                h2d = c.h2d_of.pop(t, None)

                def bwd_tiles(tp_, tn_, nt_):
                    if nt_ <= 0 or use_m:
                        return
                    with _Span(self, f'conv_bwd_fused[{ls.conv.tag}]'):
                        if tangent:
                            _lib.check(lib.snet_conv_bwd_fused_tangent(L.fplan, _ptr(h), _ptr(sh), _ptr(dsh), _ptr(h2), _ptr(h2d), _ptr(w_row),
                                                                       _ptr(g.row_ptr), _ptr(g.src), _ptr(tp_), _ptr(tn_), nt_, L.scale,
                                                                       _ptr(g_m), _ptr(g_xe), _ptr(g.edge_vec), _ptr(g_vec), _ptr(x_max),
                                                                       _ptr(g_max), st), 'snet_conv_bwd_fused_tangent')
                            return
                        _lib.check(lib.snet_conv_bwd_fused(L.fplan, _ptr(h), _ptr(sh), _ptr(dsh), _ptr(h2), _ptr(w_row),
                                                           _ptr(g.row_ptr), _ptr(g.src), _ptr(tp_), _ptr(tn_), nt_, L.scale,
                                                           _ptr(g_m), _ptr(g_xe), _ptr(g_h2),
                                                           _ptr(emb) if L.mlp_tail else None, _ptr(g_emb) if L.mlp_tail else None,
                                                           _ptr(g_vec), _ptr(x_max), _ptr(g_max), st),
                                   'snet_conv_bwd_fused')
                if rsplit:
                    (tpi, tni, nti), (tpb, tnb, ntb) = g.tiles_split(L.tile_mode)
                    if use_t:
                        gh_rows(N, NT)
                    else:
                        bwd_tiles(tpb, tnb, ntb)
                        gh_rows(N, NT)
                    with _Span(self, 'halo_rev'):
                        pending = halo.reverse_start(g_h, N)
                    if use_t:
                        bwd_tiles(*g.tiles(L.tile_mode))
                    else:
                        bwd_tiles(tpi, tni, nti)
                    gh_rows(0, N)
                elif l0 is not None:
                    self._layer0_bwd(c, g_m, h2, h2d, g_vec)
                elif E > 0:
                    bwd_tiles(*g.tiles(L.tile_mode))
            else:
                if side is not None:
                    if gw_done[t & 1] is not None:
                        torch.cuda.current_stream().wait_event(gw_done[t & 1])
                    g_w = gw_bufs[t & 1][:E * ls.conv.weight_numel].view(E, ls.conv.weight_numel)
                else:
                    g_w = self._new(E, ls.conv.weight_numel)
                with _Span(self, f'conv_bwd_edge[{ls.conv.tag}]'):
                    _lib.check(lib.snet_conv_bwd_edge_vec(L.plan, _ptr(h), _ptr(sh), _ptr(dsh), _ptr(w), _ptr(w_row),
                                                          _ptr(g.row_ptr), _ptr(g.src), N, L.scale, _ptr(g_m), _ptr(g_w),
                                                          _ptr(g_xe), _ptr(g_vec), st), 'snet_conv_bwd_edge_vec')
            if t > 0 and not rsplit:
                gh_rows(0, NT)
                if halo is not None:
                    with _Span(self, 'halo_rev'):
                        if hasattr(halo, 'reverse_start'):
                            pending = halo.reverse_start(g_h, N)
                        else:
                            halo.reverse(g_h, N)
            del g_xe
            if L.fused_bwd and (L.mlp_tail or tangent):
                pass
            elif L.fused_bwd:
                with _Span(self, 'radial_mlp_hidden_bwd'):
                    _lib.check(lib.snet_radial_mlp_hidden_bwd(L.mlp_plan, _ptr(emb), _ptr(g_h2), E, _ptr(g_emb), st),
                               'snet_radial_mlp_hidden_bwd')
            elif side is not None:
                side.wait_stream(torch.cuda.current_stream())
                with torch.cuda.stream(side):
                    with _Span(self, f'radial_mlp_bwd[wn={ls.conv.weight_numel}]@side'):
                        self._mlp_bwd(L, emb, zs, g_w, g_emb, E)
                    gw_done[t & 1] = torch.cuda.Event()
                    gw_done[t & 1].record(side)
            else:
                with _Span(self, f'radial_mlp_bwd[wn={ls.conv.weight_numel}]'):
                    self._mlp_bwd(L, emb, zs, g_w, g_emb, E)
            del g_w, g_h2
            if t == 0:
                break
            with _Span(self, 'node_linear_bwd'):
                g_x = self._linear_T(L.sc, g_y, N, g) if L.sc is not None else None
            if pending is not None:
                with _Span(self, 'halo_rev'):
                    halo.reverse_finish(pending, g_h)
            with _Span(self, 'node_linear_bwd'):
                g_x = self._linear_T(L.si1, g_h, N, g, out=g_x, accumulate=g_x is not None)
            saved[t] = None
        if side is not None:
            torch.cuda.current_stream().wait_stream(side)
        if g_emb is not None:
            _lib.check(lib.snet_edge_embed_bwd(C.byref(self.edge_params), self.coeffs, _ptr(g.edge_vec), E, _ptr(g_emb),
                                               None, _ptr(g_vec), 1, st), 'snet_edge_embed_bwd')
        return g_vec

    def _forces(self, c, g_vec, e_atom, energy, want_atomic_virial: bool):
        lib, g, halo, st, N, NT, E = self.lib, c.g, c.halo, c.st, c.N, c.NT, c.E
        keep, inter = c.keep, c.inter
        forces = self._new(NT, 3)
        vir_atom = self._new(NT, 6) if want_atomic_virial else None
        virial = torch.empty(6, dtype=torch.float64, device=self.dev)
        vir_sys = None
        if c.e_sys is None:
            _lib.check(lib.snet_edge_force(_ptr(g_vec), _ptr(g.edge_vec), _ptr(g.row_ptr), _ptr(g.col_ptr),
                                           _ptr(g.eperm), NT, E, _ptr(forces), _ptr(vir_atom), _ptr(virial), st),
                       'snet_edge_force')
        else:
            vir_sys = torch.empty(c.e_sys.numel(), 6, dtype=torch.float64, device=self.dev)
            _lib.check(lib.snet_edge_force_seg(_ptr(g_vec), _ptr(g.edge_vec), _ptr(g.row_ptr), _ptr(g.col_ptr), _ptr(g.eperm), NT, E,
                                               _ptr(g.seg_ptr), c.e_sys.numel(), _ptr(forces), _ptr(vir_atom), _ptr(vir_sys),
                                               _ptr(virial), st), 'snet_edge_force_seg')
        if halo is not None:
            with _Span(self, 'halo_rev'):
                if vir_atom is None:
                    halo.reverse(forces, N)
                else:
                    fv = torch.cat([forces, vir_atom], 1).contiguous()
                    halo.reverse(fv, N)
                    forces, vir_atom = fv[:, :3].contiguous(), fv[:, 3:].contiguous()
        if g.order is not None:
            tmp = torch.empty_like(g_vec)
            tmp[g.order] = g_vec
            g_vec = tmp
        out = dict(energy=energy, atomic_energy=e_atom, dE_dr=g_vec, forces=forces[:N], virial=virial)
        if vir_atom is not None:
            out['atomic_virial'] = vir_atom[:N]
        if vir_sys is not None:
            out['energy_per_system'], out['virial_per_system'] = c.e_sys, vir_sys
        if keep:
            out['inter'] = inter
        return out
```

### sevennet_amd/model_spec.py

```python
from __future__ import annotations

import hashlib
import math
from dataclasses import dataclass, field
from typing import Dict, List, Optional, Tuple

import numpy as np

from .irreps import Irreps, infer_irreps_out

ACT_ID = {'silu': 0, 'tanh': 1, 'relu': 2, 'abs': 3, 'ssp': 4, 'sigmoid': 5, 'elu': 6}
ACT_CST = {'silu': 1.6791767923989418, 'tanh': 1.5937334472592695, 'relu': 1.4163393446331367, 'abs': 1.001110600838467,
           'ssp': 1.878204668541552, 'sigmoid': 1.8467055342154763, 'elu': 1.2467863885570512}

DEFAULT_CONFIG = dict(
    cutoff=4.5, channel=32, irreps_manual=False, lmax=1, lmax_edge=-1, lmax_node=-1,
    is_parity=True, num_convolution_layer=3,
    radial_basis={'radial_basis_name': 'bessel'},
    cutoff_function={'cutoff_function_name': 'poly_cut'},
    act_radial='silu', act_scalar={'e': 'silu', 'o': 'tanh'}, act_gate={'e': 'silu', 'o': 'tanh'},
    weight_nn_hidden_neurons=[64, 64], conv_denominator=1.0, self_connection_type='nequip',
    _normalize_sph=True, shift=0.0, scale=1.0, version='0.12.0', use_bias_in_linear=False,
    readout_as_fcn=False, readout_fcn_hidden_neurons=[30, 30], readout_fcn_activation='relu',
)


@dataclass
class GemmBlock:
    l: int
    in_off: int
    mul_in: int
    out_off: int
    mul_out: int
    w_off: int
    alpha: float
    accumulate: bool
    species: int = -1


@dataclass
class LinearSpec:
    name: str
    irreps_in: Irreps
    irreps_out: Irreps
    blocks: List[GemmBlock]
    zero_out: List[Tuple[int, int]]
    n_species: int = 0
    numel: int = 0
    n_modal: int = 0
    modal_bias: List[Tuple[int, int, int, float]] = field(default_factory=list)
    bias_blocks: List[Tuple[int, int, int]] = field(default_factory=list)

    @property
    def bias_name(self) -> str:
        return self.name[:-len('weight')] + 'bias'

    @property
    def n_bias(self) -> int:
        return sum(m for _, m, _ in self.bias_blocks)

    @property
    def dim_in(self):
        return self.irreps_in.dim

    @property
    def dim_out(self):
        return self.irreps_out.dim


def make_linear(name: str, irreps_in: Irreps, irreps_out: Irreps, n_species: int = 0, n_modal: int = 0,
                biases: bool = False) -> LinearSpec:
    assert not (n_species and n_modal)
    ns = max(n_species, 1)
    in_off, out_off = irreps_in.offsets(), irreps_out.offsets()
    pairs = [(i, j) for i, (_, li, pi) in enumerate(irreps_in)
             for j, (_, lj, pj) in enumerate(irreps_out) if (li, pi) == (lj, pj)]
    fan = [0] * len(irreps_out)
    for i, j in pairs:
        fan[j] += irreps_in[i][0] * ns
    modal_j = [j for j, (_, l, p) in enumerate(irreps_out) if (l, p) == (0, 1)] if n_modal else []
    for j in modal_j:
        fan[j] += n_modal
    blocks, seen, w_off = [], set(), 0
    for i, j in pairs:
        mi, l, _ = irreps_in[i]
        mo = irreps_out[j][0]
        for s in range(ns):
            blocks.append(GemmBlock(l, in_off[i], mi, out_off[j], mo, w_off, 1.0 / math.sqrt(fan[j]),
                                    accumulate=(j in seen), species=(s if n_species else -1)))
        seen.add(j)
        w_off += mi * ns * mo
    modal_bias = []
    for j in modal_j:
        mo = irreps_out[j][0]
        modal_bias.append((out_off[j], mo, w_off, 1.0 / math.sqrt(fan[j])))
        seen.add(j)
        w_off += n_modal * mo
    zero = [(out_off[j], irreps_out[j][0] * (2 * irreps_out[j][1] + 1))
            for j in range(len(irreps_out)) if j not in seen]
    bias_blocks, b_off = [], 0
    if biases:
        for j, (mo, l, p) in enumerate(irreps_out):
            if (l, p) == (0, 1):
                bias_blocks.append((out_off[j], mo, b_off))
                b_off += mo
    return LinearSpec(name, irreps_in, irreps_out, blocks, zero, n_species, w_off, n_modal, modal_bias, bias_blocks)


def linear_modal_bias(spec: LinearSpec, flat: np.ndarray, modal_idx: int, bias_flat=None, dtype=np.float32):
    if not spec.n_modal and not spec.bias_blocks:
        return None
    bias = np.zeros(spec.dim_out, np.float64)
    if spec.n_modal:
        flat = np.asarray(flat, dtype=np.float64).reshape(-1)
        for off, mo, w_off, alpha in spec.modal_bias:
            bias[off:off + mo] = flat[w_off:w_off + spec.n_modal * mo].reshape(spec.n_modal, mo)[modal_idx] * alpha
    if spec.bias_blocks:
        if bias_flat is None:
            raise KeyError(f'state_dict is missing {spec.bias_name}')
        b = np.asarray(bias_flat, dtype=np.float64).reshape(-1)
        assert b.size == spec.n_bias, (spec.bias_name, b.size, spec.n_bias)
        for off, mo, b_off in spec.bias_blocks:
            bias[off:off + mo] += b[b_off:b_off + mo]
    return bias.astype(dtype)


def linear_weight_matrices(spec: LinearSpec, flat: np.ndarray):
    flat = np.asarray(flat, dtype=np.float64).reshape(-1)
    assert flat.size == spec.numel, (spec.name, flat.size, spec.numel)
    ns = max(spec.n_species, 1)
    out = []
    for b in spec.blocks:
        w = flat[b.w_off:b.w_off + b.mul_in * ns * b.mul_out]
        if spec.n_species:
            w = w.reshape(b.mul_in, ns, b.mul_out)[:, b.species, :]
        else:
            w = w.reshape(b.mul_in, b.mul_out)
        out.append(np.ascontiguousarray(w * b.alpha, dtype=np.float32))
    return out


def linear_rows_fp64(spec: LinearSpec, flat: np.ndarray, x: np.ndarray, species=None, modal_idx: int = -1, bias_flat=None) -> np.ndarray:
    flat = np.asarray(flat, dtype=np.float64).reshape(-1)
    x = np.asarray(x, dtype=np.float64)
    ns = max(spec.n_species, 1)
    y = np.zeros((x.shape[0], spec.dim_out), np.float64)
    for b in spec.blocks:
        w = flat[b.w_off:b.w_off + b.mul_in * ns * b.mul_out]
        w = (w.reshape(b.mul_in, ns, b.mul_out)[:, b.species, :] if spec.n_species else w.reshape(b.mul_in, b.mul_out)) * b.alpha
        rows = slice(None) if b.species < 0 else np.nonzero(np.asarray(species) == b.species)[0]
        for m in range(2 * b.l + 1):
            y[rows, b.out_off + m * b.mul_out:b.out_off + (m + 1) * b.mul_out] += \
                x[rows, b.in_off + m * b.mul_in:b.in_off + (m + 1) * b.mul_in] @ w
    b = linear_modal_bias(spec, flat, modal_idx, bias_flat, dtype=np.float64)
    if b is not None:
        y += b[None, :]
    return y


def species_only_tables(sp: 'ModelSpec', sd, modal_idx: int):
    ls = sp.layers[0]
    e64 = linear_rows_fp64(sp.embed, sd[sp.embed.name], np.eye(sp.num_species), None, modal_idx, sd.get(sp.embed.bias_name))
    species = np.arange(sp.num_species)
    h0 = linear_rows_fp64(ls.si1, sd[ls.si1.name], e64, species, modal_idx, sd.get(ls.si1.bias_name))
    sc0 = linear_rows_fp64(ls.sc, sd[ls.sc.name], e64, species, modal_idx) if ls.sc is not None else None
    return h0.astype(np.float32), (None if sc0 is None else sc0.astype(np.float32))


def folded_readout(sp: 'ModelSpec', sd, modal_idx: int):
    d = sp.readout1.dim_in

    def chain(x):
        return linear_rows_fp64(sp.readout2, sd[sp.readout2.name],
                                linear_rows_fp64(sp.readout1, sd[sp.readout1.name], x, None, modal_idx, sd.get(sp.readout1.bias_name)),
                                None, -1, sd.get(sp.readout2.bias_name))

    c = chain(np.zeros((1, d)))[0, 0]
    v = chain(np.eye(d))[:, 0] - c
    return np.ascontiguousarray(v, np.float64), float(c)


@dataclass
class ConvPath:
    i_x: int
    i_sh: int
    l1: int
    l2: int
    l3: int
    mul: int
    w_off: int
    x_off: int
    sh_off: int
    out_off: int
    out_mul: int
    out_ch: int


@dataclass
class ConvSpec:
    irreps_x: Irreps
    irreps_sh: Irreps
    irreps_mid: Irreps
    irreps_out: Irreps
    paths: List[ConvPath]
    weight_numel: int

    @property
    def key(self) -> str:
        ps = ';'.join(f'{p.i_x},{p.i_sh},{p.l3},{p.w_off},{p.out_off},{p.out_mul},{p.out_ch}' for p in self.paths)
        return f'x={self.irreps_x}|sh={self.irreps_sh}|{ps}'

    @property
    def tag(self) -> str:
        return hashlib.sha1(self.key.encode()).hexdigest()[:12]


def layer0_moments_eligible(conv: ConvSpec, mlp_dims) -> bool:
    from .irreps import cg_nonzeros
    if len(conv.irreps_x) != 1 or conv.irreps_x[0][1] != 0:
        return False
    mul = conv.irreps_x[0][0]
    if mul % 16 or not 16 <= mul <= 512 or len(mlp_dims) != 4 or tuple(mlp_dims[1:3]) != (64, 64):
        return False
    lmax = len(conv.paths) - 1
    if not 0 <= lmax <= 3 or conv.irreps_sh.dim != (lmax + 1) ** 2 or conv.weight_numel != (lmax + 1) * mul or mlp_dims[3] != conv.weight_numel:
        return False
    for l, p in enumerate(conv.paths):
        if (p.l1, p.l2, p.l3, p.mul, p.out_mul, p.out_ch) != (0, l, l, mul, mul, 0):
            return False
        if (p.w_off, p.x_off, p.sh_off, p.out_off) != (l * mul, 0, l * l, l * l * mul):
            return False
        terms = sorted((a, b, c, v * math.sqrt(2 * l + 1)) for a, b, c, v in cg_nonzeros(0, l, l))
        if [(a, b, c) for a, b, c, _ in terms] != [(0, m, m) for m in range(2 * l + 1)] or any(abs(v - 1.0) > 1e-12 for *_, v in terms):
            return False
    return conv.irreps_out.dim == (lmax + 1) ** 2 * mul


def transposed_scalar_conv(conv: ConvSpec):
    from .codegen import _path_terms
    if not conv.paths or any(p.l3 != 0 for p in conv.paths):
        return None
    x_off = conv.irreps_x.offsets()
    order = sorted(range(len(conv.paths)), key=lambda k: (conv.paths[k].out_off, conv.paths[k].out_ch))
    if len({conv.paths[k].i_x for k in order}) != len(order):
        return None
    irreps_g = Irreps([(conv.paths[k].mul, 0, 1) for k in order])
    g_index = {k: i for i, k in enumerate(order)}
    g_off = irreps_g.offsets()
    if irreps_g.dim != conv.irreps_out.dim or any(g_off[g_index[k]] != p.out_off + p.out_ch for k, p in enumerate(conv.paths)):
        return None
    paths, kappa = [], []
    for k, p in enumerate(conv.paths):
        mul, l, par = conv.irreps_x[p.i_x]
        q = ConvPath(g_index[k], p.i_sh, 0, p.l2, l, p.mul, p.w_off, g_off[g_index[k]], p.sh_off, x_off[p.i_x], mul, 0)
        fwd = {(a, b): v for a, b, c, v in _path_terms(p)}
        tr = {(c, b): v for a, b, c, v in _path_terms(q)}
        if set(fwd) != set(tr):
            return None
        r = [fwd[key] / tr[key] for key in fwd]
        if max(r) - min(r) > 1e-12 * max(abs(v) for v in r):
            return None
        kappa.append(float(r[0]))
        paths.append(q)
    spec = ConvSpec(irreps_g, conv.irreps_sh, Irreps(conv.irreps_x), Irreps(conv.irreps_x), paths, conv.weight_numel)
    return spec, kappa


LASTLAYER_TILES = ((1, 1), (1, 1, 1), (8, 4, 2), (8, 4, 2, 2))
LASTLAYER_LDS_BUDGET = 80 * 1024


def lastlayer_merged_eligible(conv: ConvSpec, mlp_dims) -> bool:
    from .codegen import _path_terms
    tr = transposed_scalar_conv(conv)
    if tr is None or len(mlp_dims) != 4 or tuple(mlp_dims[1:3]) != (64, 64) or mlp_dims[3] != conv.weight_numel:
        return False
    lmax = len(conv.paths) - 1
    if not 0 <= lmax <= 3 or conv.irreps_sh.dim != (lmax + 1) ** 2:
        return False
    x_offs, col, prev_x, live = conv.irreps_x.offsets(), 0, -1, 0
    for l, (p, q, kappa) in enumerate(zip(conv.paths, tr[0].paths, tr[1])):
        mul, lx, _ = conv.irreps_x[p.i_x]
        if (p.l1, p.l2, p.l3, lx) != (l, l, 0, l) or p.mul != mul or mul % 16 or p.sh_off != l * l:
            return False
        if p.w_off != col or p.out_off + p.out_ch != col or p.x_off != x_offs[p.i_x] or x_offs[p.i_x] <= prev_x:
            return False
        terms = sorted(_path_terms(q))
        if [(a, b, c) for a, b, c, _ in terms] != [(0, m, m) for m in range(2 * l + 1)] or any(abs(v - 1.0) > 1e-12 for *_, v in terms):
            return False
        if abs(kappa - 1.0 / math.sqrt(2 * l + 1)) > 1e-9:
            return False
        prev_x, col, live = x_offs[p.i_x], col + mul, live + (2 * l + 1) * mul
# ... 361 lines not shown
```

Measured before the change: 2.913 million atom-steps/s.

## Fuse two-source node linears into one multi-source split GEMM launch

Adds a multi-source grouped GEMM kernel that accumulates two linears (si2 and self-connection forward, sc^T and si1^T backward) into one output tile in a single launch. An optional per-type table is added in the epilogue for the first layer. This removes the separate accumulate pass, in which the output was written, re-read and rewritten, and it cuts kernel launches. The cost is more complex planning code and a fallback path, and the second source uses a separate accumulator, which raises register pressure.

```diff
diff --git a/include/snet_hip.h b/include/snet_hip.h
--- a/include/snet_hip.h
+++ b/include/snet_hip.h
@@ -45,6 +45,21 @@
 #define SNET_MAX_GEMM_GROUP 8
 int snet_gemm_grouped(const snet_gemm_desc *descs_host, int32_t n_desc, const float *A, float *C, int64_t n_nodes,
                       int64_t a_node_stride, int64_t c_node_stride, const int32_t *row_idx, void *stream);
+#define SNET_GEMM_MAX_SRC 2
+typedef struct snet_gemm_src {
+  const float *A;
+  const float *B;
+  const void *B_split;
+  int64_t a_node_stride, a_off;
+  int32_t K, reserved;
+} snet_gemm_src;
+typedef struct snet_gemm_multi_desc {
+  snet_gemm_src src[SNET_GEMM_MAX_SRC];
+  int64_t c_off;
+  int32_t n_src, d, N, reserved;
+} snet_gemm_multi_desc;
+int snet_gemm_multi(const snet_gemm_multi_desc *descs_host, int32_t n_desc, float *C, int64_t n_nodes, int64_t c_node_stride,
+                    const int32_t *row_idx, const float *table, const int32_t *types, void *stream);
 int64_t snet_gemm_split_size(int32_t K, int32_t N);
 int snet_gemm_split_pack(const float *B_host, int32_t K, int32_t N, void *packed_host);
 typedef struct snet_mlp_plan snet_mlp_plan;
diff --git a/sevennet_amd/_lib.py b/sevennet_amd/_lib.py
--- a/sevennet_amd/_lib.py
+++ b/sevennet_amd/_lib.py
@@ -22,6 +22,16 @@
 class GemmDesc(C.Structure):
     _fields_ = [('B', C.c_void_p), ('B_split', C.c_void_p), ('a_off', C.c_int64), ('c_off', C.c_int64), ('d', C.c_int32), ('K', C.c_int32),
                 ('N', C.c_int32), ('accumulate', C.c_int32)]
+
+
+class GemmSrc(C.Structure):
+    _fields_ = [('A', C.c_void_p), ('B', C.c_void_p), ('B_split', C.c_void_p), ('a_node_stride', C.c_int64), ('a_off', C.c_int64),
+                ('K', C.c_int32), ('reserved', C.c_int32)]
+
+
+class GemmMultiDesc(C.Structure):
+    _fields_ = [('src', GemmSrc * 2), ('c_off', C.c_int64), ('n_src', C.c_int32), ('d', C.c_int32), ('N', C.c_int32),
+                ('reserved', C.c_int32)]
 
 
 class GateSeg(C.Structure):
@@ -50,6 +60,8 @@
                             C.c_int64, C.c_int64, C.c_int64, c_i32p, C.c_int32, c_stream]),
     'snet_gemm_grouped': (C.c_int, [C.POINTER(GemmDesc), C.c_int32, c_f32p, c_f32p, C.c_int64, C.c_int64, C.c_int64,
                                     c_i32p, c_stream]),
+    'snet_gemm_multi': (C.c_int, [C.POINTER(GemmMultiDesc), C.c_int32, c_f32p, C.c_int64, C.c_int64, c_i32p, c_f32p, c_i32p,
+                                  c_stream]),
     'snet_gemm_split_size': (C.c_int64, [C.c_int32, C.c_int32]),
     'snet_gemm_split_pack': (C.c_int, [C.c_void_p, C.c_int32, C.c_int32, C.c_void_p]),
     'snet_act_fwd': (C.c_int, [c_f32p, c_f32p, C.c_int64, C.c_int32, C.c_float, c_stream]),
diff --git a/sevennet_amd/csrc/snet_gemm.hip b/sevennet_amd/csrc/snet_gemm.hip
--- a/sevennet_amd/csrc/snet_gemm.hip
+++ b/sevennet_amd/csrc/snet_gemm.hip
@@ -403,6 +403,220 @@
                            row_idx, P.accumulate);
 }
 
+struct MultiSrc {
+  const float *A;
+  const snet::u32x4 *Bp;
+  int64_t a_node_stride, a_off;
+  int K, nq;
+};
+struct MultiProb {
+  MultiSrc s[2];
+  int64_t c_off;
+  int d, N;
+};
+struct MultiArgs {
+  int n;
+  int first_block[SNET_MAX_GEMM_GROUP + 1];
+  int nby[SNET_MAX_GEMM_GROUP];
+  MultiProb p[SNET_MAX_GEMM_GROUP];
+};
+
+template <int NT>
+__device__ __forceinline__ void gemm_multi_store_table(const snet::f32x16 (&acc)[1][NT], const RowMap &rows, int64_t row0, int half,
+    int li, int tile0, float *__restrict__ C, int64_t n_rows, int N, int64_t c_node_stride, int64_t c_off,
+    const int32_t *__restrict__ row_idx, const float *__restrict__ table, const int32_t *__restrict__ types) {
+#pragma unroll
+  for (int j0 = 0; j0 < 16; j0 += 4) {
+    float *crow[4];
+    float add[4][NT];
+#pragma unroll
+    for (int jj = 0; jj < 4; ++jj) {
+      const int j = j0 + jj, off = (j & 3) + 8 * (j >> 2) + 4 * half;
+      crow[jj] = nullptr;
+      const float *trow = nullptr;
+      if (row0 + off < n_rows) {
+        int64_t n;
+        int m;
+        rows.at(off, n, m);
+        const int64_t node = row_idx ? (int64_t)row_idx[n] : n;
+        crow[jj] = C + node * c_node_stride + c_off + (int64_t)m * N;
+        trow = table + (int64_t)types[node] * c_node_stride + c_off + (int64_t)m * N;
+      }
+#pragma unroll
+      for (int t = 0; t < NT; ++t) {
+        const int col = 32 * (tile0 + t) + li;
+        add[jj][t] = (trow != nullptr && col < N) ? trow[col] : 0.f;
+      }
+    }
+#pragma unroll
+    for (int jj = 0; jj < 4; ++jj)
+#pragma unroll
+      for (int t = 0; t < NT; ++t) {
+        const int col = 32 * (tile0 + t) + li;
+        if (crow[jj] != nullptr && col < N) crow[jj][col] = acc[0][t][j0 + jj] + add[jj][t];
+      }
+  }
+}
+
+template <int NT, int NS>
+__device__ __forceinline__ void gemm_multi_body(snet::u32x4 *Bs, int bx, int by, const MultiProb &P, float *__restrict__ C,
+    int64_t n_rows, int64_t c_node_stride, const int32_t *__restrict__ row_idx, const float *__restrict__ table,
+    const int32_t *__restrict__ types) {
+  using namespace snet;
+  constexpr int SLAB = NT * 192;
+  const int tid = threadIdx.x, lane = tid & 63, wave = __builtin_amdgcn_readfirstlane(tid >> 6);
+  const int half = lane >> 5, li = lane & 31;
+  const int64_t row0 = ((int64_t)bx * 4 + wave) * 32;
+  const int N = P.N, n_tiles = (N + 31) >> 5, tile0 = by * NT;
+  const int nq0 = P.s[0].nq, nq_all = nq0 + (NS > 1 ? P.s[1].nq : 0);
+  const RowMap rows(row0, P.d);
+  const bool a_ok = row0 + li < n_rows;
+
+  int q = 0, K = 0, nq = 0;
+  bool a_vec = false;
+  const float *ap = nullptr;
+  const u32x4 *__restrict__ Bp = nullptr;
+  auto enter_source = [&](const MultiSrc &S) {
+    int64_t n = 0;
+    int m = 0;
+    int l_ = li;
+    asm volatile("" : "+v"(l_));
+    if (a_ok) rows.at(l_, n, m);
+    const int64_t node = row_idx ? (int64_t)row_idx[n] : n;
+    q = 0;
+    K = S.K;
+    nq = S.nq;
+    Bp = S.Bp;
+    ap = S.A + node * S.a_node_stride + S.a_off + (int64_t)m * S.K + 8 * half;
+    a_vec = ((S.K & 3) == 0) && ((S.a_off & 3) == 0) && ((S.a_node_stride & 3) == 0) && ((reinterpret_cast<uintptr_t>(S.A) & 15) == 0);
+  };
+  auto next_step = [&]() {
+    ++q;
+    ap += 16;
+    if (NS > 1 && q == nq) enter_source(P.s[1]);
+  };
+  auto load_a = [&](float (&v)[8]) {
+    const int k = 16 * q + 8 * half;
+    if (a_ok && a_vec && k + 7 < K) {
+      const f32x4 lo = *reinterpret_cast<const f32x4 *>(ap);
+      const f32x4 hi = *reinterpret_cast<const f32x4 *>(ap + 4);
+#pragma unroll
+      for (int i = 0; i < 4; ++i) { v[i] = lo[i]; v[4 + i] = hi[i]; }
+    } else {
+#pragma unroll
+      for (int i = 0; i < 8; ++i) v[i] = (a_ok && k + i < K) ? ap[i] : 0.f;
+    }
+  };
+  constexpr int NST = (SLAB + 255) / 256;
+  auto b_at = [&](int t, int rem) -> u32x4 {
+    const uint32_t byte_off = (((uint32_t)(tile0 + t) * (uint32_t)nq + (uint32_t)q) * 192u + (uint32_t)rem) * 16u;
+    return *reinterpret_cast<const u32x4 *>(reinterpret_cast<const char *>(Bp) + byte_off);
+  };
+  auto load_b = [&](u32x4 (&st)[NST]) {
+    if (tile0 + NT <= n_tiles) {
+#pragma unroll
+      for (int i = 0; i < NST; ++i) {
+        const int idx = tid + 256 * i;
+        const int t = idx / 192, rem = idx - 192 * t;
+        if (SLAB % 256 == 0 || idx < SLAB) st[i] = b_at(t, rem);
+      }
+      return;
+    }
+#pragma unroll
+    for (int i = 0; i < NST; ++i) {
+      const int idx = tid + 256 * i;
+      const int t = idx / 192, rem = idx - 192 * t;
+      u32x4 z = {0u, 0u, 0u, 0u};
+      if (idx < SLAB && tile0 + t < n_tiles) z = b_at(t, rem);
+      st[i] = z;
+    }
+  };
+  auto store_b = [&](int buf, const u32x4 (&st)[NST]) {
+#pragma unroll
+    for (int i = 0; i < NST; ++i) {
+      const int idx = tid + 256 * i;
+      if (idx < SLAB) Bs[buf * SLAB + idx] = st[i];
+    }
+  };
+
+  f32x16 acc[1][NT];
+#pragma unroll
+  for (int t = 0; t < NT; ++t) acc[0][t] = zero16();
+  float av[8], an[8];
+  u32x4 st[NST];
+  enter_source(P.s[0]);
+  load_a(av);
+  load_b(st);
+  store_b(0, st);
+  __syncthreads();
+  int buf = 0;
+  auto k_steps = [&](f32x16 (&ac)[NT], int s0, int s1) {
+    for (int s = s0; s < s1; ++s) {
+      const bool more = s + 1 < nq_all;
+      if (more) {
+        next_step();
+        load_a(an);
+        load_b(st);
+      }
+      const Split3 a = split8(av);
+#pragma unroll
+      for (int t = 0; t < NT; ++t) {
+        bf16x8 b[3];
+#pragma unroll
+        for (int term = 0; term < 3; ++term) b[term] = as_bf16x8(Bs[buf * SLAB + (t * 3 + term) * 64 + lane]);
+        ac[t] = mfma6(a, b, ac[t]);
+      }
+      if (more) {
+        store_b(buf ^ 1, st);
+#pragma unroll
+        for (int i = 0; i < 8; ++i) av[i] = an[i];
+      }
+      __syncthreads();
+      buf ^= 1;
+    }
+  };
+  k_steps(acc[0], 0, nq0);
+  if constexpr (NS > 1) {
+    f32x16 acc1[NT];
+#pragma unroll
+    for (int t = 0; t < NT; ++t) acc1[t] = zero16();
+    k_steps(acc1, nq0, nq_all);
+#pragma unroll
+    for (int t = 0; t < NT; ++t)
+#pragma unroll
+      for (int j = 0; j < 16; ++j) acc[0][t][j] += acc1[t][j];
+  }
+
+  if (table != nullptr)
+    gemm_multi_store_table<NT>(acc, rows, row0, half, li, tile0, C, n_rows, N, c_node_stride, P.c_off, row_idx, table, types);
+  else
+    gemm_split_store<NT, 1>(acc, rows, row0, half, li, tile0, C, n_rows, N, c_node_stride, P.c_off, row_idx, 0);
+}
+
+__global__ __launch_bounds__(256, SNET_GEMM_OCC) void gemm_multi_kernel(MultiArgs G, float *__restrict__ C, int64_t n_nodes,
+                                                                        int64_t c_node_stride, const int32_t *__restrict__ row_idx,
+                                                                        const float *__restrict__ table,
+                                                                        const int32_t *__restrict__ types) {
+  __shared__ snet::u32x4 Bs[2 * 4 * 192];
+  int q = 0;
+  while (q + 1 < G.n && (int)blockIdx.x >= G.first_block[q + 1]) ++q;
+  const MultiProb P = G.p[q];
+  const int b = blockIdx.x - G.first_block[q];
+  const int by = b % G.nby[q], bx = b / G.nby[q];
+  const int64_t n_rows = n_nodes * P.d;
+  if (P.s[1].nq > 0) {
+    if (P.N > 32)
+      gemm_multi_body<2, 2>(Bs, bx, by, P, C, n_rows, c_node_stride, row_idx, table, types);
+    else
+      gemm_multi_body<1, 2>(Bs, bx, by, P, C, n_rows, c_node_stride, row_idx, table, types);
+  } else if (P.N > 64)
+    gemm_multi_body<4, 1>(Bs, bx, by, P, C, n_rows, c_node_stride, row_idx, table, types);
+  else if (P.N > 32)
+    gemm_multi_body<2, 1>(Bs, bx, by, P, C, n_rows, c_node_stride, row_idx, table, types);
+  else
+    gemm_multi_body<1, 1>(Bs, bx, by, P, C, n_rows, c_node_stride, row_idx, table, types);
+}
+
 inline uint16_t bf16_rne(float v) {
   uint32_t u;
   memcpy(&u, &v, 4);
@@ -488,6 +702,56 @@
   else
     gemm_split_grouped_kernel<1><<<(unsigned)total, 256, 0, st>>>(G, A, C, n_nodes, a_node_stride, c_node_stride, row_idx);
   SNET_CHECK_LAUNCH("snet_gemm_grouped");
+  return 0;
+}
+
+extern "C" int snet_gemm_multi(const snet_gemm_multi_desc *descs_host, int32_t n_desc, float *C, int64_t n_nodes,
+                               int64_t c_node_stride, const int32_t *row_idx, const float *table, const int32_t *types,
+                               void *stream) {
+  SNET_REQUIRE(descs_host != nullptr && n_desc >= 1 && n_desc <= SNET_MAX_GEMM_GROUP, "snet_gemm_multi: 1..8 problems required");
+  if (n_nodes <= 0) return 0;
+  SNET_REQUIRE(C != nullptr && (table == nullptr) == (types == nullptr), "snet_gemm_multi: bad argument (C, table without types)");
+  MultiArgs G;
+  G.n = n_desc;
+  int64_t total = 0;
+  int n_src = 0, n_split = 0;
+  for (int i = 0; i < n_desc; ++i) {
+    const snet_gemm_multi_desc &p = descs_host[i];
+    SNET_REQUIRE(p.n_src >= 1 && p.n_src <= SNET_GEMM_MAX_SRC, "snet_gemm_multi: one or two sources per problem");
+    SNET_REQUIRE(p.d >= 1 && p.d <= 150 && p.N >= 1, "snet_gemm_multi: bad problem (1 <= d <= 150)");
+    for (int e = 0; e < p.n_src; ++e) {
+      const snet_gemm_src &s = p.src[e];
+      SNET_REQUIRE(s.A != nullptr && s.K >= 1 && (s.B != nullptr || s.B_split != nullptr), "snet_gemm_multi: bad source");
+      SNET_REQUIRE(snet_gemm_split_size(s.K, p.N) < (1ll << 32), "snet_gemm_multi: weight block too large");
+      ++n_src;
+      n_split += s.B_split != nullptr && s.B == nullptr;
+    }
+  }
+  SNET_REQUIRE(n_split == 0 || n_split == n_src, "snet_gemm_multi: mix of split-packed and fp32 weights in one launch");
+  SNET_REQUIRE(n_split == n_src, "snet_gemm_multi: split-packed weights only (fp32 weights: snet_gemm_grouped)");
+  for (int i = 0; i < n_desc; ++i) {
+    const snet_gemm_multi_desc &p = descs_host[i];
+    MultiProb &P = G.p[i];
+    for (int e = 0; e < 2; ++e) {
+      const snet_gemm_src &s = p.src[e < p.n_src ? e : 0];
+      P.s[e] = {s.A, static_cast<const snet::u32x4 *>(s.B_split), s.a_node_stride, s.a_off, s.K, e < p.n_src ? (s.K + 15) / 16 : 0};
+    }
+    P.c_off = p.c_off;
+    P.d = p.d;
+    P.N = p.N;
+    const int bn = (p.N > 64 && p.n_src == 1) ? 128 : (p.N > 32 ? 64 : 32);
+    const int64_t nbx = (n_nodes * p.d + 127) / 128;
+    const int64_t nby = (p.N + bn - 1) / bn;
+    SNET_REQUIRE(nbx < (1ll << 30), "snet_gemm_multi: too many rows");
+    G.nby[i] = (int)nby;
+    G.first_block[i] = (int)total;
+    total += nbx * nby;
+  }
+  G.first_block[n_desc] = (int)total;
+  SNET_REQUIRE(total < (1ll << 31), "snet_gemm_multi: grid too large");
+  hipStream_t st = static_cast<hipStream_t>(stream);
+  gemm_multi_kernel<<<(unsigned)total, 256, 0, st>>>(G, C, n_nodes, c_node_stride, row_idx, table, types);
+  SNET_CHECK_LAUNCH("snet_gemm_multi");
   return 0;
 }
 
diff --git a/sevennet_amd/csrc/snet_model.cpp b/sevennet_amd/csrc/snet_model.cpp
--- a/sevennet_amd/csrc/snet_model.cpp
+++ b/sevennet_amd/csrc/snet_model.cpp
@@ -1,4 +1,5 @@
 #include <algorithm>
+#include <array>
 #include <cmath>
 #include <cstdio>
 #include <cstdlib>
@@ -110,7 +111,97 @@
     written.push_back({tgt, b.species});
   }
 }
+
+struct MultiPlan {
+  struct Launch {
+    int species;
+    std::vector<snet_gemm_multi_desc> descs;
+    std::vector<std::array<int, SNET_GEMM_MAX_SRC>> which;
+  };
+  bool ok = false;
+  bool transpose = false;
+  int dim = 0;
+  std::vector<const float *> bias;
+  std::vector<Launch> launches;
+  std::vector<std::pair<int, int>> zero;
+};
+
+void plan_multi_source(MultiPlan &P, std::vector<const Linear *> linears, bool transpose) {
+  P = MultiPlan();
+  P.transpose = transpose;
+  for (const Linear *L : linears) P.bias.push_back(L->bias);
+  if (linears.empty() || linears.size() > SNET_GEMM_MAX_SRC) return;
+  int ns = 0;
+  P.dim = transpose ? linears[0]->dim_in : linears[0]->dim_out;
+  for (const Linear *L : linears) {
+    if ((transpose ? L->dim_in : L->dim_out) != P.dim) return;
+    if (L->n_species > 0) {
+      if (ns > 0 && ns != L->n_species) return;
+      ns = L->n_species;
+    }
+  }
+  for (auto &z : transpose ? linears[0]->zero_in : linears[0]->zero) {
+    bool all = true;
+    for (size_t i = 1; i < linears.size(); ++i) {
+      bool found = false;
+      for (auto &y : transpose ? linears[i]->zero_in : linears[i]->zero) found |= (y == z);
+      all &= found;
+    }
+    if (all) P.zero.push_back(z);
+  }
+  std::sort(P.zero.begin(), P.zero.end());
+  for (int s = ns > 0 ? 0 : -1; s < (ns > 0 ? ns : 0); ++s) {
+    MultiPlan::Launch la;
+    la.species = s;
+    for (size_t i = 0; i < linears.size(); ++i)
+      for (const Block &b : linears[i]->blocks) {
+        if (b.species != -1 && b.species != s) continue;
+        const int tgt = transpose ? b.in_off : b.out_off, n = transpose ? b.mul_in : b.mul_out, d = 2 * b.l + 1;
+        size_t k = 0;
+        while (k < la.descs.size() && la.descs[k].c_off != tgt) ++k;
+        if (k == la.descs.size()) {
+          snet_gemm_multi_desc nd;
+          memset(&nd, 0, sizeof nd);
+          nd.c_off = tgt;
+          nd.d = d;
+          nd.N = n;
+          la.descs.push_back(nd);
+          la.which.push_back({});
+        }
+        snet_gemm_multi_desc &p = la.descs[k];
+        if (p.d != d || p.N != n || p.n_src >= SNET_GEMM_MAX_SRC) return;
+        for (int e = 0; e < p.n_src; ++e)
+          if (la.which[k][e] == (int)i) return;
+        snet_gemm_src &src = p.src[p.n_src];
+        src.B_split = transpose ? b.WT : b.W;
+        src.a_node_stride = transpose ? linears[i]->dim_out : linears[i]->dim_in;
+        src.a_off = transpose ? b.out_off : b.in_off;
+        src.K = transpose ? b.mul_out : b.mul_in;
+        la.which[k][p.n_src++] = (int)i;
+      }
+    std::vector<char> covered((size_t)P.dim, 0);
+    auto cover = [&](int64_t off, int64_t len) {
+      if (off < 0 || off + len > P.dim) return false;
+      for (int64_t c = off; c < off + len; ++c) {
+        if (covered[c]) return false;
+        covered[c] = 1;
+      }
+      return true;
+    };
+    for (auto &p : la.descs)
+      if (!cover(p.c_off, (int64_t)p.d * p.N)) return;
+    for (auto &z : P.zero)
+      if (!cover(z.first, z.second)) return;
+    for (char c : covered)
+      if (!c) return;
+    if (la.descs.empty() || la.descs.size() > SNET_MAX_GEMM_GROUP) return;
+    P.launches.push_back(std::move(la));
+  }
+  P.ok = true;
+}
+
 struct Layer {
+  MultiPlan fwd2, rev2, fwd_tab;
   int dx, dmid, gin, dout, wn;
   char tag[13];
   float conv_scale;
@@ -312,6 +403,37 @@
   return 0;
 }
 
+int run_multi(snet_model *m, MultiPlan &P, const float *a0, const float *a1, float *out, int64_t n, const float *table,
+              const int32_t *types, hipStream_t st) {
+  if (n <= 0) return 0;
+  for (auto &z : P.zero)
+    if (hipMemset2DAsync(out + z.first, (size_t)P.dim * 4, 0, (size_t)z.second * 4, (size_t)n, st) != hipSuccess) {
+      snet::set_error("snet_model_eval: memset failed");
+      return 1;
+    }
+  const float *a[SNET_GEMM_MAX_SRC] = {a0, a1};
+  for (MultiPlan::Launch &la : P.launches) {
+    const int32_t *rows = nullptr;
+    int64_t cnt = n;
+    if (la.species >= 0) {
+      cnt = m->species_cnt[la.species];
+      rows = m->species_rows + m->species_off[la.species];
+      if (cnt == 0) continue;
+    }
+    for (size_t k = 0; k < la.descs.size(); ++k)
+      for (int e = 0; e < la.descs[k].n_src; ++e) la.descs[k].src[e].A = a[la.which[k][e]];
+    const int rc = snet_gemm_multi(la.descs.data(), (int)la.descs.size(), out, cnt, P.dim, rows, table, table ? types : nullptr, st);
+    if (rc) return rc;
+  }
+  if (!P.transpose)
+    for (size_t i = P.bias.size(); i-- > 0;)
+      if (P.bias[i]) {
+        const int rc = snet_add_row_bias(out, P.bias[i], n, P.dim, st);
+        if (rc) return rc;
+      }
+  return 0;
+}
+
 }
 
 extern "C" int snet_model_load_memory(const void *blob, int64_t n_bytes, snet_model **out) {
@@ -383,6 +505,15 @@
       }
     }
     good = good && read_linear(r, L.sc) && read_linear(r, L.si1) && read_linear(r, L.si2);
+    if (good && L.sc.present()) {
+      if (t == 0) {
+        plan_multi_source(L.fwd_tab, {&L.si2}, false);
+        if (!L.fwd_tab.zero.empty()) L.fwd_tab.ok = false;
+      } else {
+        plan_multi_source(L.fwd2, {&L.si2, &L.sc}, false);
+        plan_multi_source(L.rev2, {&L.sc, &L.si1}, true);
+      }
+    }
     if (good) {
       const int ns = r.i32();
       good = r.ok && ns >= 1 && ns <= SNET_MAX_GATE_SEGS;
@@ -979,14 +1110,15 @@
     A.off = mark;
     float *sc = nullptr;
     float *h = saved[t].h;
+    const bool merged_y = t == 0 ? L.fwd_tab.ok : L.fwd2.ok;
     if (t == 0) {
-      if (L.sc.present()) {
+      if (L.sc.present() && !merged_y) {
         sc = saved[t].y;
         if ((rc = snet_embed_rows(m->sc0_table, types, sc, N, L.gin, st))) return rc;
       }
       if ((rc = snet_embed_rows(m->h0_table, types, h, NT, L.dx, st))) return rc;
     } else {
-      if (L.sc.present()) {
+      if (L.sc.present() && !merged_y) {
         sc = saved[t].y;
         if ((rc = run_linear(m, L.sc, x, sc, N, false, false, st))) return rc;
       }
@@ -1026,7 +1158,12 @@
         return rc;
     }
     float *y = saved[t].y;
-    if ((rc = run_linear(m, L.si2, mid, y, N, false, sc != nullptr, st))) return rc;
+    if (merged_y)
+      rc = t == 0 ? run_multi(m, L.fwd_tab, mid, nullptr, y, N, m->sc0_table, types, st)
+                  : run_multi(m, L.fwd2, mid, x, y, N, nullptr, nullptr, st);
+    else
+      rc = run_linear(m, L.si2, mid, y, N, false, sc != nullptr, st);
+    if (rc) return rc;
     if ((rc = snet_gate_fwd(y, nullptr, x2, N, L.gin, L.dout, L.segs.data(), (int)L.segs.size(), st))) return rc;
     std::swap(x, x2);
   }
@@ -1086,6 +1223,10 @@
     }
   }
   const size_t mark2 = A.off;
+  auto node_gx = [&](Layer &L, const float *g_y, const float *g_h, float *gx) -> int {
+    if (L.rev2.ok) return run_multi(m, L.rev2, g_y, g_h, gx, N, nullptr, nullptr, st);
+    return run_linear(m, L.si1, g_h, gx, N, true, L.sc.present(), st);
+  };
   for (int t = Lc - 1; t >= 0; --t) {
     Layer &L = m->layers[t];
     A.off = mark2;
@@ -1148,11 +1289,11 @@
           if ((rc = transposed ? bwd_all() : packed ? bwd_tiles(ptile_e0, ptile_nodes, ptile_k) : bwd_tiles(tile_ptr, tile_node, tile_k))) return rc;
           if ((rc = gh_rows(0, N))) return rc;
           if (!tail && (rc = snet_radial_mlp_hidden_bwd(L.mlp_plan, emb, g_h2, E, g_emb, st))) return rc;
-          if (L.sc.present())
+          if (L.sc.present() && !L.rev2.ok)
             if ((rc = run_linear(m, L.sc, g_y, gx_next, N, true, false, st))) return rc;
           SNET_REQUIRE(hipStreamWaitEvent(st, m->ev_h1, 0) == hipSuccess, "snet_model_eval: stream ordering failed");
           if ((rc = snet_halo_reverse_accumulate(m->halo_user, g_h, L.dx, st))) return rc;
-          if ((rc = run_linear(m, L.si1, g_h, gx_next, N, true, L.sc.present(), st))) return rc;
+          if ((rc = node_gx(L, g_y, g_h, gx_next))) return rc;
           std::swap(g_x, gx_next);
           continue;
         }
@@ -1163,9 +1304,9 @@
             return rc;
           }
         if (!tail && (rc = snet_radial_mlp_hidden_bwd(L.mlp_plan, emb, g_h2, E, g_emb, st))) return rc;
-        if (L.sc.present())
+        if (L.sc.present() && !L.rev2.ok)
           if ((rc = run_linear(m, L.sc, g_y, gx_next, N, true, false, st))) return rc;
-        if ((rc = run_linear(m, L.si1, g_h, gx_next, N, true, L.sc.present(), st))) return rc;
+        if ((rc = node_gx(L, g_y, g_h, gx_next))) return rc;
         std::swap(g_x, gx_next);
         continue;
       }
@@ -1196,9 +1337,9 @@
         snet::set_error("snet_model_eval: reverse halo callback failed");
         return rc;
       }
-    if (L.sc.present())
+    if (L.sc.present() && !L.rev2.ok)
       if ((rc = run_linear(m, L.sc, g_y, gx_next, N, true, false, st))) return rc;
-    if ((rc = run_linear(m, L.si1, g_h, gx_next, N, true, L.sc.present(), st))) return rc;
+    if ((rc = node_gx(L, g_y, g_h, gx_next))) return rc;
     std::swap(g_x, gx_next);
   }
   for (int b = 0; b < 2; ++b)
diff --git a/sevennet_amd/engine.py b/sevennet_amd/engine.py
--- a/sevennet_amd/engine.py
+++ b/sevennet_amd/engine.py
@@ -9,7 +9,8 @@
 
 from . import _lib
 from .model_spec import (ACT_CST, ACT_ID, LinearSpec, ModelSpec, build_model_spec, folded_readout, lastlayer_merged_eligible,
-                         layer0_moments_eligible,                         linear_modal_bias, linear_weight_matrices, species_only_tables, transposed_scalar_conv)
+                         layer0_moments_eligible,                         linear_modal_bias, linear_weight_matrices, plan_multi_source, species_only_tables,
+                         transposed_scalar_conv)
 
 
 def _ptr(t: Optional[torch.Tensor]):
@@ -228,6 +229,29 @@
         return out
 
 
+class _MultiPlan:
+
+    def __init__(self, linears: List[_Linear], transpose: bool):
+        self.linears, self.transpose = linears, transpose
+        plan = plan_multi_source([l.spec for l in linears], transpose) if all(l.split for l in linears) else None
+        self.ok = plan is not None
+        if not self.ok:
+            return
+        self.dim_out = linears[0].spec.dim_in if transpose else linears[0].spec.dim_out
+        self.zero = plan[1]
+        self.launches = []
+        for species, probs in plan[0]:
+            arr = (_lib.GemmMultiDesc * len(probs))()
+            for p, (c_off, d, n, srcs) in zip(arr, probs):
+                p.c_off, p.n_src, p.d, p.N = c_off, len(srcs), d, n
+                for s, (i, j) in zip(p.src, srcs):
+                    lin, b = linears[i], linears[i].spec.blocks[j]
+                    s.B_split = (lin.wt if transpose else lin.w)[j].data_ptr()
+                    s.a_node_stride = lin.spec.dim_out if transpose else lin.spec.dim_in
+                    s.a_off, s.K = (b.out_off, b.mul_out) if transpose else (b.in_off, b.mul_in)
+            self.launches.append((species, arr, len(probs), [[i for i, _ in srcs] for _, _, _, srcs in probs]))
+
+
 class _Span:
 
     def __init__(self, eng, name):
@@ -301,6 +325,7 @@
                 L.sc = _Linear(ls.sc, sd[ls.sc.name], self.dev, split, mi) if ls.sc is not None else None
                 L.si1 = _Linear(ls.si1, sd[ls.si1.name], self.dev, split, mi, sd.get(ls.si1.bias_name))
                 L.si2 = _Linear(ls.si2, sd[ls.si2.name], self.dev, split, mi, sd.get(ls.si2.bias_name))
+                self._plan_two_source(L, first=not self.layers)
                 L.mlp_w, L.mlp_wt = [], []
                 rw = ls.radial_weights(sd)
                 for i in range(len(ls.mlp_dims) - 1):
@@ -478,6 +503,37 @@
             _lib.check(self.lib.snet_add_row_bias(_ptr(y), _ptr(lin.bias), n, sp.dim_out, _stream()), 'snet_add_row_bias')
         return y
 
+    @staticmethod
+    def _plan_two_source(L, first: bool):
+        L.fwd2 = _MultiPlan([L.si2, L.sc], False) if L.sc is not None else None
+        L.rev2 = _MultiPlan([L.sc, L.si1], True) if (L.sc is not None and not first) else None
+        L.fwd_tab = _MultiPlan([L.si2], False) if (L.sc is not None and first) else None
+        if L.fwd_tab is not None and L.fwd_tab.ok and L.fwd_tab.zero:
+            L.fwd_tab.ok = False
+
+    def _linear_multi(self, plan: _MultiPlan, srcs, n, g: Graph, table=None):
+        out = self._new(max(n, 0), plan.dim_out)
+        for off, ln in plan.zero:
+            out[:, off:off + ln].zero_()
+        ptrs = [s.data_ptr() for s in srcs]
+        for species, arr, cnt, which in plan.launches:
+            rows, m = None, n
+            if species >= 0:
+                rows = g.species_rows[species]
+                m = rows.numel()
+                if m == 0:
+                    continue
+            for p, w in zip(arr, which):
+                for s, i in zip(p.src, w):
+                    s.A = ptrs[i]
+            _lib.check(self.lib.snet_gemm_multi(arr, cnt, _ptr(out), m, plan.dim_out, _ptr(rows), _ptr(table),
+                                                _ptr(g.types) if table is not None else None, _stream()), 'snet_gemm_multi')
+        if not plan.transpose and n > 0:
+            for lin in reversed(plan.linears):
+                if lin.bias is not None:
+                    _lib.check(self.lib.snet_add_row_bias(_ptr(out), _ptr(lin.bias), n, plan.dim_out, _stream()), 'snet_add_row_bias')
+        return out
+
     def _linear_T(self, lin: _Linear, gy, n, g: Graph, out=None, accumulate=False):
         sp = lin.spec
         gx = out if out is not None else self._new(max(n, 0), sp.dim_in)
@@ -687,8 +743,12 @@
                         pending = halo.forward_start(h, N)
                     else:
                         halo.forward(h, N)
+            tab0 = t == 0 and self.h0_table is not None
+            merged_y = (L.fwd_tab is not None and L.fwd_tab.ok and self.sc0_table is not None) if tab0 else (L.fwd2 is not None and L.fwd2.ok)
             with _Span(self, 'node_linear_fwd'):
-                if t == 0 and self.h0_table is not None:
+                if merged_y:
+                    sc = None
+                elif tab0:
                     sc = None
                     if self.sc0_table is not None:
                         sc = self._new(N, ls.gate.irreps_in.dim)
@@ -734,7 +794,10 @@
             if L.fused_bwd:
                 w = None
             with _Span(self, 'node_linear_fwd'):
-                y = self._linear(L.si2, m, N, g) if sc is None else self._linear(L.si2, m, N, g, out=sc, accumulate=True)
+                if merged_y:
+                    y = self._linear_multi(L.fwd_tab, [m], N, g, table=self.sc0_table) if tab0 else self._linear_multi(L.fwd2, [m, x], N, g)
+                else:
+                    y = self._linear(L.si2, m, N, g) if sc is None else self._linear(L.si2, m, N, g, out=sc, accumulate=True)
             xo = self._new(N, ls.gate.irreps_out.dim)
             with _Span(self, 'gate_fwd'):
                 _lib.check(lib.snet_gate_fwd(_ptr(y), None, _ptr(xo), N, ls.gate.irreps_in.dim,
@@ -962,13 +1025,18 @@
             del g_w, g_h2
             if t == 0:
                 break
-            with _Span(self, 'node_linear_bwd'):
-                g_x = self._linear_T(L.sc, g_y, N, g) if L.sc is not None else None
+            merged_gx = L.rev2 is not None and L.rev2.ok
+            if not merged_gx:
+                with _Span(self, 'node_linear_bwd'):
+                    g_x = self._linear_T(L.sc, g_y, N, g) if L.sc is not None else None
             if pending is not None:
                 with _Span(self, 'halo_rev'):
                     halo.reverse_finish(pending, g_h)
             with _Span(self, 'node_linear_bwd'):
-                g_x = self._linear_T(L.si1, g_h, N, g, out=g_x, accumulate=g_x is not None)
+                if merged_gx:
+                    g_x = self._linear_multi(L.rev2, [g_y, g_h], N, g)
+                else:
+                    g_x = self._linear_T(L.si1, g_h, N, g, out=g_x, accumulate=g_x is not None)
             saved[t] = None
         if side is not None:
             torch.cuda.current_stream().wait_stream(side)
diff --git a/sevennet_amd/model_spec.py b/sevennet_amd/model_spec.py
--- a/sevennet_amd/model_spec.py
+++ b/sevennet_amd/model_spec.py
@@ -138,6 +138,58 @@
             w = w.reshape(b.mul_in, b.mul_out)
         out.append(np.ascontiguousarray(w * b.alpha, dtype=np.float32))
     return out
+
+
+MAX_GEMM_GROUP = 8
+MAX_GEMM_SRC = 2
+
+
+def linear_untouched(spec: LinearSpec, transpose: bool):
+    if not transpose:
+        return list(spec.zero_out)
+    fed = {b.in_off for b in spec.blocks}
+    return [(off, m * (2 * l + 1)) for off, (m, l, _) in zip(spec.irreps_in.offsets(), spec.irreps_in) if off not in fed]
+
+
+def plan_multi_source(linears, transpose: bool):
+    assert 1 <= len(linears) <= MAX_GEMM_SRC
+    dim = {(sp.dim_in if transpose else sp.dim_out) for sp in linears}
+    ns = {sp.n_species for sp in linears if sp.n_species}
+    if len(dim) != 1 or len(ns) > 1:
+        return None
+    dim = dim.pop()
+    zero = set(linear_untouched(linears[0], transpose))
+    for sp in linears[1:]:
+        zero &= set(linear_untouched(sp, transpose))
+    zero = sorted(zero)
+    launches = []
+    for s in (range(ns.pop()) if ns else (-1,)):
+        probs, by_tgt = [], {}
+        for i, sp in enumerate(linears):
+            for j, b in enumerate(sp.blocks):
+                if b.species not in (-1, s):
+                    continue
+                tgt, n = (b.in_off, b.mul_in) if transpose else (b.out_off, b.mul_out)
+                if tgt not in by_tgt:
+                    by_tgt[tgt] = len(probs)
+                    probs.append((tgt, 2 * b.l + 1, n, []))
+                _, d, n0, src = probs[by_tgt[tgt]]
+                if (d, n0) != (2 * b.l + 1, n) or any(i_ == i for i_, _ in src):
+                    return None
+                src.append((i, j))
+        covered = np.zeros(dim, bool)
+        for off, d, n, _ in probs:
+            if off + d * n > dim or covered[off:off + d * n].any():
+                return None
+            covered[off:off + d * n] = True
+        for off, ln in zero:
+            if covered[off:off + ln].any():
+                return None
+            covered[off:off + ln] = True
+        if not probs or len(probs) > MAX_GEMM_GROUP or not covered.all():
+            return None
+        launches.append((s, probs))
+    return launches, zero
 
 
 def linear_rows_fp64(spec: LinearSpec, flat: np.ndarray, x: np.ndarray, species=None, modal_idx: int = -1, bias_flat=None) -> np.ndarray:
```

Result: no change. 2.946 million atom-steps/s (median of 6 runs) (+1.1%).
